# siliconsorcery/crdt

Hardware: AMD Instinct MI355X
Metric: merged records/sec (node) + % HBM roofline, 1B records x 1024 replicas (higher is better)
Workload: dtype int64

## Files before the change

crdt_amd/_capi.py:

```python
from __future__ import annotations

import ctypes
import os
import sys

_HERE = os.path.dirname(os.path.abspath(__file__))
LIB_PATH = os.environ.get("CRDT_LIB_PATH") or os.path.join(_HERE, "libcrdt_mi355x.so")

CRDT_OK = 0
CRDT_CLOCK_DRIFT = 1
CRDT_DUPLICATE_NODE = 2
CRDT_OVERFLOW = 3
CRDT_E_INVALID = -1
CRDT_E_HIP = -2
CRDT_E_NOMEM = -3
CRDT_E_KEY_RANGE = -4
CRDT_E_NO_DEVICE = -5
CRDT_E_COMM = -6

CRDT_MEM_HOST = 0
CRDT_MEM_DEVICE = 1
CRDT_NULL_VALUE = 0xFFFFFFFF


class CrdtBatch(ctypes.Structure):
    _fields_ = [("key_id", ctypes.c_void_p), ("lt", ctypes.c_void_p), ("rank", ctypes.c_void_p),
                ("val", ctypes.c_void_p), ("millis", ctypes.c_void_p), ("offsets", ctypes.c_void_p),
                ("n_changesets", ctypes.c_uint32), ("mem", ctypes.c_int32)]


class CrdtResult(ctypes.Structure):
    _fields_ = [("status", ctypes.c_int32), ("n_stored", ctypes.c_uint32),
                ("exc_changeset", ctypes.c_uint32), ("reserved", ctypes.c_uint32),
                ("exc_index", ctypes.c_uint64), ("canonical_lt", ctypes.c_int64),
                ("drift_ms", ctypes.c_int64), ("counter", ctypes.c_int64),
                ("n_present", ctypes.c_uint64), ("n_won", ctypes.c_uint64)]

    def as_dict(self) -> dict:
        return {f: getattr(self, f) for f, _ in self._fields_ if f != "reserved"}


class CrdtTiming(ctypes.Structure):
    _fields_ = [("scan_ms", ctypes.c_double), ("clock_ms", ctypes.c_double),
                ("apply_ms", ctypes.c_double), ("apply_launches", ctypes.c_uint32),
                ("apply_total", ctypes.c_uint32), ("total_ms", ctypes.c_double),
                ("route_ms", ctypes.c_double), ("part1_ms", ctypes.c_double), ("part2_ms", ctypes.c_double),
                ("resolve_ms", ctypes.c_double), ("part1_records", ctypes.c_uint64),
                ("sent_bytes", ctypes.c_uint64)]

    def as_dict(self) -> dict:
        return {f: getattr(self, f) for f, _ in self._fields_}


class CrdtExport(ctypes.Structure):
    _fields_ = [("key_id", ctypes.c_void_p), ("lt", ctypes.c_void_p), ("rank", ctypes.c_void_p),
                ("val", ctypes.c_void_p), ("mod", ctypes.c_void_p), ("n", ctypes.c_uint64),
                ("n_live", ctypes.c_uint64), ("mem", ctypes.c_int32), ("device", ctypes.c_int32)]


EXPORT_TILE = 2048
EXPORT_SCAN_STEP = 1024
EXPORT_COUNT_GRID = 2048
TABLE_TILE = 2048
TABLE_CLOCK_GRID = 2048
FANIN_MAX = 8
FANOUT_MAX = 8
SYNC_CLOCK_GRID = 2048

ALL_REDUCE_FN = ctypes.CFUNCTYPE(ctypes.c_int, ctypes.c_void_p, ctypes.c_void_p, ctypes.c_uint64, ctypes.c_int32,
                                 ctypes.c_void_p)
ALL_GATHER_FN = ctypes.CFUNCTYPE(ctypes.c_int, ctypes.c_void_p, ctypes.c_void_p, ctypes.c_void_p, ctypes.c_uint64,
                                 ctypes.c_void_p)
ALL_TO_ALL_FN = ctypes.CFUNCTYPE(ctypes.c_int, ctypes.c_void_p, ctypes.c_uint32, ctypes.POINTER(ctypes.c_void_p),
                                 ctypes.POINTER(ctypes.c_void_p), ctypes.POINTER(ctypes.c_uint32),
                                 ctypes.POINTER(ctypes.c_uint64), ctypes.POINTER(ctypes.c_uint64),
                                 ctypes.POINTER(ctypes.c_uint64), ctypes.POINTER(ctypes.c_uint64), ctypes.c_void_p)


class CrdtCommOps(ctypes.Structure):
    _fields_ = [("user", ctypes.c_void_p), ("mem", ctypes.c_int32), ("reserved", ctypes.c_int32),
                ("all_reduce_i64", ALL_REDUCE_FN), ("all_gather_i64", ALL_GATHER_FN),
                ("all_to_all_v", ALL_TO_ALL_FN)]


COMM_ID_BYTES = 128
ABI_VERSION = 5

_P = ctypes.c_void_p
_U32 = ctypes.c_uint32
_U64 = ctypes.c_uint64
_I64 = ctypes.c_int64
_I32 = ctypes.c_int32
_INT = ctypes.c_int

SIGNATURES = {
    "crdt_abi_version": (_INT, []),
    "crdt_status_string": (ctypes.c_char_p, [_INT]),
    "crdt_device_count": (_INT, [_P]),
    "crdt_create": (_INT, [_INT, _U32, _U64, _P]),
    "crdt_destroy": (None, [_P]),
    "crdt_reserve": (_INT, [_P, _U64]),
    "crdt_capacity": (_INT, [_P, _P]),
    "crdt_set_local_rank": (_INT, [_P, _U32]),
    "crdt_get_canonical": (_INT, [_P, _P]),
    "crdt_set_canonical": (_INT, [_P, _I64]),
    "crdt_put_rows": (_INT, [_P, _P, _P, _P, _P, _P, _U64, _I32]),
    "crdt_read_rows": (_INT, [_P, _P, _U64, _P, _P, _P, _P, _I32]),
    "crdt_modified_since": (_INT, [_P, _U64, _I64, _P, _P]),
    "crdt_export_since": (_INT, [_P, _U64, _I64, _P]),
    "crdt_export_read": (_INT, [_P, _U64, _U64, _P, _P, _P, _P, _P]),
    "crdt_export_release": (_INT, [_P]),
    "crdt_count_since": (_INT, [_P, _U64, _I64, _P, _P]),
    "crdt_export_flagged": (_INT, [_P, _U64, _P, _I32, ctypes.c_uint8, _P]),
    "crdt_clear_rows": (_INT, [_P, _U64, _U64]),
    "crdt_remap_ranks": (_INT, [_P, _U64, _P, _U32]),
    "crdt_put_stamped": (_INT, [_P, _P, _P, _U64, _I64, _I32, _P]),
    "crdt_refresh_canonical": (_INT, [_P, _U64, _P]),
    "crdt_merge": (_INT, [_P, _P, _I64, _P, _P]),
    "crdt_merge_table": (_INT, [_P, _P, _U64, _I64, _I64, _P, _I32, _P]),
    "crdt_sync_tables": (_INT, [_P, _P, _U64, _I64, _I64, _I64, _P, _P, _I32, _P, _P]),
    "crdt_fanin_tables": (_INT, [_P, _P, _P, _U32, _U64, _I64, _P, _I32, _P]),
    "crdt_fanout_tables": (_INT, [_P, _P, _P, _U32, _U64, _I64, _P, _I32, _P]),
    "crdt_comm_unique_id": (_INT, [_P]),
    "crdt_comm_init_rccl": (_INT, [_P, _U32, _U32, _P]),
    "crdt_comm_init_ops": (_INT, [_P, _U32, _U32, _P]),
    "crdt_comm_info": (_INT, [_P, _P, _P]),
    "crdt_comm_free": (_INT, [_P]),
    "crdt_set_presharded": (_INT, [_P, _INT]),
    "crdt_set_comm_timeout": (_INT, [_P, _U32]),
    "crdt_comm_state": (_INT, [_P, _P, _P]),
    "crdt_set_merge_path": (_INT, [_P, _INT]),
    "crdt_set_counts": (_INT, [_P, _INT]),
    "crdt_set_rank_bound": (_INT, [_P, _U32]),
    "crdt_reserve_scratch": (_INT, [_P, _U64]),
    "crdt_set_row_bytes": (_INT, [_P, _U32]),
    "crdt_last_plan": (_INT, [_P, _P]),
    "crdt_route_tune_info": (_INT, [_P, _P, _P]),
    "crdt_place_info": (_INT, [_P, _P, _P, _P, _P]),
    "crdt_last_path": (_INT, [_P, _P]),
    "crdt_set_timing": (_INT, [_P, _INT]),
    "crdt_get_timing": (_INT, [_P, _P]),
}


class NativeLibraryMissing(RuntimeError):
    pass


_lib = None


def load():
    global _lib
    if _lib is not None:
        return _lib
    if os.environ.get("CRDT_AMD_NO_TORCH") != "1" and "torch" not in sys.modules:
        try:
            import torch
        except ImportError:
            pass
    if not os.path.exists(LIB_PATH):
        raise NativeLibraryMissing(
            f"{LIB_PATH} is missing: build it with `python -c 'import __graft_entry__ as g; g.build()'`"
            " (there is no CPU fallback)")
    lib = ctypes.CDLL(LIB_PATH)
    for name, (res, args) in SIGNATURES.items():
        fn = getattr(lib, name)
        fn.restype = res
        fn.argtypes = args
    if lib.crdt_abi_version() != ABI_VERSION:
        raise NativeLibraryMissing(f"{LIB_PATH} has ABI {lib.crdt_abi_version()}, the bindings ABI {ABI_VERSION}:"
                                   " rebuild it")
    _lib = lib
    return lib


def status_string(status: int) -> str:
    return load().crdt_status_string(status).decode()


def device_count() -> int:
    n = ctypes.c_int(0)
    load().crdt_device_count(ctypes.byref(n))
    return n.value
```

crdt_amd/csrc/crdt_merge.hip:

```cpp
#include <dlfcn.h>
#include <hip/hip_runtime.h>
#include <rccl/rccl.h>

#include <stdint.h>
#include <stdio.h>
#include <stdlib.h>
#include <string.h>

#include <unistd.h>

#include <algorithm>
#include <atomic>
#include <chrono>
#include <thread>
#include <new>
#include <vector>

#include "crdt_merge.h"

namespace {

constexpr int kShift = 16;
constexpr int64_t kMaxCounter = 0xFFFF;
constexpr int64_t kMaxDrift = 60000;
// ... 27 lines not shown
}
__device__ inline uint2 load_cold(const Table& t, uint64_t k) {
    const u32x2u v = *reinterpret_cast<const u32x2u*>(row_ptr(t, k) + 16);
    return make_uint2(v.x, v.y);
}
__device__ inline void store_hc(const Table& t, uint64_t k, uint4 h, uint2 x) {
    char* p = row_ptr(t, k);
    if (t.stride == 32) {
        u32x8a a;
        a.s0 = h.x; a.s1 = h.y; a.s2 = h.z; a.s3 = h.w; a.s4 = x.x; a.s5 = x.y; a.s6 = 0u; a.s7 = 0u;
        *reinterpret_cast<u32x8a*>(p) = a;
        return;
    }
    u32x4u a;
    a.x = h.x; a.y = h.y; a.z = h.z; a.w = h.w;
    *reinterpret_cast<u32x4u*>(p) = a;
    u32x2u b;
    b.x = x.x; b.y = x.y;
    *reinterpret_cast<u32x2u*>(p + 16) = b;
}
__device__ inline int64_t row_mod(const Table& t, uint64_t k) {
    const uint4 h = load_hot(t, k);
    return (int64_t)(((uint64_t)h.w << 32) | load_cold(t, k).x);
}
__device__ inline void store_row(const Table& t, uint64_t k, int64_t lt, uint32_t rank, uint32_t val, int64_t mod) {
    store_hc(t, k, make_uint4((uint32_t)lt, (uint32_t)((uint64_t)lt >> 32), rank, (uint32_t)((uint64_t)mod >> 32)),
             make_uint2((uint32_t)mod, val));
}

struct Misc {
    uint32_t cand_count;
    uint32_t stop;
    uint32_t err;
    uint32_t vdone;
    uint32_t tiles_hot;
    crdt_result result;
    unsigned long long fr_lo, fr_hi;
    uint32_t fr_rlo, fr_rhi;
    unsigned long long key_end;
    unsigned long long route_own;
    unsigned long long shard_status;
    unsigned long long fr_cmax;
    unsigned long long hot_n;
    unsigned long long hot_spare;
    unsigned long long present[kCounterSlots];
    unsigned long long won[kCounterSlots];
};
static_assert(sizeof(Misc) % 16 == 0, "Misc is memset as whole 16-B words");

typedef unsigned int u32x4 __attribute__((ext_vector_type(4)));
typedef long long i64x2 __attribute__((ext_vector_type(2)));

__host__ __device__ inline int64_t wsub(int64_t a, int64_t b) { return (int64_t)((uint64_t)a - (uint64_t)b); }
__host__ __device__ inline int64_t imax(int64_t a, int64_t b) { return a > b ? a : b; }

struct HlcSend {
    int32_t status;
    int64_t drift_ms;
    int64_t counter;
    int64_t canonical;
    __host__ __device__ void into(crdt_result& res) const {
        res.status = status;
        res.drift_ms = drift_ms;
        res.counter = counter;
        res.canonical_lt = canonical;
    }
};
__host__ __device__ inline HlcSend hlc_send(int64_t r, int64_t wall) {
    const int64_t m = r >> kShift, mn = imax(m, wall);
    const int64_t cn = (m == mn) ? (r & kMaxCounter) + 1 : 0;
    if (wsub(mn, wall) > kMaxDrift) return {CRDT_CLOCK_DRIFT, wsub(mn, wall), 0, r};
    if (cn > kMaxCounter) return {CRDT_OVERFLOW, 0, cn, r};
    return {CRDT_OK, 0, 0, (int64_t)(((uint64_t)mn << kShift) + (uint64_t)cn)};
}

__device__ inline int64_t wave_max(int64_t v) {
#pragma unroll
    for (int off = 32; off > 0; off >>= 1) v = imax(v, __shfl_xor(v, off, 64));
    return v;
}

__device__ inline void block_raise_u64(unsigned long long v, unsigned long long* dst) {
    __shared__ unsigned long long s_v[4];
#pragma unroll
    for (int off = 32; off > 0; off >>= 1) {
        const unsigned long long o = __shfl_xor(v, off, 64);
        v = o > v ? o : v;
    }
    if ((threadIdx.x & 63) == 0) s_v[threadIdx.x >> 6] = v;
    __syncthreads();
    if (threadIdx.x == 0) {
        for (int w = 1; w < 4; ++w) v = s_v[w] > v ? s_v[w] : v;
        if (v > *(volatile unsigned long long*)dst) atomicMax(dst, v);
    }
    __syncthreads();
}

__device__ inline int64_t wave_scan_max_incl(int64_t v, int lane) {
#pragma unroll
    for (int off = 1; off < 64; off <<= 1) {
        int64_t u = __shfl_up(v, off, 64);
        if (lane >= off) v = imax(v, u);
    }
    return v;
}

__device__ inline uint32_t digit_count(uint32_t* bins, uint32_t d, bool act, int lane) {
    const unsigned long long a = __ballot(act);
    if (!a) return 0;
    const int L = __ffsll((long long)a) - 1;
    const uint32_t d0 = __shfl(d, L, 64);
    const bool same = act && d == d0;
    const unsigned long long m = __ballot(same);
    const unsigned long long below = (1ull << lane) - 1;
    uint32_t base = 0;
    if (lane == L) base = atomicAdd(&bins[d0], (uint32_t)__popcll(m));
    base = __shfl(base, L, 64);
    if (same) return base + (uint32_t)__popcll(m & below);
    return act ? atomicAdd(&bins[d], 1u) : 0u;
}

constexpr uint32_t kHotSample = 16;

__host__ __device__ inline uint64_t ord64(int64_t x) { return (uint64_t)x ^ (1ull << 63); }

constexpr uint32_t kHistSub = 7;

struct KeyMap {
    uint32_t gsh;
    uint32_t dsh;
};
__host__ __device__ inline uint32_t km_digit(KeyMap m, uint32_t k, uint32_t shift) {
    return ((((k & ((1u << m.gsh) - 1u)) << m.dsh) | ((k >> m.gsh) >> shift)) & 255u);
}

constexpr uint32_t kHotShift = 12;
constexpr uint32_t kHotProbe = 15;
constexpr uint32_t kHotMax = 256;

struct ScanHist {
    const uint32_t* key;
    const uint32_t* ptb;
    uint64_t cap;
    uint32_t shift;
    uint32_t* hist;
    KeyMap km{0u, 8u};
    uint32_t htile = kHistSub * kTile;
};
struct ScanHot {
    uint32_t hot = 0;
    uint32_t* hhist = nullptr;
};

__global__ __launch_bounds__(1024) void k_hot_count(const uint32_t* __restrict__ hhist, uint64_t tiles, uint32_t hot,
                                                    Misc* __restrict__ misc)
{
    __shared__ unsigned long long s_sum[16];
    unsigned long long n = 0;
    const uint64_t words = tiles * 256;
    for (uint64_t x = (uint64_t)blockIdx.x * 1024 + threadIdx.x; x < words; x += (uint64_t)gridDim.x * 1024)
        if ((x & 255u) < hot) n += hhist[x];
#pragma unroll
    for (int off = 32; off > 0; off >>= 1) n += __shfl_xor(n, off, 64);
    if ((threadIdx.x & 63) == 0) s_sum[threadIdx.x >> 6] = n;
    __syncthreads();
    if (threadIdx.x == 0) {
        for (int k = 1; k < 16; ++k) n += s_sum[k];
        if (n) atomicAdd(&misc->hot_n, n);
    }
}

template <bool kEager, bool kMillis, bool kFrame, bool kHist, bool kVec, bool kHot = false>
__device__ __forceinline__ void scan_body(
    const int64_t* __restrict__ lt, const uint32_t* __restrict__ rank,
    const int64_t* __restrict__ millis, const uint64_t* __restrict__ offs,
    const uint32_t* __restrict__ tstart, uint32_t jbase, int64_t c0,
    int64_t wall, uint32_t local_rank,
    int64_t* __restrict__ T, Misc* __restrict__ misc, uint32_t* __restrict__ cand_tile, ScanHist sh, bool jx,
    ScanHot ho = ScanHot{})
{
    __shared__ int64_t s_max[kScanThreads / 64];
    __shared__ int s_flag[kScanThreads / 64];
    __shared__ unsigned long long s_fr[kFrame ? 5 * (kScanThreads / 64) : 1];
    constexpr uint32_t kBins = kHot ? 512u : 256u;
    __shared__ uint32_t s_h[kHist ? 2 * kBins : 1];
    static_assert(!kHist || kScanThreads == 256, "one histogram bin per thread");
    static_assert(!kHot || kHist, "hot bins: beside the fused histogram");
    const uint32_t j = jbase + (jx ? blockIdx.x : blockIdx.y);
    const uint64_t beg = offs[j], end = offs[j + 1];
    const uint32_t t0 = tstart[j], nt = tstart[j + 1] - t0;
    const int lane = threadIdx.x & 63, w = threadIdx.x >> 6;
    constexpr uint32_t kStep = kHist ? kHistSub : 1u;
    const uint32_t ustride = jx ? gridDim.y : gridDim.x;
    for (uint32_t u = jx ? blockIdx.y : blockIdx.x; u * kStep < nt; u += ustride) {
      if (kHist) {
#pragma unroll
        for (uint32_t x = 0; x < (kHist ? 2 * kBins : 0u); x += 256) s_h[kHist ? x + threadIdx.x : 0] = 0;
        __syncthreads();
      }
      const uint32_t te = std::min<uint32_t>(u * kStep + kStep, nt);
      for (uint32_t t = u * kStep; t < te; ++t) {
        const uint64_t base = beg + (uint64_t)t * kTile;
        int64_t m = INT64_MIN;
        int f = 0;
        int64_t v[kScanItems];
        uint32_t rk[kEager ? kScanItems : 1];
        int64_t mv[kEager && kMillis ? kScanItems : 1];
        uint32_t kk[kHist ? kScanItems : 1];
        auto idx = [&](int q) -> uint64_t {
            return kVec ? base + (uint64_t)(q >> 2) * (4 * kScanThreads) + threadIdx.x * 4u + (q & 3)
                        : base + (uint64_t)q * kScanThreads + threadIdx.x;
        };
        bool vec_done[kVec ? kScanItems / 4 : 1];
#pragma unroll
        for (int g = 0; g < (kVec ? kScanItems / 4 : 0); ++g) {
            const uint64_t i0 = idx(4 * g);
            vec_done[kVec ? g : 0] = i0 + 4 <= end;
            if (i0 + 4 <= end) {
                const u32x4u a = *reinterpret_cast<const u32x4u*>(lt + i0);
                const u32x4u b = *reinterpret_cast<const u32x4u*>(lt + i0 + 2);
                v[4 * g] = (int64_t)(((uint64_t)a.y << 32) | a.x); v[4 * g + 1] = (int64_t)(((uint64_t)a.w << 32) | a.z);
                v[4 * g + 2] = (int64_t)(((uint64_t)b.y << 32) | b.x); v[4 * g + 3] = (int64_t)(((uint64_t)b.w << 32) | b.z);
                if (kHist) {
                    const u32x4u kv = *reinterpret_cast<const u32x4u*>(sh.key + i0);
                    kk[kHist ? 4 * g : 0] = kv.x; kk[kHist ? 4 * g + 1 : 0] = kv.y;
                    kk[kHist ? 4 * g + 2 : 0] = kv.z; kk[kHist ? 4 * g + 3 : 0] = kv.w;
                }
                if (kEager) {
                    const u32x4u rv = *reinterpret_cast<const u32x4u*>(rank + i0);
                    rk[kEager ? 4 * g : 0] = rv.x; rk[kEager ? 4 * g + 1 : 0] = rv.y;
                    rk[kEager ? 4 * g + 2 : 0] = rv.z; rk[kEager ? 4 * g + 3 : 0] = rv.w;
                }
            }
        }
#pragma unroll
        for (int q = 0; q < kScanItems; ++q) {
            const uint64_t i = idx(q);
            const bool vd = kVec && vec_done[kVec ? q >> 2 : 0];
            if (!vd) {
                v[q] = i < end ? lt[i] : INT64_MIN;
                if (kHist) kk[kHist ? q : 0] = i < end ? __builtin_nontemporal_load(sh.key + i) : UINT32_MAX;
            }
            if (kEager) {
                if (!vd) rk[kEager ? q : 0] = i < end ? rank[i] : 0u;
                if (kMillis) mv[kMillis ? q : 0] = (millis && i < end) ? millis[i] : 0;
            }
            m = imax(m, v[q]);
        }
        if (kHist) {
            const uint32_t tb = (t - u * kStep) * (uint32_t)kTile;
#pragma unroll
            for (int q = 0; q < kScanItems; ++q) {
                const uint32_t k = kk[kHist ? q : 0];
                const uint32_t gb = kVec ? (uint32_t)(q >> 2) * (4u * kScanThreads) : (uint32_t)q * kScanThreads;
                uint32_t dg = km_digit(sh.km, k, sh.shift);
                if (kHot) dg = (k >> kHotShift) < ho.hot ? 256u + (k >> kHotShift) : dg;
                digit_count(s_h + (tb + gb >= sh.htile ? kBins : 0u), dg, (k >> sh.km.gsh) < sh.cap, lane);
            }
        }
#pragma unroll
        for (int q = 0; q < kScanItems; ++q) {
            if (v[q] > c0) {
                const uint64_t i = idx(q);
                const int64_t ms = (kMillis && millis) ? (kEager ? mv[kEager && kMillis ? q : 0] : millis[i])
                                                       : (v[q] >> kShift);
                const uint32_t r = kEager ? rk[kEager ? q : 0] : rank[i];
                f |= (r == local_rank) | (wsub(ms, wall) > kMaxDrift);
            }
        }
        unsigned long long flo = 0, fhi = 0, frl = 0, frh = 0;
        uint32_t fcm = 0;
        if (kFrame) {
#pragma unroll
            for (int q = 0; q < kScanItems; ++q) {
                const uint64_t i = idx(q);
                if (i < end) {
                    const uint64_t o = ord64(v[q]);
                    flo = ~o > flo ? ~o : flo;
                    fhi = o > fhi ? o : fhi;
                    fcm = std::max<uint32_t>(fcm, (uint32_t)v[q] & 0xFFFFu);
                    if (kEager) {
                        const uint32_t r = rk[kEager ? q : 0];
                        frl = (uint32_t)~r > frl ? (uint32_t)~r : frl;
                        frh = r > frh ? r : frh;
                    }
                }
            }
#pragma unroll
            for (int off = 32; off > 0; off >>= 1) {
                const unsigned long long a = __shfl_xor(flo, off, 64), b = __shfl_xor(fhi, off, 64);
                const unsigned long long c = __shfl_xor(frl, off, 64), d = __shfl_xor(frh, off, 64);
                flo = a > flo ? a : flo; fhi = b > fhi ? b : fhi; frl = c > frl ? c : frl; frh = d > frh ? d : frh;
                fcm = std::max<uint32_t>(fcm, (uint32_t)__shfl_xor(fcm, off, 64));
            }
            if (lane == 0) {
                s_fr[5 * w] = flo; s_fr[5 * w + 1] = fhi; s_fr[5 * w + 2] = frl; s_fr[5 * w + 3] = frh; s_fr[5 * w + 4] = fcm;
            }
        }
        m = wave_max(m);
        const int fw = __any(f) | (m > c0 ? 2 : 0);
        if (lane == 0) { s_max[w] = m; s_flag[w] = fw; }
        __syncthreads();
        if (threadIdx.x == 0) {
            if (kFrame) {
                unsigned long long fc = fcm;
                for (int k = 1; k < kScanThreads / 64; ++k) {
                    flo = s_fr[5 * k] > flo ? s_fr[5 * k] : flo;
                    fhi = s_fr[5 * k + 1] > fhi ? s_fr[5 * k + 1] : fhi;
                    frl = s_fr[5 * k + 2] > frl ? s_fr[5 * k + 2] : frl;
                    frh = s_fr[5 * k + 3] > frh ? s_fr[5 * k + 3] : frh;
                    fc = s_fr[5 * k + 4] > fc ? s_fr[5 * k + 4] : fc;
                }
                if (fc > *(volatile unsigned long long*)&misc->fr_cmax) atomicMax(&misc->fr_cmax, fc);
                if (flo > *(volatile unsigned long long*)&misc->fr_lo) atomicMax(&misc->fr_lo, flo);
                if (fhi > *(volatile unsigned long long*)&misc->fr_hi) atomicMax(&misc->fr_hi, fhi);
                if ((uint32_t)frl > *(volatile uint32_t*)&misc->fr_rlo) atomicMax(&misc->fr_rlo, (uint32_t)frl);
                if ((uint32_t)frh > *(volatile uint32_t*)&misc->fr_rhi) atomicMax(&misc->fr_rhi, (uint32_t)frh);
            }
            int64_t tm = s_max[0];
            int tf = s_flag[0];
            for (int k = 1; k < kScanThreads / 64; ++k) { tm = imax(tm, s_max[k]); tf |= s_flag[k]; }
            T[t0 + t] = tm;
// ... 1233 lines not shown
        n = 0;
    }
};

template <typename T>
struct HBuf {
    T* p = nullptr;
    size_t n = 0;
    hipError_t ensure(size_t want) {
        if (want <= n && p) return hipSuccess;
        if (p) { hipHostFree(p); p = nullptr; n = 0; }
        size_t m = std::max<size_t>(want, 16);
        hipError_t e = hipHostMalloc(&p, m * sizeof(T), hipHostMallocDefault);
        if (e == hipSuccess) n = m;
        return e;
    }
    void release() { if (p) hipHostFree(p); p = nullptr; n = 0; }
};

constexpr uint32_t kRl1MaxPieces = 4;
struct Rl1Scratch {
    DBuf<uint32_t> hist, toff, part, choff, dstart2, tseg, ibase, ibucket, ksu32, kj2;
    DBuf<int64_t> kslt;
    DBuf<u32x4> rec2;
    DBuf<uint64_t> plan;
    HBuf<uint64_t> hplan;
    size_t pw = 0, u32w = 0;
    uint32_t nt2 = 0, nc2 = 0;
    uint32_t ngrp = 0;
    size_t nsg = 0;
    uint64_t nw = 0;
    void release() {
        hist.release(); toff.release(); part.release(); choff.release(); dstart2.release(); tseg.release();
        ibase.release(); ibucket.release(); ksu32.release(); kj2.release(); kslt.release(); rec2.release();
        plan.release(); hplan.release();
    }
};

struct Segs {
    std::vector<uint64_t> beg, end;
    std::vector<uint32_t> j;
    void from_offsets(const uint64_t* offs, uint32_t R) {
        beg.resize(R); end.resize(R); j.resize(R);
        for (uint32_t x = 0; x < R; ++x) { beg[x] = offs[x]; end[x] = offs[x + 1]; j[x] = x; }
    }
};

}

constexpr uint32_t kFormNoWholeLines = 64;
constexpr uint32_t kFormNoKey8 = 128;
constexpr uint32_t kFormNoKey16 = 256;
constexpr uint32_t kFormNoReverse = 512;
constexpr uint32_t kFormNoHistW = 1024;
constexpr uint32_t kFormNoHw = 2048;
constexpr uint32_t kFormNoVecLoads = 8192;
constexpr uint32_t kFormNoVecScan = 32768;
constexpr uint32_t kFormNoVecRoute = 131072;
constexpr uint32_t kFormBigTile2 = 65536;
constexpr uint32_t kFormNoOwnInPlace = 524288;
constexpr uint32_t kFormNoCompact = 1u << 20;
constexpr uint32_t kFormFbackXcd = 1u << 21;
constexpr uint32_t kFormFbackWide = 1u << 22;
constexpr uint32_t kFormScanJx = 1u << 24;
constexpr uint32_t kFormNoScanJx = 1u << 25;
constexpr uint32_t kFormNoPosT = 1u << 31;
constexpr uint32_t kFormNoItemLists = 1u << 28;
constexpr uint32_t kFormNoFbackPre = 1u << 27;
constexpr uint32_t kFormFbackPre512 = 1u << 29;
constexpr uint32_t kFormNoSparseK = 1u << 26;
constexpr uint32_t kScanJxMax = 8192;
constexpr uint32_t kFormOverlap = 1u << 23;
constexpr uint32_t kPartPad = 1024;
constexpr uint32_t kPutGrid = 2048;

struct crdt_ctx {
    int device = 0;
    hipStream_t stream = nullptr;
    uint32_t local_rank = 0;
    Table table{nullptr, 24};
    uint64_t cap = 0;
    int64_t canonical = 0;

    Misc* d_misc = nullptr;
    Misc* h_misc = nullptr;
    DBuf<long long> d_M;
    DBuf<long long> d_event;
    DBuf<uint64_t> d_plan;
    HBuf<uint64_t> h_plan;
    const uint64_t* d_offs = nullptr;
    const uint32_t* d_tstart = nullptr;
    DBuf<int64_t> d_T, d_Cprev, d_Rj, d_Cj, d_candP, d_candms;
    DBuf<uint32_t> d_candtile, d_candkind;
    DBuf<long long> d_candkey;
    DBuf<uint32_t> s_key, s_rank, s_val;
    hipStream_t cstream = nullptr;
    std::vector<hipEvent_t> cevents;
    const uint32_t* kv_key = nullptr;
    const uint32_t* kv_val = nullptr;
    uint64_t kv_n = 0, kv_done = 0, kv_window = 4ull << 20;
    uint32_t kv_win = 0;
    DBuf<int64_t> s_lt, s_millis, s_mod;
    DBuf<uint8_t> s_flags;
    DBuf<uint32_t> s_out;
    DBuf<uint32_t> x_key, x_rank, x_val, x_counts;
    DBuf<int64_t> x_lt, x_mod;
    DBuf<uint64_t> x_offs;
    DBuf<unsigned long long> x_words;
    bool x_valid = false;
    uint64_t x_n = 0;
    DBuf<uint32_t> t_sel;
    DBuf<unsigned long long> t_words, t_mask;
    DBuf<uint8_t> t_wflags;
    DBuf<uint8_t> t_fstep, t_fmask;
    DBuf<unsigned long long> t_fcounts;
    bool table_merge = true;
    bool last_table = false;
    bool last_sync = false;
    bool last_fanin = false;
    bool last_fanout = false;
    DBuf<long long> d_word;
    DBuf<unsigned long long> d_ibase;
    uint32_t plan_R = 0;
    uint64_t plan_tiles = 0;
    uint32_t plan_mt = 0;
    int apply_items = 0;
    bool timing = false;
    std::vector<hipEvent_t> events;
    std::vector<uint32_t> windows;
    bool sorted_phases = false;
    uint64_t p1_records = 0;
    uint32_t apply_total = 0;
    int merge_path = 0;
    uint64_t hw = 0;
    uint64_t hw_read = 0;
    uint64_t hw_next = 0;
    bool key_end_valid = false;
    DBuf<u32x4> p1_rec, p2_rec;
    DBuf<uint32_t> p1_kj, p2_kj;
    static constexpr int kPlaceMax = 4;
    DBuf<u32x4> pc_rec[kPlaceMax];
    DBuf<uint32_t> pc_kj[kPlaceMax];
    int place_k = 0;
    int place_trial = 0;
    int place_best = -1;
    int place_idle = 0;
    float place_ms[kPlaceMax] = {};
    bool place_timed = false;
    bool place_warm = false;
    hipEvent_t place_ev[2] = {};
    DBuf<uint32_t> p_hist, p_toff, p_part, p_choff, p_dstart1, p_dstart2, p_l2map;
    DBuf<uint64_t> p_plan, p_l1beg;
    DBuf<uint32_t> p_ibase, p_ksu32, p_tseg, p_ibucket;
    DBuf<uint32_t> p_ilist;
    HBuf<uint32_t> h_ilist;
    DBuf<int64_t> p_kslt;
    HBuf<uint64_t> h_pplan;
    bool last_sorted = false;
    bool counts = true;
    bool fused = false;
    bool scan_eager = false;
    bool no_fuse = false;
    bool xcd_map = true;
    bool packed_resolve = true;
    bool frame_on = false;
    uint32_t rank_bound = 0;
    uint32_t form_off = 0;
    bool env_dynamic = false;
    bool hist_fuse = true;
    uint32_t l1_tile = 0;
    uint32_t plan_l1_tile = 28672;
    bool last_hist1_fused = false;
    bool frame_lt_only = false;
    const uint32_t* d_ptb = nullptr;
    uint64_t plan_ptiles = 0;
    DBuf<uint32_t> p_hist1;
    bool hist1_fused = false;
    bool hist1_routed = false;
    const uint32_t* hist1_key = nullptr;
    uint32_t hist1_shift = 0;
    bool last_packed = false;
    bool last_wire_pk = false;
    bool last_own_in_place = false;
    bool last_key8 = false;
    bool last_key16 = false;
    bool last_compact = false;
    bool last_hw = false;
    bool flags_sorted = true;
    int fback_chk = 6;
    bool last_flagged = false;
    int combine = 1;
    bool last_combined = false;
    uint32_t sparse_t = 2048;
    uint32_t hot_buckets = 256;
    uint32_t hot_share = 5;
    uint32_t hot_probe = kHotProbe;
    uint32_t hot_skip = 0;
    uint32_t hist1_hot = 0;
    bool last_hot_direct = false;
    DBuf<uint32_t> p_hist1h, p_toffh, p_dstarth;
    DBuf<uint64_t> p_l1begh;
    int route_l1 = 1;
    bool rl1_call_head = false;
    bool rl1_call_all = false;
    bool rl1_cmp = false;
    bool last_rl1_head = false;
    uint64_t last_rl1_head_in = 0, last_rl1_head_out = 0;
    uint32_t last_rl1_head_digits = 0;
    uint64_t sent_bytes = 0;
    uint32_t rl1_pieces = 2;
    uint32_t rl1_call_pieces = 2;
    uint32_t last_rl1_pieces = 0;
    bool last_route_l1 = false;
    bool route_tune = true;
    struct RouteTune {
        uint64_t shape = 0;
        uint32_t trial = 0;
        int best = -1;
        long long us[5] = {-1, -1, -1, -1, -1};
    } rt;
    int tune_mode = -1;
    bool tune_trial = false;
    DBuf<long long> d_tune;
    HBuf<long long> h_tune;
    DBuf<uint32_t> rl_rec;
    DBuf<uint16_t> rl_k16;
    uint64_t rl_cap = 0;
    Rl1Scratch rl_os[kRl1MaxPieces + 1];
    Rl1Scratch rl_hf;
    DBuf<uint32_t> rl_hrec;
    DBuf<uint16_t> rl_hk16;
    DBuf<unsigned long long> rl_hcnt;
    HBuf<unsigned long long> h_hcnt;
    hipEvent_t rl_evh = nullptr;
    hipEvent_t ov_ev[2] = {};
    DBuf<uint32_t> e_key, e_val;
    DBuf<uint64_t> e_pk;
    DBuf<unsigned long long> e_cnt, e_cur;
    HBuf<unsigned long long> h_ebase;
    DBuf<uint32_t> e_icnt;
    DBuf<uint32_t> e_bbase;
    DBuf<uint64_t> e_off;
    DBuf<unsigned long long> e_csum;
    bool last_ordered = false;
    DBuf<uint16_t> f_pos1, f_pos2;
    DBuf<uint8_t> f_flag1, f_flag2;
    DBuf<uint32_t> f_hist2, f_toff2;
    DBuf<unsigned long long> f_cin_key;
    DBuf<uint32_t> f_cin_val;
    DBuf<uint8_t> f_cin_pres;
    bool keys_checked = false;
    bool resolved = false;
    crdt_timing last_timing{};
    Segs segs;
    uint32_t n_ranks = 1, rank = 0;
    bool has_comm = false;
    bool presharded = false;
    crdt_comm_ops ops{};
    void* rccl_comm = nullptr;
    DBuf<long long> d_gsend, d_grecv, d_pbase, d_sum;
    DBuf<unsigned long long> d_rcnt, d_rrecv;
    DBuf<unsigned long long> d_rcur;
    hipEvent_t route_ev = nullptr;
    hipStream_t sstream = nullptr;
    hipStream_t ostream = nullptr;
    hipEvent_t rl_evs[kRl1MaxPieces] = {};
    hipEvent_t rl_evx[kRl1MaxPieces] = {};
    hipEvent_t rl_evo = nullptr;
    uint64_t recv_cap = 0;
    HBuf<uint64_t> h_rcnt;
    DBuf<uint32_t> r_skey, r_srank, r_sval, r_key, r_rank, r_val;
    DBuf<int64_t> r_slt, r_lt;
    DBuf<uint64_t> r_perm;
    DBuf<uint8_t> r_flags, r_sflags;
    HBuf<uint8_t> h_stage;
    HBuf<long long> h_sum;
    DBuf<long long> d_agree;
    HBuf<long long> h_agree;
    DBuf<unsigned long long> d_rl1cnt;
    HBuf<uint64_t> h_rl1cnt;
    bool finish_posted = false;
    int fail_rank = -1, fail_at = 0;
    uint32_t comm_timeout_ms = 300000;
    int64_t comm_deadline_ns = 0;
    std::atomic<int> comm_state{0};
    std::atomic<const char*> comm_phase{"idle"};
    int stall_rank = -1, stall_at = 0, stall_ms = 0;
    bool stall_dev = false;
};

constexpr uint32_t kL1TileDefault = 28672;
inline uint32_t l1_choose(const crdt_ctx* c, uint32_t R, uint64_t n) {
    if (c->l1_tile == 14336u || c->l1_tile == 28672u) return c->l1_tile;
    return R && n / R < 4ull * kL1TileDefault ? 14336u : kL1TileDefault;
}
inline uint32_t l1_plan_tile(const crdt_ctx* c) { return c->plan_l1_tile; }


namespace {

#define HIPCHK(expr)                                   \
    do {                                               \
        hipError_t _e = (expr);                        \
        if (_e != hipSuccess) return CRDT_E_HIP;       \
    } while (0)

#define HIPALLOC(expr)                                                     \
    do {                                                                   \
        hipError_t _e = (expr);                                            \
        if (_e == hipErrorOutOfMemory) return CRDT_E_NOMEM;                \
        if (_e != hipSuccess) return CRDT_E_HIP;                           \
    } while (0)

#define HIPLST(expr)                                                       \
    do {                                                                   \
        hipError_t _e = (expr);                                            \
        if (_e != hipSuccess && !lst) lst = CRDT_E_HIP;                    \
    } while (0)

int comm_wait(crdt_ctx* c, hipStream_t s, hipEvent_t e = nullptr);
#define SYNCHK(c, s)                                                       \
    do {                                                                   \
        int _w = comm_wait((c), (s));                                      \
        if (_w) return _w;                                                 \
    } while (0)

inline unsigned grid_for(uint64_t n, unsigned per) { return (unsigned)((n + per - 1) / per); }

hipError_t ensure_events(crdt_ctx* c, size_t n) {
    while (c->events.size() < n) {
        hipEvent_t e;
        hipError_t r = hipEventCreate(&e);
        if (r != hipSuccess) return r;
        c->events.push_back(e);
    }
    return hipSuccess;
}

int overlap_fork(crdt_ctx* c) {
    if (!c->sstream) HIPCHK(hipStreamCreateWithFlags(&c->sstream, hipStreamNonBlocking));
    for (hipEvent_t& e : c->ov_ev)
        if (!e) HIPCHK(hipEventCreateWithFlags(&e, hipEventDisableTiming));
    HIPCHK(hipEventRecord(c->ov_ev[0], c->stream));
    HIPCHK(hipStreamWaitEvent(c->sstream, c->ov_ev[0], 0));
    return CRDT_OK;
}
int overlap_join(crdt_ctx* c) {
    HIPCHK(hipEventRecord(c->ov_ev[1], c->sstream));
    HIPCHK(hipStreamWaitEvent(c->stream, c->ov_ev[1], 0));
    return CRDT_OK;
}

template <typename T>
int stage(crdt_ctx* c, DBuf<T>& buf, const T* src, uint64_t n, int32_t mem, const T** out) {
    if (!src) { *out = nullptr; return CRDT_OK; }
    if (mem == CRDT_MEM_DEVICE) { *out = src; return CRDT_OK; }
    HIPALLOC(buf.ensure(n ? n : 1));
    if (n) HIPCHK(hipMemcpyAsync(buf.p, src, n * sizeof(T), hipMemcpyHostToDevice, c->stream));
    *out = buf.p;
    return CRDT_OK;
}

struct Cols {
    const uint32_t* key = nullptr;
    const int64_t* lt = nullptr;
    const uint32_t* rank = nullptr;
    const uint32_t* val = nullptr;
    const int64_t* millis = nullptr;
    bool packed_in = false;
};

int validate_batch(const crdt_batch* b) {
    if (!b || !b->offsets) return CRDT_E_INVALID;
    if (b->mem != CRDT_MEM_HOST && b->mem != CRDT_MEM_DEVICE) return CRDT_E_INVALID;
    if (b->offsets[0] != 0) return CRDT_E_INVALID;
    for (uint32_t j = 0; j < b->n_changesets; ++j)
        if (b->offsets[j + 1] < b->offsets[j]) return CRDT_E_INVALID;
    const uint64_t n = b->offsets[b->n_changesets];
    if (n > 0 && (!b->lt || !b->rank)) return CRDT_E_INVALID;
    if ((uint64_t)b->n_changesets >= (1ull << 24)) return CRDT_E_INVALID;
    for (uint32_t j = 0; j < b->n_changesets; ++j)
        if (b->offsets[j + 1] - b->offsets[j] >= kLowMask) return CRDT_E_INVALID;
    return CRDT_OK;
}

int stage_check_cols(crdt_ctx* c, const crdt_batch* b, Cols* cols) {
    const uint64_t n = b->offsets[b->n_changesets];
    int st;
    if ((st = stage(c, c->s_lt, b->lt, n, b->mem, &cols->lt))) return st;
    if ((st = stage(c, c->s_rank, b->rank, n, b->mem, &cols->rank))) return st;
    if ((st = stage(c, c->s_millis, b->millis, n, b->mem, &cols->millis))) return st;
    return CRDT_OK;
}

int stage_apply_cols(crdt_ctx* c, const crdt_batch* b, Cols* cols) {
    const uint64_t n = b->offsets[b->n_changesets];
    if (n > 0 && (!b->key_id || !b->val)) return CRDT_E_INVALID;
    int st;
    if ((st = stage(c, c->s_key, b->key_id, n, b->mem, &cols->key))) return st;
    if ((st = stage(c, c->s_lt, b->lt, n, b->mem, &cols->lt))) return st;
    if ((st = stage(c, c->s_rank, b->rank, n, b->mem, &cols->rank))) return st;
    if ((st = stage(c, c->s_val, b->val, n, b->mem, &cols->val))) return st;
    return CRDT_OK;
}

int upload_plan(crdt_ctx* c, const crdt_batch* b, uint64_t* tiles_out, uint32_t* max_tiles) {
    const uint32_t R = b->n_changesets;
    const size_t half = (R + 2) / 2;
    const size_t words = (R + 1) + 2 * half;
    HIPALLOC(c->h_plan.ensure(words));
    HIPALLOC(c->d_plan.ensure(words));
    uint64_t* h_offs = c->h_plan.p;
    uint32_t* h_tstart = reinterpret_cast<uint32_t*>(c->h_plan.p + (R + 1));
    uint32_t* h_ptb = reinterpret_cast<uint32_t*>(c->h_plan.p + (R + 1) + half);
    uint64_t tiles = 0, ptiles = 0;
    uint32_t mt = 0;
    c->plan_l1_tile = l1_choose(c, R, b->offsets[R] - b->offsets[0]);
    for (uint32_t j = 0; j <= R; ++j) {
        h_offs[j] = b->offsets[j];
        h_tstart[j] = (uint32_t)tiles;
        h_ptb[j] = (uint32_t)ptiles;
        if (j < R) {
            const uint64_t nj = b->offsets[j + 1] - b->offsets[j];
            const uint64_t tj = (nj + kTile - 1) / kTile;
            tiles += tj;
            ptiles += (nj + l1_plan_tile(c) - 1) / l1_plan_tile(c);
            mt = std::max<uint32_t>(mt, (uint32_t)tj);
        }
    }
    if (tiles >= (1ull << 32)) return CRDT_E_INVALID;
    HIPCHK(hipMemcpyAsync(c->d_plan.p, c->h_plan.p, words * sizeof(uint64_t), hipMemcpyHostToDevice, c->stream));
    c->d_offs = c->d_plan.p;
    c->d_tstart = reinterpret_cast<const uint32_t*>(c->d_plan.p + (R + 1));
    c->d_ptb = reinterpret_cast<const uint32_t*>(c->d_plan.p + (R + 1) + half);
    c->plan_ptiles = ptiles;
    *tiles_out = tiles;
    *max_tiles = mt;
    return CRDT_OK;
}

int reset_misc(crdt_ctx* c) {
    HIPCHK(hipMemsetAsync(c->d_misc, 0, sizeof(Misc), c->stream));
    return CRDT_OK;
}

crdt_result cleared_result(int64_t canonical) {
    crdt_result res;
    memset(&res, 0, sizeof(res));
    res.exc_index = UINT64_MAX;
    res.canonical_lt = canonical;
    return res;
}

constexpr size_t kEvStart = 0, kEvScan = 1, kEvClock = 2, kEvApply = 3, kEvEnd = 4;
inline size_t ev_window(size_t k, bool end) { return 5 + 2 * k + (end ? 1 : 0); }
inline size_t events_for(size_t nsegs) {
    return std::max(ev_window(nsegs / kTimingStride + 2, true), ev_window(3, true)) + 1;
}

inline void raise_hw(crdt_ctx* c, uint64_t key_end) {
    c->hw = std::max<uint64_t>(c->hw, std::min<uint64_t>(key_end, c->cap));
}

inline void ev_record(crdt_ctx* c, size_t idx) {
    if (c->timing && idx < c->events.size()) hipEventRecord(c->events[idx], c->stream);
}

int phase_scan(crdt_ctx* c, const crdt_batch* home, int64_t wall, long long* d_maxima, bool allow_fuse = false,
               bool frame = false, bool bound_ok = true, bool keys_ready = false, const KeyMap* route_km = nullptr) {
    c->fused = false;
    c->resolved = false;
    c->hist1_fused = false;
    c->hist1_hot = 0;
    int st = validate_batch(home);
    if (st) return st;
    const uint32_t R = home->n_changesets;
    Cols cols;
    if ((st = stage_check_cols(c, home, &cols))) return st;
    uint64_t tiles = 0;
    uint32_t mt = 0;
    if ((st = upload_plan(c, home, &tiles, &mt))) return st;
    HIPALLOC(c->d_T.ensure(tiles + 1));
    HIPALLOC(c->d_candtile.ensure(tiles + 1));
    HIPALLOC(c->d_candkey.ensure(tiles + 1));
    HIPALLOC(c->d_candP.ensure(tiles + 1));
    HIPALLOC(c->d_candkind.ensure(tiles + 1));
    HIPALLOC(c->d_candms.ensure(tiles + 1));
    if ((st = reset_misc(c))) return st;
    if (!tiles)
        k_fill_i64<<<grid_for(std::max<uint32_t>(R, 1), 256), 256, 0, c->stream>>>(d_maxima, std::max<uint32_t>(R, 1),
                                                                                     INT64_MIN);
    c->plan_R = R;
    c->plan_tiles = tiles;
    c->plan_mt = mt;
    c->frame_on = frame;
    c->frame_lt_only = frame && bound_ok && c->rank_bound && !c->scan_eager;
    c->fused = allow_fuse && !c->no_fuse && tiles > 0 && tiles <= kClockTilesMax && R <= kClockRMax;
    const bool hist = c->frame_lt_only && c->hist_fuse && keys_ready && home->mem == CRDT_MEM_DEVICE &&
                      R <= kWindow && tiles > 0 && home->key_id;
    const bool rhist = !hist && route_km && frame && c->hist_fuse && R <= kWindow && tiles > 0 && home->key_id &&
                       !home->millis;
    if (hist || rhist) {
        HIPALLOC(c->p_hist1.ensure(c->plan_ptiles * kDigits));
        c->hist1_fused = true;
        c->hist1_routed = rhist;
        c->hist1_key = home->key_id;
        c->hist1_shift = rhist || c->cap > (1ull << 20) ? 20u : (uint32_t)kSBits;
    }
    uint32_t hot = hist && c->cap > (1ull << 20) ? std::min<uint32_t>(c->hot_buckets, kHotMax) : 0u;
    if (hot && c->hot_skip) {
        --c->hot_skip;
        hot = 0;
    }
    if (hot) {
        HIPALLOC(c->p_hist1h.ensure(c->plan_ptiles * kDigits));
        c->hist1_hot = hot;
    }
    const ScanHot shot{hot, c->p_hist1h.p};
    ScanHist shr{home->key_id, c->d_ptb, c->cap, 20u, c->p_hist1.p};
    shr.htile = l1_plan_tile(c);
    ScanHist shist{home->key_id, c->d_ptb, c->cap, c->hist1_shift, c->p_hist1.p};
    shist.htile = l1_plan_tile(c);
    if (rhist) shr.km = *route_km;
    if (tiles) {
        const uint32_t cap_x = std::max<uint32_t>(1, 65536u / std::max<uint32_t>(R, 1));
        const uint32_t gx = std::max<uint32_t>(1, std::min<uint32_t>(mt, cap_x));
        const uint32_t gxh = std::max<uint32_t>(1, std::min<uint32_t>((mt + kHistSub - 1) / kHistSub, cap_x));
        const bool hgrid = hist || rhist;
        const uint64_t nwg = (uint64_t)(hgrid ? gxh : gx) * R;
        const bool jx = !(c->form_off & kFormNoScanJx) && ((c->form_off & kFormScanJx) || nwg <= kScanJxMax);
        for (uint32_t jb = 0; jb < R; jb += 65535) {
            const uint32_t gy = std::min<uint32_t>(65535, R - jb);
            const dim3 gdh = jx ? dim3(gy, std::min<uint32_t>(gxh, 65535)) : dim3(gxh, gy);
            const dim3 gd = jx ? dim3(gy, std::min<uint32_t>(gx, 65535)) : dim3(gx, gy);
            if (rhist)
                k_scan<true, false, true, true, true><<<gdh, kScanThreads, 0, c->stream>>>(
                    cols.lt, cols.rank, nullptr, c->d_offs, c->d_tstart, jb, c->canonical, wall,
                    c->local_rank, c->d_T.p, c->d_misc, c->d_candtile.p, shr, jx);
            else if (hist && hot && !(c->form_off & kFormNoVecScan))
                k_scan<true><<<gdh, kScanThreads, 0, c->stream>>>(
                    cols.lt, cols.rank, cols.millis, c->d_offs, c->d_tstart, jb, c->canonical, wall,
                    c->local_rank, c->d_T.p, c->d_misc, c->d_candtile.p, shist, jx, shot);
            else if (hist && hot)
                k_scan<false><<<gdh, kScanThreads, 0, c->stream>>>(
                    cols.lt, cols.rank, cols.millis, c->d_offs, c->d_tstart, jb, c->canonical, wall,
                    c->local_rank, c->d_T.p, c->d_misc, c->d_candtile.p, shist, jx, shot);
            else if (hist && !(c->form_off & kFormNoVecScan))
                k_scan<false, true, true, true, true><<<gdh, kScanThreads, 0, c->stream>>>(
                    cols.lt, cols.rank, cols.millis, c->d_offs, c->d_tstart, jb, c->canonical, wall,
                    c->local_rank, c->d_T.p, c->d_misc, c->d_candtile.p,
                    shist, jx);
            else if (hist)
                k_scan<false, true, true, true><<<gdh, kScanThreads, 0, c->stream>>>(
                    cols.lt, cols.rank, cols.millis, c->d_offs, c->d_tstart, jb, c->canonical, wall,
                    c->local_rank, c->d_T.p, c->d_misc, c->d_candtile.p, shist, jx);
            else if (c->frame_lt_only)
                k_scan<false, true, true><<<gd, kScanThreads, 0, c->stream>>>(
                    cols.lt, cols.rank, cols.millis, c->d_offs, c->d_tstart, jb, c->canonical, wall,
                    c->local_rank, c->d_T.p, c->d_misc, c->d_candtile.p, ScanHist{}, jx);
            else if (frame && !cols.millis)
                k_scan<true, false, true><<<gd, kScanThreads, 0, c->stream>>>(
                    cols.lt, cols.rank, nullptr, c->d_offs, c->d_tstart, jb, c->canonical, wall,
                    c->local_rank, c->d_T.p, c->d_misc, c->d_candtile.p, ScanHist{}, jx);
            else if (frame)
                k_scan<true, true, true><<<gd, kScanThreads, 0, c->stream>>>(
                    cols.lt, cols.rank, cols.millis, c->d_offs, c->d_tstart, jb, c->canonical, wall,
                    c->local_rank, c->d_T.p, c->d_misc, c->d_candtile.p, ScanHist{}, jx);
            else if (c->scan_eager && !cols.millis)
                k_scan<true, false><<<gd, kScanThreads, 0, c->stream>>>(
                    cols.lt, cols.rank, nullptr, c->d_offs, c->d_tstart, jb, c->canonical, wall,
                    c->local_rank, c->d_T.p, c->d_misc, c->d_candtile.p, ScanHist{}, jx);
            else if (c->scan_eager)
                k_scan<true><<<gd, kScanThreads, 0, c->stream>>>(
                    cols.lt, cols.rank, cols.millis, c->d_offs, c->d_tstart, jb, c->canonical, wall,
                    c->local_rank, c->d_T.p, c->d_misc, c->d_candtile.p, ScanHist{}, jx);
            else
                k_scan<false><<<gd, kScanThreads, 0, c->stream>>>(
                    cols.lt, cols.rank, cols.millis, c->d_offs, c->d_tstart, jb, c->canonical, wall,
                    c->local_rank, c->d_T.p, c->d_misc, c->d_candtile.p, ScanHist{}, jx);
        }
        if (hot)
            k_hot_count<<<64, 1024, 0, c->stream>>>(c->p_hist1h.p, c->plan_ptiles, hot, c->d_misc);
        if (!c->fused)
            k_tmax<<<std::min<uint32_t>(R, 4096), 256, 0, c->stream>>>(c->d_T.p, c->d_tstart, R, d_maxima);
        HIPCHK(hipGetLastError());
    }
    return CRDT_OK;
}

int phase_clock(crdt_ctx* c, const crdt_batch* home, int64_t wall, const long long* d_maxima,
                long long* d_event, const long long* d_pbase = nullptr,
                const unsigned long long* d_ibase_in = nullptr) {
    const uint32_t R = c->plan_R;
    if (!home || home->n_changesets != R) return CRDT_E_INVALID;
    int st;
    Cols cols;
    if ((st = stage_check_cols(c, home, &cols))) return st;
    HIPALLOC(c->d_Cprev.ensure(R + 1));
    HIPALLOC(c->d_Rj.ensure(R + 1));
    HIPALLOC(c->d_Cj.ensure(R + 1));
    const unsigned long long* d_ibase = d_ibase_in;
    if (!R) k_event_init<<<1, 64, 0, c->stream>>>(d_event);
    if (c->fused) {
        k_clock<true><<<1, 1024, 0, c->stream>>>(nullptr, c->d_T.p, c->d_tstart, R, wall, c->canonical,
                                                 c->d_Cprev.p, c->d_Rj.p, c->d_Cj.p, d_event);
        k_verify<true><<<kVerifyBlocks, 64, 0, c->stream>>>(
            cols.lt, cols.rank, cols.millis, c->d_offs, c->d_tstart, R, c->d_T.p, c->d_Cprev.p, wall,
            c->local_rank, c->d_misc, c->d_candtile.p, c->d_candkey.p, c->d_candP.p, c->d_candkind.p,
            c->d_candms.p, d_pbase, d_ibase, d_event, c->canonical, c->d_Rj.p, c->d_Cj.p, (uint32_t)kTile);
        c->resolved = true;
        HIPCHK(hipGetLastError());
        return CRDT_OK;
    }
    if (R) k_clock<false><<<1, 1024, 0, c->stream>>>(d_maxima, nullptr, nullptr, R, wall, c->canonical,
                                                     c->d_Cprev.p, c->d_Rj.p, c->d_Cj.p, d_event);
    if (c->plan_tiles)
        k_verify<false><<<kVerifyBlocks, 64, 0, c->stream>>>(
            cols.lt, cols.rank, cols.millis, c->d_offs, c->d_tstart, R, c->d_T.p, c->d_Cprev.p, wall,
            c->local_rank, c->d_misc, c->d_candtile.p, c->d_candkey.p, c->d_candP.p, c->d_candkind.p,
            c->d_candms.p, d_pbase, d_ibase, d_event, 0, nullptr, nullptr, (uint32_t)kTile);
    HIPCHK(hipGetLastError());
    return CRDT_OK;
}

int phase_resolve(crdt_ctx* c, long long* d_event) {
    k_resolve_local<<<1, 256, 0, c->stream>>>(c->d_misc, c->d_candkey.p, c->d_candP.p, c->d_candkind.p,
                                              c->d_candms.p, d_event);
    HIPCHK(hipGetLastError());
    return CRDT_OK;
}


int kv_copy_next(crdt_ctx* c) {
    const uint64_t b = c->kv_done, e = std::min<uint64_t>(c->kv_n, b + c->kv_window);
    if (c->kv_win >= c->cevents.size()) {
        hipEvent_t ev;
        HIPCHK(hipEventCreateWithFlags(&ev, hipEventDisableTiming));
        c->cevents.push_back(ev);
    }
    HIPCHK(hipMemcpyAsync(c->s_key.p + b, c->kv_key + b, (e - b) * sizeof(uint32_t), hipMemcpyHostToDevice,
                          c->cstream));
    HIPCHK(hipMemcpyAsync(c->s_val.p + b, c->kv_val + b, (e - b) * sizeof(uint32_t), hipMemcpyHostToDevice,
                          c->cstream));
    HIPCHK(hipEventRecord(c->cevents[c->kv_win], c->cstream));
    HIPCHK(hipStreamWaitEvent(c->stream, c->cevents[c->kv_win], 0));
    c->kv_win++;
    c->kv_done = e;
    return CRDT_OK;
}

int kv_copy_all(crdt_ctx* c) {
    while (c->kv_key && c->kv_done < c->kv_n) {
        int st = kv_copy_next(c);
        if (st) return st;
    }
    return CRDT_OK;
}

int comm_all_reduce(crdt_ctx* c, long long* d, uint64_t n, int32_t op);
void test_stall(crdt_ctx* c, int point);

PackFrame frame_of(const crdt_ctx* c) {
    const Misc* m = c->h_misc;
    const bool any = m->fr_lo != 0 || m->fr_hi != 0;
    const bool bound = c->frame_lt_only;
    const uint32_t rlo = bound ? (any ? ~0u : 0u) : m->fr_rlo;
    const uint32_t rhi = bound ? (any ? c->rank_bound - 1 : 0u) : m->fr_rhi;
    PackFrame f = make_frame(m->fr_lo, m->fr_hi, rlo, rhi, c->plan_R);
    f.rk_limit = bound ? c->rank_bound : UINT32_MAX;
    return f;
}

int finish_apply(crdt_ctx* c, uint8_t* host_flags, const uint8_t* dflags, uint64_t n, bool sorted,
                 crdt_result* out, int local_st = 0) {
    const bool counted = !sorted || c->counts || c->last_flagged;
    if (c->has_comm) {
        c->finish_posted = true;
        k_sum_counts<<<1, 64, 0, c->stream>>>(c->d_misc, counted, c->d_sum.p, local_st);
        int st = comm_all_reduce(c, c->d_sum.p, kSumWords + kSumCodes, CRDT_REDUCE_SUM);
        if (st) return st;
        test_stall(c, 5);
        HIPCHK(hipMemcpyAsync(c->h_sum.p, c->d_sum.p, (kSumWords + kSumCodes) * sizeof(long long),
                              hipMemcpyDeviceToHost, c->stream));
    } else if (local_st) {
        return local_st;
    }
    HIPCHK(hipMemcpyAsync(c->h_misc, c->d_misc, sizeof(Misc), hipMemcpyDeviceToHost, c->stream));
    if (host_flags && n && !local_st) HIPCHK(hipMemcpyAsync(host_flags, dflags, n, hipMemcpyDeviceToHost, c->stream));
    SYNCHK(c, c->stream);
    if (c->has_comm)
        for (int k = kSumCodes - 1; k > 0; --k)
            if (c->h_sum.p[kSumWords + k]) return -k;
    crdt_result res = c->h_misc->result;
    c->scan_eager = 2ull * kHotSample * c->h_misc->tiles_hot > c->plan_tiles;
    if (c->key_end_valid && !c->has_comm)
        c->hw_next = std::max<uint64_t>(c->hw, std::min<uint64_t>(c->h_misc->key_end, c->cap));
    uint64_t np = 0, nw = 0;
    for (int s = 0; s < kCounterSlots; ++s) { np += c->h_misc->present[s]; nw += c->h_misc->won[s]; }
    bool all_counted = counted, err = c->h_misc->err != 0;
    if (c->has_comm) {
        np = (uint64_t)c->h_sum.p[0];
        nw = (uint64_t)c->h_sum.p[1];
        err = c->h_sum.p[2] != 0;
        all_counted = c->h_sum.p[3] == 0;
    }
    res.n_present = all_counted ? np : UINT64_MAX;
    res.n_won = all_counted ? nw : UINT64_MAX;
    if (c->h_misc->err & 2u) {
        res.status = CRDT_E_INVALID;
        res.canonical_lt = c->canonical;
        if (out) *out = res;
        return res.status;
    }
    if (err) {
        res.status = CRDT_E_KEY_RANGE;
        if ((sorted || c->keys_checked) && (c->h_misc->err & 1u)) {
            res.canonical_lt = c->canonical;
            if (out) *out = res;
            return res.status;
        }
    }
    c->canonical = res.canonical_lt;
    if (out) *out = res;
    return res.status;
}

int apply_ranges(crdt_ctx* c, const Cols& cols, const Segs& sg, uint64_t n, int32_t mem,
                 int64_t wall, const long long* d_event, uint8_t* win_flags, crdt_result* out) {
    const uint32_t R = c->plan_R;
    uint8_t* dflags = nullptr;
    if (win_flags) {
        if (mem == CRDT_MEM_DEVICE) {
            dflags = win_flags;
        } else {
            HIPALLOC(c->s_flags.ensure(n ? n : 1));
// ... 7 lines not shown
    c->keys_checked = !c->kv_key;
    if (c->keys_checked && n)
        k_key_check<<<std::min<uint32_t>(grid_for(n, 256 * 16), 8192), 256, 0, c->stream>>>(cols.key, n, c->cap,
                                                                                           c->d_misc);
    ev_record(c, kEvApply);
    c->windows.clear();
    uint32_t nl = 0;
    c->apply_total = 0;
    bool win_open = false;
    uint32_t win_n = 0;
    for (size_t s = 0; s < sg.j.size(); ++s) {
      const uint32_t j = sg.j[s];
      for (uint64_t pb = sg.beg[s], pe; pb < sg.end[s]; pb = pe) {
        pe = sg.end[s];
        if (c->kv_key) {
            while (c->kv_done <= pb) {
                int st = kv_copy_next(c);
                if (st) return st;
            }
            pe = std::min<uint64_t>(pe, c->kv_done);
        }
        const uint64_t b = pb, e = pe;
        if (c->timing && b == sg.beg[s] && (nl++ % kTimingStride) == 0 && !win_open) {
            win_open = true;
            win_n = 0;
            ev_record(c, ev_window(c->windows.size(), false));
        }
        c->apply_total++;
        const int items = c->apply_items ? c->apply_items : ((e - b) >= (512ull << 10) ? 4 : 2);
        const unsigned grid = grid_for(e - b, (uint64_t)kApplyThreads * items);
        if (items == 8)
            k_apply<8><<<grid, kApplyThreads, 0, c->stream>>>(cols.key, cols.lt, cols.rank, cols.val, b, e, j,
                                                              c->table, c->cap, c->d_Rj.p, c->d_misc, dflags);
        else if (items == 4)
            k_apply<4><<<grid, kApplyThreads, 0, c->stream>>>(cols.key, cols.lt, cols.rank, cols.val, b, e, j,
                                                              c->table, c->cap, c->d_Rj.p, c->d_misc, dflags);
        else if (items == 2)
            k_apply<2><<<grid, kApplyThreads, 0, c->stream>>>(cols.key, cols.lt, cols.rank, cols.val, b, e, j,
                                                              c->table, c->cap, c->d_Rj.p, c->d_misc, dflags);
        else
            k_apply<1><<<grid, kApplyThreads, 0, c->stream>>>(cols.key, cols.lt, cols.rank, cols.val, b, e, j,
                                                              c->table, c->cap, c->d_Rj.p, c->d_misc, dflags);
        if (win_open && ++win_n == kTimingWindow) {
            ev_record(c, ev_window(c->windows.size(), true));
            c->windows.push_back(win_n);
            win_open = false;
        }
      }
    }
    if (win_open) {
        ev_record(c, ev_window(c->windows.size(), true));
        c->windows.push_back(win_n);
    }
    HIPCHK(hipGetLastError());
    return finish_apply(c, win_flags && mem == CRDT_MEM_HOST ? win_flags : nullptr, dflags, n, false, out);
}

#ifdef CRDT_PROF_RESOLVE
void prof_resolve_report() {
        unsigned long long pr[8];
        hipMemcpyFromSymbol(pr, HIP_SYMBOL(g_rprof), sizeof(pr));
        fprintf(stderr, "[rprof] items %llu chunks %llu | per item: init %.2f us final %.2f us | per chunk: "
                "A %.2f us B %.2f us | max chunk B %.2f us, max item %.2f us\n", pr[4], pr[5],
                pr[0] / 100.0 / (pr[4] ? pr[4] : 1), pr[3] / 100.0 / (pr[4] ? pr[4] : 1),
                pr[1] / 100.0 / (pr[5] ? pr[5] : 1), pr[2] / 100.0 / (pr[5] ? pr[5] : 1), pr[6] / 100.0,
                pr[7] / 100.0);
        memset(pr, 0, sizeof(pr));
        hipMemcpyToSymbol(HIP_SYMBOL(g_rprof), pr, sizeof(pr));
        static std::vector<unsigned long long> it(1 << 18);
        hipMemcpyFromSymbol(it.data(), HIP_SYMBOL(g_item_dur), it.size() * 8);
        uint64_t hist[8] = {0}, hsum[8] = {0};
        unsigned long long top = 0;
        size_t top_i = 0;
        for (size_t i = 0; i < it.size(); ++i) {
            const double us = (it[i] >> 24) / 100.0;
            if (!it[i]) continue;
            int b = us < 25 ? 0 : us < 50 ? 1 : us < 100 ? 2 : us < 200 ? 3 : us < 400 ? 4 : us < 800 ? 5 : us < 1600 ? 6 : 7;
            hist[b]++;
            hsum[b] += (it[i] >> 8) & 0xFFFF;
            if (it[i] > top) { top = it[i]; top_i = i; }
        }
        fprintf(stderr, "[rprof] items by duration <25/50/100/200/400/800/1600/more us: ");
        for (int b = 0; b < 8; ++b) fprintf(stderr, "%llu(%.1f ch) ", (unsigned long long)hist[b], hist[b] ? (double)hsum[b] / hist[b] : 0.0);
        fprintf(stderr, "| slowest item %zu: %.1f us, %llu chunks, flags %llu\n", top_i, (top >> 24) / 100.0,
                (top >> 8) & 0xFFFF, top & 3);
        std::fill(it.begin(), it.end(), 0ull);
        hipMemcpyToSymbol(HIP_SYMBOL(g_item_dur), it.data(), it.size() * 8);
}
#endif

void place_take(crdt_ctx* c, size_t rec_units, size_t kj_units) {
    size_t free_b = 0, total_b = 0;
    if (hipMemGetInfo(&free_b, &total_b) != hipSuccess) free_b = total_b = 0;
    const size_t cb = rec_units * sizeof(u32x4) + kj_units * sizeof(uint32_t);
    size_t used = 0;
    int k = 1;
    for (; k < c->place_k; ++k) {
        if (used + cb > total_b / 8 || free_b < used + cb + total_b / 4) break;
        if (c->pc_rec[k].ensure(rec_units) != hipSuccess || c->pc_kj[k].ensure(kj_units) != hipSuccess) {
            c->pc_rec[k].release();
            c->pc_kj[k].release();
            break;
        }
        used += cb;
    }
    c->place_k = k;
    if (k == 1) {
        c->place_trial = 0;
        c->place_best = 0;
    }
}

void place_drop(crdt_ctx* c) {
    for (int i = 1; i < crdt_ctx::kPlaceMax; ++i) { c->pc_rec[i].release(); c->pc_kj[i].release(); }
    c->place_k = 1;
    c->place_trial = 0;
    c->place_best = 0;
}

int apply_sorted(crdt_ctx* c, const Cols& cols, const Segs& sg, int64_t wall, const long long* d_event,
                 crdt_result* out, uint8_t* dflags = nullptr,
                 EmitOut* emit = nullptr) {
    const uint32_t R = c->plan_R;
    const bool fl = dflags != nullptr;
    const bool em = emit != nullptr;
    if (!em) {
        if (!c->resolved)
            k_resolve<<<1, 64, 0, c->stream>>>(d_event, R, wall, c->canonical, c->d_Rj.p, c->d_Cj.p, c->d_misc);
        c->resolved = false;
        ev_record(c, kEvApply);
        c->windows.clear();
        c->apply_total = 1;
        if (c->timing) ev_record(c, ev_window(0, false));
    }
    const bool two = c->cap > (1ull << 20);
    const uint32_t shift1 = two ? 20u : (uint32_t)kSBits;
    const size_t ns_all = sg.j.size();
    PackFrame pf{};
    bool pk = false;
    if (cols.packed_in || (c->packed_resolve && c->frame_on)) {
        HIPCHK(hipMemcpyAsync(c->h_misc, c->d_misc, sizeof(Misc), hipMemcpyDeviceToHost, c->stream));
        SYNCHK(c, c->stream);
        pf = frame_of(c);
        pk = pf.ok;
        if (cols.packed_in && !pk) return CRDT_E_INVALID;
    }
    if ((fl || em) && (!pk || cols.packed_in)) return CRDT_E_INVALID;
    const bool ord = !em && (fl || (c->counts && pk && !cols.packed_in));
    c->last_ordered = ord;
    c->last_packed = pk;
    c->key_end_valid = true;
    c->last_hist1_fused = false;
    c->last_hot_direct = false;
    c->sorted_phases = false;
    const bool k8 = pk && two && pf.key4 && !(c->form_off & kFormNoKey8);
    const bool k16 = k8 && !(c->form_off & kFormNoKey16);
    bool cmp = false;
    if (k16 && (ord || !c->counts) && !em && !c->has_comm && !cols.packed_in && c->frame_on &&
        !(c->form_off & (kFormNoCompact | kFormNoHistW | kFormBigTile2 | kFormNoWholeLines | kFormNoVecLoads))) {
        const PackFrame cf = compact_frame(pf, (uint32_t)std::min<unsigned long long>(c->h_misc->fr_cmax, 0xFFFFull),
                                           c->plan_R);
        if (cf.cb) {
            pf = cf;
            cmp = true;
        }
    }
    c->last_compact = cmp;
    c->last_key8 = k8;
    c->last_key16 = k16;
    c->last_hw = pk && (!c->counts || ord) && c->hw_read < c->cap;
    const uint32_t win0 = pk ? pf.jwin : kWindow;
    const bool pt1 = fl && cmp && ns_all && sg.j[0] / win0 == sg.j[ns_all - 1] / win0 &&
                     !(c->form_off & (kFormNoPosT | kFormNoFbackPre | kFormFbackWide)) &&
                     !(c->xcd_map && (c->form_off & kFormFbackXcd));
    if (fl && !pt1) {
        uint64_t ncol = 0;
        for (size_t s = 0; s < ns_all; ++s) ncol = std::max<uint64_t>(ncol, sg.end[s]);
        HIPALLOC(c->f_pos1.ensure((ncol ? ncol : 1) + 8));
    }
    for (size_t sb = 0; sb < ns_all;) {
        const uint32_t win = pk ? pf.jwin : kWindow;
        const uint32_t jb = sg.j[sb] - sg.j[sb] % win;
        size_t se = sb;
        uint64_t nw = 0;
        while (se < ns_all && sg.j[se] < jb + win) { nw += sg.end[se] - sg.beg[se]; ++se; }
        const uint32_t nseg = (uint32_t)(se - sb);
        const size_t s0 = sb;
        sb = se;
        if (nw == 0) continue;
        if (s0 > 0) SYNCHK(c, c->stream);
        const size_t u32_words = (2 * (size_t)nseg + 2) / 2;
        const size_t words = 2 * (size_t)nseg + u32_words + 3;
        HIPALLOC(c->h_pplan.ensure(words));
        HIPALLOC(c->p_plan.ensure(words));
        uint64_t* h_beg = c->h_pplan.p;
        uint64_t* h_end = c->h_pplan.p + nseg;
        uint32_t* h_sj = reinterpret_cast<uint32_t*>(c->h_pplan.p + 2 * (size_t)nseg);
        uint32_t* tb = h_sj + nseg;
        uint32_t nt1 = 0;
        const uint32_t l1t = !c->l1_tile ? l1_plan_tile(c) : c->l1_tile;
        for (uint32_t s = 0; s <= nseg; ++s) {
            tb[s] = nt1;
            if (s < nseg) {
                h_beg[s] = sg.beg[s0 + s];
                h_end[s] = sg.end[s0 + s];
                h_sj[s] = sg.j[s0 + s];
                nt1 += (uint32_t)((h_end[s] - h_beg[s] + l1t - 1) / l1t);
            }
        }
        const uint32_t nc1 = (nt1 + kChunkTiles - 1) / kChunkTiles;
        const size_t tail = 2 * (size_t)nseg + u32_words;
        uint32_t* sm_t = reinterpret_cast<uint32_t*>(c->h_pplan.p + tail);
        sm_t[0] = 0; sm_t[1] = nt1;
        uint32_t* sm_c = reinterpret_cast<uint32_t*>(c->h_pplan.p + tail + 1);
        sm_c[0] = 0; sm_c[1] = nc1;
        c->h_pplan.p[tail + 2] = 0;
        HIPCHK(hipMemcpyAsync(c->p_plan.p, c->h_pplan.p, words * sizeof(uint64_t), hipMemcpyHostToDevice,
                              c->stream));
        const uint32_t nt2 = two ? (uint32_t)((nw + kPTile2 - 1) / kPTile2) + kDigits : 0;
        const uint32_t nc2 = two ? (nt2 + kChunkTiles - 1) / kChunkTiles + kDigits : 0;
        const uint32_t ntm = std::max(nt1, nt2), ncm = std::max(nc1, nc2);
        HIPALLOC(c->p_hist.ensure((size_t)ntm * kDigits));
        HIPALLOC(c->p_toff.ensure((size_t)ntm * kDigits));
        HIPALLOC(c->p_part.ensure((size_t)ncm * kDigits));
        HIPALLOC(c->p_choff.ensure((size_t)ncm * kDigits));
        HIPALLOC(c->p_dstart1.ensure(kDigits + 1));
        const size_t rec_units = (pk ? (3 * (size_t)nw + 3) / 4 : (size_t)nw) + kPartPad;
        const size_t kj1_units = (k16 ? ((size_t)nw + 1) / 2 : (size_t)nw) + kPartPad;
        const size_t kj2_units = (k8 ? ((size_t)nw + 3) / 4 : (size_t)nw) + kPartPad;
        if (c->place_k > 1 && c->place_trial < 0 && !c->has_comm && s0 == 0 && !c->place_warm) {
            c->place_warm = true;
            place_take(c, rec_units, kj1_units);
        }
        if (c->place_k > 1 && c->place_trial >= 0 && c->place_trial < 2 * c->place_k && !c->has_comm && s0 == 0 &&
            !c->place_timed) {
            const int k = c->place_trial % c->place_k;
            if (k) {
                HIPALLOC(c->pc_rec[k].ensure(rec_units));
                HIPALLOC(c->pc_kj[k].ensure(kj1_units));
                std::swap(c->p1_rec, c->pc_rec[k]);
                std::swap(c->p1_kj, c->pc_kj[k]);
            }
            for (hipEvent_t& e : c->place_ev)
                if (!e) HIPCHK(hipEventCreate(&e));
            c->place_timed = true;
        }
        HIPALLOC(c->p1_rec.ensure(rec_units)); HIPALLOC(c->p1_kj.ensure(kj1_units));
        u32x4* p1r = c->p1_rec.p;
        uint32_t* p1k = c->p1_kj.p;
        u32x4* p2r = nullptr;
        uint32_t* p2k = nullptr;
        const uint64_t* d_beg = c->p_plan.p;
        const uint64_t* d_end = c->p_plan.p + nseg;
        const uint32_t* d_sj = reinterpret_cast<const uint32_t*>(c->p_plan.p + 2 * (size_t)nseg);
        const uint32_t* d_tb1 = d_sj + nseg;
        HIPALLOC(c->p_tseg.ensure(ntm));
        k_seg_index<<<std::min<uint32_t>(grid_for(nt1, 256), 4096), 256, 0, c->stream>>>(d_tb1, nseg, nt1, c->p_tseg.p);
        const TileMap tm1{d_beg, d_end, d_tb1, c->p_tseg.p, d_sj, nseg, l1t};
        const ScanMap sm1z{reinterpret_cast<const uint32_t*>(c->p_plan.p + tail),
                          reinterpret_cast<const uint32_t*>(c->p_plan.p + tail + 1), c->p_plan.p + tail + 2, 1};
        if (two) HIPALLOC(c->p_l1beg.ensure(kDigits + 1));
        const bool h1 = c->hist1_fused && !c->hist1_routed && s0 == 0 && se == ns_all && !cols.packed_in &&
                        cols.key == c->hist1_key && c->hist1_shift == shift1 && nt1 == c->plan_ptiles &&
                        l1t == l1_plan_tile(c);
        const uint32_t* hist1 = h1 ? c->p_hist1.p : c->p_hist.p;
        const uint32_t hb = h1 ? c->hist1_hot : 0u;
        const uint64_t hot_n = hb && pk ? std::min<uint64_t>(c->h_misc->hot_n, nw) : 0;
        const bool hotp = hb && cmp && !ord && !em && two && !c->has_comm && hot_n * 100 >= (uint64_t)c->hot_share * nw;
        if (hb && !hotp) {
            k_hot_fold<<<std::min<uint32_t>(nt1, 1024u), 64, 0, c->stream>>>(c->p_hist1.p, c->p_hist1h.p, nt1);
            c->hist1_hot = 0;
            c->hot_skip = c->hot_probe;
        }
        c->last_hot_direct = hotp;
        if (hotp) {
            HIPALLOC(c->p_toffh.ensure((size_t)nt1 * kDigits));
            HIPALLOC(c->p_dstarth.ensure(kDigits + 1));
            HIPALLOC(c->p_l1begh.ensure(kDigits + 1));
            HIPALLOC(c->p2_rec.ensure(rec_units));
            k_hist_trim<<<256, 256, 0, c->stream>>>(c->p_hist1h.p, c->d_ptb, R, c->d_misc);
            k_scan_part<<<nc1, 256, 0, c->stream>>>(c->p_hist1h.p, sm1z, c->p_part.p);
            k_scan_seg<<<1, 256, 0, c->stream>>>(c->p_part.p, sm1z, c->p_choff.p, c->p_dstarth.p, c->p_l1begh.p);
            k_scan_tiles<<<nc1, 256, 0, c->stream>>>(c->p_hist1h.p, c->p_choff.p, sm1z, c->p_dstarth.p, c->p_toffh.p);
        }
        const ScanMap sm1 = hotp ? ScanMap{sm1z.tbase, sm1z.cbase, c->p_l1begh.p + kDigits, 1} : sm1z;
        if (h1)
            k_hist_trim<<<256, 256, 0, c->stream>>>(c->p_hist1.p, c->d_ptb, R, c->d_misc);
        else
            k_part_hist<true><<<nt1, kHThreads, 0, c->stream>>>(cols.key, tm1, jb, c->d_misc,
                                                                 c->cap, shift1, c->p_hist.p);
        c->last_hist1_fused = h1;
        k_scan_part<<<nc1, 256, 0, c->stream>>>(hist1, sm1, c->p_part.p);
        k_scan_seg<<<1, 256, 0, c->stream>>>(c->p_part.p, sm1, c->p_choff.p, c->p_dstart1.p,
                                             two ? c->p_l1beg.p : nullptr);
        k_scan_tiles<<<nc1, 256, 0, c->stream>>>(hist1, c->p_choff.p, sm1, c->p_dstart1.p, c->p_toff.p);
        const bool ph = c->timing && s0 == 0 && !em;
        if (ph) ev_record(c, ev_window(1, false));
        if (c->place_timed && s0 == 0) HIPCHK(hipEventRecord(c->place_ev[0], c->stream));
        const uint32_t xper1 = c->xcd_map ? (nt1 + kXcds - 1) / kXcds : 0;
        const bool rev1 = c->xcd_map && !(c->form_off & kFormNoReverse);
        if (pt1) HIPALLOC(c->f_pos1.ensure((size_t)nt1 * kPTile + 16));
        if (pt1)
            k_part_scatter1<true, false, true, kL1Items, true, true, true, true, true>
                <<<xcd_grid(nt1, c->xcd_map), kPThreads, 0, c->stream>>>(
                cols.key, cols.lt, cols.rank, cols.val, tm1, jb, c->d_misc, c->cap, shift1, c->p_toff.p, p1r,
                p1k, xper1, pf, rev1 ? hist1 : nullptr, c->f_pos1.p, hist1);
        else if (cmp && fl)
            k_part_scatter1<true, false, true, kL1Items, true, true, true, true>
                <<<xcd_grid(nt1, c->xcd_map), kPThreads, 0, c->stream>>>(
                cols.key, cols.lt, cols.rank, cols.val, tm1, jb, c->d_misc, c->cap, shift1, c->p_toff.p, p1r,
                p1k, xper1, pf, rev1 ? hist1 : nullptr, c->f_pos1.p, hist1);
        else if (hotp)
            k_part_scatter1<kL1Items><<<xcd_grid(nt1, c->xcd_map), kPThreads, 0, c->stream>>>(
                cols.key, cols.lt, cols.rank, cols.val, tm1, jb, c->d_misc, c->cap, shift1, c->p_toff.p, p1r,
                p1k, xper1, pf, rev1 ? hist1 : nullptr,
                HotL1{hb, c->p_toffh.p, rev1 ? c->p_hist1h.p : nullptr, c->p2_rec.p});
        else if (cmp)
            k_part_scatter1<true, false, true, kL1Items, true, true, false, true>
                <<<xcd_grid(nt1, c->xcd_map), kPThreads, 0, c->stream>>>(
                cols.key, cols.lt, cols.rank, cols.val, tm1, jb, c->d_misc, c->cap, shift1, c->p_toff.p, p1r,
                p1k, xper1, pf, rev1 ? hist1 : nullptr);
        else if (fl && k16)
            k_part_scatter1<true, false, true, kL1Items, true, true, true>
                <<<xcd_grid(nt1, c->xcd_map), kPThreads, 0, c->stream>>>(
                cols.key, cols.lt, cols.rank, cols.val, tm1, jb, c->d_misc, c->cap, shift1, c->p_toff.p, p1r,
                p1k, xper1, pf, rev1 ? hist1 : nullptr, c->f_pos1.p, hist1);
        else if (fl)
            k_part_scatter1<true, false, false, kL1Items, true, false, true>
                <<<xcd_grid(nt1, c->xcd_map), kPThreads, 0, c->stream>>>(
                cols.key, cols.lt, cols.rank, cols.val, tm1, jb, c->d_misc, c->cap, shift1, c->p_toff.p, p1r,
                p1k, xper1, pf, rev1 ? hist1 : nullptr, c->f_pos1.p, hist1);
        else if (cols.packed_in && k16)
            k_part_scatter1<true, true, true, kL1Items, true><<<xcd_grid(nt1, c->xcd_map), kPThreads, 0, c->stream>>>(
                cols.key, cols.lt, cols.rank, cols.val, tm1, jb, c->d_misc, c->cap, shift1, c->p_toff.p, p1r,
                p1k, xper1, pf, rev1 ? hist1 : nullptr);
        else if (cols.packed_in)
            k_part_scatter1<true, true, false, kL1Items, true><<<xcd_grid(nt1, c->xcd_map), kPThreads, 0, c->stream>>>(
                cols.key, cols.lt, cols.rank, cols.val, tm1, jb, c->d_misc, c->cap, shift1, c->p_toff.p, p1r,
                p1k, xper1, pf, rev1 ? hist1 : nullptr);
        else if (k16 && !(c->form_off & kFormNoVecLoads))
            k_part_scatter1<true, false, true, kL1Items, true><<<xcd_grid(nt1, c->xcd_map), kPThreads, 0, c->stream>>>(
                cols.key, cols.lt, cols.rank, cols.val, tm1, jb, c->d_misc, c->cap, shift1, c->p_toff.p, p1r,
                p1k, xper1, pf, rev1 ? hist1 : nullptr);
        else if (k16)
            k_part_scatter1<true, false, true><<<xcd_grid(nt1, c->xcd_map), kPThreads, 0, c->stream>>>(
                cols.key, cols.lt, cols.rank, cols.val, tm1, jb, c->d_misc, c->cap, shift1, c->p_toff.p, p1r,
                p1k, xper1, pf, rev1 ? hist1 : nullptr);
        else if (pk)
            k_part_scatter1<true, false, false, kL1Items, true><<<xcd_grid(nt1, c->xcd_map), kPThreads, 0, c->stream>>>(
                cols.key, cols.lt, cols.rank, cols.val, tm1, jb, c->d_misc, c->cap, shift1, c->p_toff.p, p1r,
                p1k, xper1, pf, rev1 ? hist1 : nullptr);
        else
            k_part_scatter1<false, false, false, kL1Items, true><<<xcd_grid(nt1, c->xcd_map), kPThreads, 0, c->stream>>>(
                cols.key, cols.lt, cols.rank, cols.val, tm1, jb, c->d_misc, c->cap, shift1, c->p_toff.p, p1r,
                p1k, xper1, pf, rev1 ? hist1 : nullptr);
        if (ph) ev_record(c, ev_window(1, true));
        if (c->place_timed && s0 == 0) HIPCHK(hipEventRecord(c->place_ev[1], c->stream));
        if (ph) ev_record(c, ev_window(2, false));
        TileMap tm2f{};
        uint32_t nt2f = 0;
        const uint32_t* h2f = nullptr;
        const uint32_t* t2f = nullptr;
        if (two) {
            HIPALLOC(c->p_l2map.ensure(2 * (kDigits + 1)));
            HIPALLOC(c->p_dstart2.ensure(kDigits * kDigits + 1));
            HIPALLOC(c->p2_rec.ensure(rec_units)); HIPALLOC(c->p2_kj.ensure(kj2_units));
            p2r = c->p2_rec.p;
            p2k = c->p2_kj.p;
            uint32_t* tb2 = c->p_l2map.p;
            uint32_t* cb2 = c->p_l2map.p + kDigits + 1;
            const uint32_t ts2 = k16 && !(c->form_off & kFormNoHistW) && !(c->form_off & kFormBigTile2)
                                 ? (uint32_t)kPTile2 : (uint32_t)kPTile;
            if (fl) {
                HIPALLOC(c->f_hist2.ensure((size_t)nt2 * kDigits));
                HIPALLOC(c->f_toff2.ensure((size_t)nt2 * kDigits));
            }
            uint32_t* h2p = fl ? c->f_hist2.p : c->p_hist.p;
            uint32_t* t2p = fl ? c->f_toff2.p : c->p_toff.p;
            h2f = h2p;
            t2f = t2p;
            k_l2_plan<<<1, 256, 0, c->stream>>>(c->p_l1beg.p, tb2, cb2, ts2);
            k_seg_index<<<std::min<uint32_t>(grid_for(nt2, 256), 4096), 256, 0, c->stream>>>(tb2, kDigits, nt2,
                                                                                            c->p_tseg.p);
            const TileMap tm2{c->p_l1beg.p, c->p_l1beg.p + 1, tb2, c->p_tseg.p, nullptr, kDigits, ts2};
            tm2f = tm2;
            nt2f = (uint32_t)((nw + ts2 - 1) / ts2) + kDigits;
            const ScanMap sm2{tb2, cb2, c->p_l1beg.p, kDigits};
            if (cmp)
                k_part_hist16w<256, kPTile2, true><<<nt2, 256, 0, c->stream>>>(
                    reinterpret_cast<const uint16_t*>(p1k), tm2, 0, h2p);
            else if (k16 && !(c->form_off & kFormNoHistW) && ts2 == (uint32_t)kPTile2)
                k_part_hist16w<256, kPTile2><<<nt2, 256, 0, c->stream>>>(
                    reinterpret_cast<const uint16_t*>(p1k), tm2, kSBits - 4, h2p);
            else if (k16 && !(c->form_off & kFormNoHistW))
                k_part_hist16w<<<nt2, kHThreads, 0, c->stream>>>(
                    reinterpret_cast<const uint16_t*>(p1k), tm2, kSBits - 4, h2p);
            else if (k16)
                k_part_hist<false, true><<<nt2, kHThreads, 0, c->stream>>>(p1k, tm2, 0, c->d_misc, c->cap,
                                                                          kSBits - 4, h2p);
            else
                k_part_hist<false><<<nt2, kHThreads, 0, c->stream>>>(p1k, tm2, 0, c->d_misc, c->cap, kSBits,
                                                                      h2p);
            k_scan_part<<<nc2, 256, 0, c->stream>>>(h2p, sm2, c->p_part.p);
            k_scan_seg<<<kDigits, 256, 0, c->stream>>>(c->p_part.p, sm2, c->p_choff.p, c->p_dstart2.p, nullptr);
            k_scan_tiles<<<nc2, 256, 0, c->stream>>>(h2p, c->p_choff.p, sm2, c->p_dstart2.p, t2p);
            if (hotp) k_hot_starts<<<1, 256, 0, c->stream>>>(c->p_dstart2.p, c->p_dstarth.p, hb);
            const uint64_t nw2 = hotp ? nw - hot_n : nw;
            const uint32_t nt2s = (uint32_t)((nw2 + ts2 - 1) / ts2) + kDigits;
            const uint32_t xper2 = c->xcd_map ? (nt2s + kXcds - 1) / kXcds : 0;
            if (ord) {
                if (fl) HIPALLOC(c->f_pos2.ensure(nw + 8));
                uint16_t* pos2 = fl ? c->f_pos2.p : nullptr;
                const Rec12* i12 = reinterpret_cast<const Rec12*>(p1r);
                Rec12* o12 = reinterpret_cast<Rec12*>(p2r);
                const uint32_t jm = (uint32_t)pack_jmask(pf);
                if (cmp)
                    k_part_scatter2_seg<true, true, true><<<xcd_grid(nt2s, c->xcd_map), kPThreads, 0, c->stream>>>(
                        i12, nullptr, tm2, 24, t2p, o12, nullptr, xper2, jm, pos2, h2p);
                else if (k16)
                    k_part_scatter2_seg<true, true><<<xcd_grid(nt2s, c->xcd_map), kPThreads, 0, c->stream>>>(
                        i12, p1k, tm2, kSBits - 4, t2p, o12, p2k, xper2, jm, pos2, h2p);
                else if (k8)
                    k_part_scatter2_seg<true, false><<<xcd_grid(nt2s, c->xcd_map), kPThreads, 0, c->stream>>>(
                        i12, p1k, tm2, kSBits, t2p, o12, p2k, xper2, jm, pos2, h2p);
                else
                    k_part_scatter2_seg<false, false><<<xcd_grid(nt2s, c->xcd_map), kPThreads, 0, c->stream>>>(
                        i12, p1k, tm2, kSBits, t2p, o12, p2k, xper2, jm, pos2, h2p);
            } else if (c->counts)
                k_part_scatter2<true, false><<<xcd_grid(nt2s, c->xcd_map), kPThreads, 0, c->stream>>>(
                    p1r, p1k, tm2, kSBits, t2p, p2r, p2k, xper2, rev1 ? h2p : nullptr);
            else if (pk)
                if (cmp)
                    k_part_scatter2<false, true, true, true, true, true>
                        <<<xcd_grid(nt2s, c->xcd_map), kPThreads, 0, c->stream>>>(
                        p1r, nullptr, tm2, 24, t2p, p2r, nullptr, xper2, rev1 ? h2p : nullptr);
                else if (k16)
                    k_part_scatter2<false, true, true, true><<<xcd_grid(nt2s, c->xcd_map), kPThreads, 0, c->stream>>>(
                        p1r, p1k, tm2, kSBits - 4, t2p, p2r, p2k, xper2, rev1 ? h2p : nullptr);
                else if (k8)
                    k_part_scatter2<false, true, true><<<xcd_grid(nt2s, c->xcd_map), kPThreads, 0, c->stream>>>(
                        p1r, p1k, tm2, kSBits, t2p, p2r, p2k, xper2, rev1 ? h2p : nullptr);
                else
                    k_part_scatter2<false, true><<<xcd_grid(nt2s, c->xcd_map), kPThreads, 0, c->stream>>>(
                        p1r, p1k, tm2, kSBits, t2p, p2r, p2k, xper2, rev1 ? h2p : nullptr);
            else
                k_part_scatter2<false, false><<<xcd_grid(nt2s, c->xcd_map), kPThreads, 0, c->stream>>>(
                    p1r, p1k, tm2, kSBits, t2p, p2r, p2k, xper2, rev1 ? h2p : nullptr);
        }
        if (ph) ev_record(c, ev_window(2, true));
        const uint32_t nb = two ? kDigits * kDigits : kDigits;
        const uint32_t* bst = two ? c->p_dstart2.p : c->p_dstart1.p;
        const u32x4* rec = two ? p2r : p1r;
        const uint32_t* rv = two ? p2k : p1k;
        const uint32_t max_items = nb + (uint32_t)(nw / kRPart) + 1;
        const size_t ksn = (size_t)(2 * (nw / kRPart) + 2) * kSKeys;
        const uint32_t max_hot = std::min<uint32_t>(nb, (uint32_t)(nw / kRPart) + 1);
        HIPALLOC(c->p_ibase.ensure(2 * (nb + 1) + 1 + max_hot));
        HIPALLOC(c->p_kslt.ensure(2 * ksn));
        HIPALLOC(c->p_ksu32.ensure(6 * ksn));
        uint32_t* d_ib = c->p_ibase.p;
        uint32_t* d_hb = c->p_ibase.p + nb + 1;
        uint32_t* d_hot = c->p_ibase.p + 2 * (nb + 1);
        KeyState ps{c->p_kslt.p, c->p_ksu32.p, c->p_ksu32.p + ksn, c->p_ksu32.p + 2 * ksn};
        KeyState cy{c->p_kslt.p + ksn, c->p_ksu32.p + 3 * ksn, c->p_ksu32.p + 4 * ksn, c->p_ksu32.p + 5 * ksn};
        HIPALLOC(c->p_ibucket.ensure(max_items));
        const bool ov = !em && pk && (ord || !c->counts) && two && (c->form_off & kFormOverlap);
        if (ph) ev_record(c, ev_window(3, false));
        if (em) HIPALLOC(c->e_bbase.ensure(nb));
        k_bucket_items<<<(nb + 1023) / 1024, 1024, 0, c->stream>>>(bst, nb, d_ib, d_hb, d_hot, c->d_misc,
                                                                    em ? c->e_bbase.p : nullptr);
        k_seg_index<<<std::min<uint32_t>(grid_for(max_items, 256), 4096), 256, 0, c->stream>>>(d_ib, nb, max_items,
                                                                                               c->p_ibucket.p);
        auto item_lists = [&](uint64_t hw_s, uint32_t sparse_s, uint32_t* n_fold, uint32_t* n_dense, uint32_t* n_sparse,
                              uint32_t* n_hot, uint32_t* n_items) -> int {
            HIPALLOC(c->p_ilist.ensure(kListHead + 3 * (size_t)max_items));
            HIPALLOC(c->h_ilist.ensure(kListHead));
            k_item_lists<<<(nb + 1023) / 1024, 1024, 0, c->stream>>>(bst, nb, d_ib, d_hb, d_hot, hw_s, sparse_s,
                                                                    c->p_ilist.p, max_items);
            HIPCHK(hipMemcpyAsync(c->h_ilist.p, c->p_ilist.p, kListHead * sizeof(uint32_t), hipMemcpyDeviceToHost,
                                  c->stream));
            HIPCHK(hipStreamSynchronize(c->stream));
            const uint32_t* h = c->h_ilist.p;
            if (h[0] > max_items || h[1] > max_items || h[2] > max_items || h[3] > max_hot || h[4] > max_items)
                return CRDT_E_HIP;
            *n_fold = h[0]; *n_dense = h[1]; *n_sparse = h[2]; *n_hot = h[3]; *n_items = h[4];
            return CRDT_OK;
        };
        if (em) {
            const uint32_t n_items = max_items + max_hot * (kSKeys / 256);
            const size_t slots = (size_t)std::min<uint64_t>(nw, (uint64_t)nb * kSKeys) + 1;
            HIPALLOC(c->e_key.ensure(slots));
            HIPALLOC(c->e_pk.ensure(slots));
            HIPALLOC(c->e_val.ensure(slots));
            HIPALLOC(c->e_icnt.ensure((size_t)n_items * (2 + emit->G)));
            HIPCHK(hipMemsetAsync(c->e_icnt.p, 0, (size_t)n_items * (2 + emit->G) * sizeof(uint32_t), c->stream));
            emit->key = c->e_key.p;
            emit->pk = c->e_pk.p;
            emit->val = c->e_val.p;
            emit->bbase = c->e_bbase.p;
            emit->icount = c->e_icnt.p;
            emit->ibase = c->e_icnt.p + n_items;
            emit->ocount = c->e_icnt.p + 2 * (size_t)n_items;
            emit->item0 = max_items;
            emit->n_items = n_items;
            uint64_t* ps_key = reinterpret_cast<uint64_t*>(c->p_kslt.p);
            uint32_t* ps_val = c->p_ksu32.p;
            const Rec12* rec12 = reinterpret_cast<const Rec12*>(rec);
            if (k8) {
                k_resolve_packed<true, true, true><<<max_items, kQThreads, 0, c->stream>>>(
                    bst, d_ib, d_hb, c->p_ibucket.p, nb, rec12, rv, c->table, c->cap, 0, c->d_Rj.p, jb, ps_key, ps_val,
                    pf, c->d_misc);
                k_resolve_packed<false, false, true, true><<<max_items, kQThreads, 0, c->stream>>>(
                    bst, d_ib, d_hb, c->p_ibucket.p, nb, rec12, rv, c->table, c->cap, 0, c->d_Rj.p, jb, ps_key, ps_val,
                    pf, c->d_misc, *emit);
            } else {
                k_resolve_packed<true><<<max_items, kQThreads, 0, c->stream>>>(
                    bst, d_ib, d_hb, c->p_ibucket.p, nb, rec12, rv, c->table, c->cap, 0, c->d_Rj.p, jb, ps_key, ps_val,
                    pf, c->d_misc);
                k_resolve_packed<false, false, false, true><<<max_items, kQThreads, 0, c->stream>>>(
                    bst, d_ib, d_hb, c->p_ibucket.p, nb, rec12, rv, c->table, c->cap, 0, c->d_Rj.p, jb, ps_key, ps_val,
                    pf, c->d_misc, *emit);
            }
            k_part_carry_packed<true><<<dim3(kSKeys / 256, max_hot), 256, 0, c->stream>>>(
                d_hot, d_ib, d_hb, c->table, c->cap, 0, ps_key, ps_val, c->d_Rj.p, jb, pf, c->d_misc, *emit);
        } else if (ord) {
            uint64_t* ps_key = reinterpret_cast<uint64_t*>(c->p_kslt.p);
            uint32_t* ps_val = c->p_ksu32.p;
            const Rec12* rec12 = reinterpret_cast<const Rec12*>(rec);
            HIPALLOC(c->f_cin_key.ensure(ksn));
            HIPALLOC(c->f_cin_val.ensure(ksn));
            HIPALLOC(c->f_cin_pres.ensure(ksn));
            if (fl) HIPALLOC(c->f_flag2.ensure(nw + 8));
            uint8_t* fl2 = fl ? c->f_flag2.p : nullptr;
            int st = CRDT_OK;
            uint32_t g_fold = max_items, g_hot = max_hot, g_items = max_items, g_d, g_s;
            const uint32_t* l_fold = nullptr;
            if (!c->has_comm && !(c->form_off & kFormNoItemLists)) {
                if ((st = item_lists(0, 0, &g_fold, &g_d, &g_s, &g_hot, &g_items))) return st;
                l_fold = c->p_ilist.p + kListHead;
            }
            if ((st = ov ? overlap_fork(c) : CRDT_OK)) return st;
            const hipStream_t fs = ov ? c->sstream : c->stream;
            if (!g_fold) {
            } else if (cmp)
                k_resolve_packed<true, true, false, false, true><<<g_fold, kQThreads, 0, fs>>>(
                    bst, d_ib, d_hb, c->p_ibucket.p, nb, rec12, nullptr, c->table, c->cap, c->hw_read, c->d_Rj.p, jb,
                    ps_key, ps_val, pf, c->d_misc, EmitOut{}, 0, false, l_fold);
            else if (k8)
                k_resolve_packed<true, true, true><<<g_fold, kQThreads, 0, fs>>>(
                    bst, d_ib, d_hb, c->p_ibucket.p, nb, rec12, rv, c->table, c->cap, c->hw_read, c->d_Rj.p, jb, ps_key,
                    ps_val, pf, c->d_misc, EmitOut{}, 0, false, l_fold);
            else
                k_resolve_packed<true><<<g_fold, kQThreads, 0, fs>>>(
                    bst, d_ib, d_hb, c->p_ibucket.p, nb, rec12, rv, c->table, c->cap, c->hw_read, c->d_Rj.p, jb, ps_key,
                    ps_val, pf, c->d_misc, EmitOut{}, 0, false, l_fold);
            if (g_hot)
                k_part_cin_packed<<<dim3(kSKeys / 256, g_hot), 256, 0, fs>>>(
                    d_hot, d_ib, d_hb, c->table, c->cap, c->hw_read, ps_key, ps_val, pf, c->d_misc,
                    reinterpret_cast<uint64_t*>(c->f_cin_key.p), c->f_cin_val.p, c->f_cin_pres.p);
            const uint64_t* cink = reinterpret_cast<const uint64_t*>(c->f_cin_key.p);
            for (uint32_t which = ov ? 1u : 0u; which <= (ov ? 2u : 0u); ++which) {
                if (which == 2 && (st = overlap_join(c))) return st;
                if (!g_items) {
                } else if (cmp)
                    k_resolve_pflags<false, true><<<g_items, kRThreads, 0, c->stream>>>(
                        bst, d_ib, d_hb, c->p_ibucket.p, nb, rec12, nullptr, c->table, c->cap, c->hw_read, c->d_Rj.p,
                        jb, cink, c->f_cin_val.p, c->f_cin_pres.p, pf, c->d_misc, fl2, which);
                else if (k8)
                    k_resolve_pflags<true><<<g_items, kRThreads, 0, c->stream>>>(
                        bst, d_ib, d_hb, c->p_ibucket.p, nb, rec12, rv, c->table, c->cap, c->hw_read, c->d_Rj.p, jb,
                        cink, c->f_cin_val.p, c->f_cin_pres.p, pf, c->d_misc, fl2, which);
                else
                    k_resolve_pflags<false><<<g_items, kRThreads, 0, c->stream>>>(
                        bst, d_ib, d_hb, c->p_ibucket.p, nb, rec12, rv, c->table, c->cap, c->hw_read, c->d_Rj.p, jb,
                        cink, c->f_cin_val.p, c->f_cin_pres.p, pf, c->d_misc, fl2, which);
            }
            const uint8_t* f1 = c->f_flag2.p;
            if (fl && two) {
                HIPALLOC(c->f_flag1.ensure(nw + 8));
                const bool fx = c->xcd_map && (c->form_off & kFormFbackXcd);
                const uint32_t xf2 = fx ? (nt2f + kXcds - 1) / kXcds : 0;
#define CRDT_FBACK2(CHK, W)                                                                               \
    if (tm2f.tsize == (uint32_t)kPTile2)                                                                  \
        k_flags_back<false, CHK, kPTile2, W><<<xcd_grid(nt2f, fx), 512, 0, c->stream>>>(                  \
            tm2f, h2f, t2f, c->f_pos2.p, c->f_flag2.p, c->f_flag1.p, c->d_misc, xf2);                     \
    else                                                                                                  \
        k_flags_back<false, CHK, kPTile, W><<<xcd_grid(nt2f, fx), 512, 0, c->stream>>>(                   \
            tm2f, h2f, t2f, c->f_pos2.p, c->f_flag2.p, c->f_flag1.p, c->d_misc, xf2)
                const bool pre2 = !(c->form_off & (kFormNoFbackPre | kFormFbackWide)) && !fx &&
                                  tm2f.tsize == (uint32_t)kPTile2;
                if (pre2 && (c->form_off & kFormFbackPre512))
                    k_flags_back_pre<false, 6, kPTile2, 16><<<nt2f, 512, 0, c->stream>>>(
                        tm2f, h2f, t2f, c->f_pos2.p, c->f_flag2.p, c->f_flag1.p, c->d_misc);
                else if (pre2)
                    k_flags_back_pre<false, 6, kPTile2, 32, 256><<<nt2f, 256, 0, c->stream>>>(
                        tm2f, h2f, t2f, c->f_pos2.p, c->f_flag2.p, c->f_flag1.p, c->d_misc);
                else if (c->form_off & kFormFbackWide) { CRDT_FBACK2(6, true); }
                else if (c->fback_chk == 4) { CRDT_FBACK2(4, false); }
                else if (c->fback_chk == 6) { CRDT_FBACK2(6, false); }
                else { CRDT_FBACK2(0, false); }
#undef CRDT_FBACK2
                f1 = c->f_flag1.p;
                k_seg_index<<<std::min<uint32_t>(grid_for(nt1, 256), 4096), 256, 0, c->stream>>>(d_tb1, nseg, nt1,
                                                                                                 c->p_tseg.p);
            }
            const bool fx1 = c->xcd_map && (c->form_off & kFormFbackXcd);
            const uint32_t xf1 = fx1 ? (nt1 + kXcds - 1) / kXcds : 0;
#define CRDT_FBACK1(CHK, W)                                                                               \
    k_flags_back<true, CHK, kPTile, W><<<xcd_grid(nt1, fx1), 512, 0, c->stream>>>(                        \
        tm1, hist1, c->p_toff.p, c->f_pos1.p, f1, dflags, c->d_misc, xf1)
            if (fl) {
                if (pt1)
                    k_flags_back_pre<true, 6, kPTile, 14, 512, true><<<nt1, 512, 0, c->stream>>>(
                        tm1, hist1, c->p_toff.p, c->f_pos1.p, f1, dflags, c->d_misc);
                else if (!(c->form_off & (kFormNoFbackPre | kFormFbackWide)) && !fx1)
                    k_flags_back_pre<true, 6, kPTile, 14><<<nt1, 512, 0, c->stream>>>(
                        tm1, hist1, c->p_toff.p, c->f_pos1.p, f1, dflags, c->d_misc);
                else if (c->form_off & kFormFbackWide) { CRDT_FBACK1(6, true); }
                else if (c->fback_chk == 4) { CRDT_FBACK1(4, false); }
                else if (c->fback_chk == 6) { CRDT_FBACK1(6, false); }
                else { CRDT_FBACK1(0, false); }
            }
#undef CRDT_FBACK1
        } else if (c->counts) {
            k_resolve<true><<<max_items, kRThreads, 0, c->stream>>>(bst, d_ib, d_hb, c->p_ibucket.p, nb, rec, rv,
                                                                    c->table, c->cap, c->d_Rj.p, jb, ps, cy, c->d_misc);
            k_part_carry<false><<<dim3(kSKeys / 256, max_hot), 256, 0, c->stream>>>(d_hot, d_ib, d_hb, c->table,
                                                                                    c->cap, ps, cy, c->d_Rj.p, jb, c->d_misc);
            k_resolve<false><<<max_items, kRThreads, 0, c->stream>>>(bst, d_ib, d_hb, c->p_ibucket.p, nb, rec, rv,
                                                                     c->table, c->cap, c->d_Rj.p, jb, ps, cy, c->d_misc);
        } else if (pk) {
            uint64_t* ps_key = reinterpret_cast<uint64_t*>(c->p_kslt.p);
            uint32_t* ps_val = c->p_ksu32.p;
            const Rec12* rec12 = reinterpret_cast<const Rec12*>(rec);
            const bool spk = c->sparse_t > 0 && !(c->form_off & (kFormNoSparseK | kFormNoWholeLines));
            int st = CRDT_OK;
            const bool lists = !c->has_comm && !(c->form_off & (kFormNoItemLists | kFormNoWholeLines));
            uint32_t g_fold = max_items, g_dense = max_items, g_sparse = max_items, g_hot = max_hot;
            const uint32_t *l_fold = nullptr, *l_dense = nullptr, *l_sparse = nullptr;
            if (lists) {
                uint32_t g_items;
                if ((st = item_lists(spk ? c->hw_read : 0, spk ? c->sparse_t : 0, &g_fold, &g_dense, &g_sparse, &g_hot,
                                     &g_items)))
                    return st;
                l_fold = c->p_ilist.p + kListHead;
                l_dense = l_fold + max_items;
                l_sparse = l_dense + max_items;
            }
            if ((st = ov ? overlap_fork(c) : CRDT_OK)) return st;
            const hipStream_t fs = ov ? c->sstream : c->stream;
            if (g_fold) {
                if (cmp)
                    k_resolve_packed<true, true, false, false, true><<<g_fold, kQThreads, 0, fs>>>(
                        bst, d_ib, d_hb, c->p_ibucket.p, nb, rec12, nullptr, c->table, c->cap, c->hw_read, c->d_Rj.p, jb,
                        ps_key, ps_val, pf, c->d_misc, EmitOut{}, 0, false, l_fold);
                else if (k8)
                    k_resolve_packed<true, true, true><<<g_fold, kQThreads, 0, fs>>>(
                        bst, d_ib, d_hb, c->p_ibucket.p, nb, rec12, rv, c->table, c->cap, c->hw_read, c->d_Rj.p, jb, ps_key,
                        ps_val, pf, c->d_misc, EmitOut{}, 0, false, l_fold);
                else
                    k_resolve_packed<true><<<g_fold, kQThreads, 0, fs>>>(
                        bst, d_ib, d_hb, c->p_ibucket.p, nb, rec12, rv, c->table, c->cap, c->hw_read, c->d_Rj.p, jb, ps_key,
                        ps_val, pf, c->d_misc, EmitOut{}, 0, false, l_fold);
            }
            if (g_hot)
                k_part_carry_packed<false><<<dim3(kSKeys / 256, g_hot), 256, 0, fs>>>(
                    d_hot, d_ib, d_hb, c->table, c->cap, c->hw_read, ps_key, ps_val, c->d_Rj.p, jb, pf, c->d_misc);
            if (!g_dense) {
            } else if (cmp)
                k_resolve_packed<false, true, false, false, true><<<g_dense, kQThreads, 0, c->stream>>>(
                    bst, d_ib, d_hb, c->p_ibucket.p, nb, rec12, nullptr, c->table, c->cap, c->hw_read, c->d_Rj.p, jb,
                    ps_key, ps_val, pf, c->d_misc, EmitOut{}, c->sparse_t, spk, l_dense);
            else if ((c->form_off & kFormNoWholeLines) && k8)
                k_resolve_packed<false, false, true><<<max_items, kQThreads, 0, c->stream>>>(
                    bst, d_ib, d_hb, c->p_ibucket.p, nb, rec12, rv, c->table, c->cap, c->hw_read, c->d_Rj.p, jb, ps_key, ps_val,
                    pf, c->d_misc);
            else if (c->form_off & kFormNoWholeLines)
                k_resolve_packed<false, false><<<max_items, kQThreads, 0, c->stream>>>(
                    bst, d_ib, d_hb, c->p_ibucket.p, nb, rec12, rv, c->table, c->cap, c->hw_read, c->d_Rj.p, jb, ps_key, ps_val,
                    pf, c->d_misc);
            else if (k8)
                k_resolve_packed<false, true, true><<<g_dense, kQThreads, 0, c->stream>>>(
                    bst, d_ib, d_hb, c->p_ibucket.p, nb, rec12, rv, c->table, c->cap, c->hw_read, c->d_Rj.p, jb, ps_key, ps_val,
                    pf, c->d_misc, EmitOut{}, c->sparse_t, spk, l_dense);
            else
                k_resolve_packed<false><<<g_dense, kQThreads, 0, c->stream>>>(
                    bst, d_ib, d_hb, c->p_ibucket.p, nb, rec12, rv, c->table, c->cap, c->hw_read, c->d_Rj.p, jb, ps_key, ps_val,
                    pf, c->d_misc, EmitOut{}, c->sparse_t, spk, l_dense);
            if (!spk || !g_sparse) {
            } else if (cmp)
                k_resolve_sparse<false, true><<<g_sparse, kSpThreads, 0, c->stream>>>(
                    bst, d_ib, c->p_ibucket.p, nb, rec12, nullptr, c->table, c->hw_read, c->d_Rj.p, jb, pf, c->d_misc,
                    c->sparse_t, l_sparse);
            else if (k8)
                k_resolve_sparse<true, false><<<g_sparse, kSpThreads, 0, c->stream>>>(
                    bst, d_ib, c->p_ibucket.p, nb, rec12, rv, c->table, c->hw_read, c->d_Rj.p, jb, pf, c->d_misc,
                    c->sparse_t, l_sparse);
            else
                k_resolve_sparse<false, false><<<g_sparse, kSpThreads, 0, c->stream>>>(
                    bst, d_ib, c->p_ibucket.p, nb, rec12, rv, c->table, c->hw_read, c->d_Rj.p, jb, pf, c->d_misc,
                    c->sparse_t, l_sparse);
            if (ov && (st = overlap_join(c))) return st;
        } else {
            k_resolve<true, true><<<max_items, kRThreads, 0, c->stream>>>(bst, d_ib, d_hb, c->p_ibucket.p, nb, rec,
                                                                          rv, c->table, c->cap, c->d_Rj.p, jb, ps, cy,
                                                                          c->d_misc);
            k_part_carry<true><<<dim3(kSKeys / 256, max_hot), 256, 0, c->stream>>>(d_hot, d_ib, d_hb, c->table,
                                                                                   c->cap, ps, cy, c->d_Rj.p, jb, c->d_misc);
            k_resolve<false, true><<<max_items, kRThreads, 0, c->stream>>>(bst, d_ib, d_hb, c->p_ibucket.p, nb, rec,
                                                                           rv, c->table, c->cap, c->d_Rj.p, jb, ps, cy,
                                                                           c->d_misc);
        }
        if (ph) {
            ev_record(c, ev_window(3, true));
            c->sorted_phases = true;
            c->p1_records = nw;
        }
        HIPCHK(hipGetLastError());
        c->hw_read = c->cap;
    }
    if (em) return CRDT_OK;
    if (c->timing) {
        ev_record(c, ev_window(0, true));
        c->windows.push_back(1u);
    }
    HIPCHK(hipGetLastError());
#ifdef CRDT_PROF_RESOLVE
    HIPCHK(hipStreamSynchronize(c->stream));
    prof_resolve_report();
#endif
    return finish_apply(c, nullptr, nullptr, 0, true, out);
}

bool use_sorted(const crdt_ctx* c, const Segs& sg, uint32_t R, const uint8_t* win_flags) {
    if (c->merge_path == 1 || c->canonical < 0 || c->cap > kSortedMaxCap) return false;
    if (win_flags && (!c->flags_sorted || !c->packed_resolve)) return false;
    uint64_t n = 0, nw = 0;
    uint32_t jb = 0;
    for (size_t s = 0; s < sg.j.size(); ++s) {
        if (sg.j[s] >= jb + kWindow) { jb = sg.j[s] - sg.j[s] % kWindow; nw = 0; }
        nw += sg.end[s] - sg.beg[s];
        n += sg.end[s] - sg.beg[s];
        if (nw >= (1ull << 31)) return false;
    }
    if (c->merge_path == 2) return true;
    return R >= 64 && n >= (8ull << 20) &&
           (win_flags || !c->counts || c->packed_resolve || n / R <= (256ull << 10));
}

int apply_segs(crdt_ctx* c, const Cols& cols, uint64_t n, int32_t mem, int64_t wall, const long long* d_event,
               uint8_t* win_flags, crdt_result* out, bool allow_sorted) {
    if (c->timing) HIPCHK(ensure_events(c, events_for(c->segs.j.size())));
    c->last_sorted = allow_sorted && use_sorted(c, c->segs, c->plan_R, win_flags);
    c->last_flagged = false;
    const uint64_t nrec = c->segs.j.empty() ? 0 : n;
    const bool big_cs = c->counts && c->merge_path != 2 && c->plan_R && nrec / c->plan_R > (256ull << 10);
    if (c->last_sorted && (win_flags || big_cs)) {
        bool ok = mem == CRDT_MEM_DEVICE && c->frame_on && !cols.packed_in;
        if (ok) {
            HIPCHK(hipMemcpyAsync(c->h_misc, c->d_misc, sizeof(Misc), hipMemcpyDeviceToHost, c->stream));
            SYNCHK(c, c->stream);
            ok = frame_of(c).ok;
        }
        c->last_sorted = ok;
    }
    if (c->last_sorted) {
        int st = kv_copy_all(c);
        if (st) return st;
        if (win_flags) {
            if (n) HIPCHK(hipMemsetAsync(win_flags, 0, n, c->stream));
            c->last_flagged = true;
        }
        return apply_sorted(c, cols, c->segs, wall, d_event, out, win_flags);
    }
    return apply_ranges(c, cols, c->segs, n, mem, wall, d_event, win_flags, out);
}

int phase_apply(crdt_ctx* c, const crdt_batch* owned, int64_t wall, const long long* d_event,
                uint8_t* win_flags, crdt_result* out, bool allow_sorted = false) {
    int st = validate_batch(owned);
    if (st) return st;
    const uint32_t R = c->plan_R;
    if (owned->n_changesets != R) return CRDT_E_INVALID;
    Cols cols;
    if ((st = stage_apply_cols(c, owned, &cols))) return st;
    c->segs.from_offsets(owned->offsets, R);
    return apply_segs(c, cols, owned->offsets[R], owned->mem, wall, d_event, win_flags, out, allow_sorted);
}

void place_finish(crdt_ctx* c, bool ok) {
    if (c->place_warm) {
        c->place_warm = false;
        if (ok) c->place_trial = 0;
        return;
    }
    if (!c->place_timed) return;
    c->place_timed = false;
// ... 17 lines not shown
    if (c->timing) {
        float ms = 0;
        auto el = [&](size_t a, size_t b) {
            return hipEventElapsedTime(&ms, c->events[a], c->events[b]) == hipSuccess ? (double)ms : 0.0;
        };
        t.scan_ms = el(kEvStart, kEvScan);
        t.clock_ms = el(kEvScan, kEvClock);
        t.route_ms = el(kEvClock, kEvApply);
        for (size_t k = 0; k < c->windows.size(); ++k) {
            t.apply_ms += el(ev_window(k, false), ev_window(k, true));
            t.apply_launches += c->windows[k];
        }
        t.apply_total = c->apply_total;
        t.total_ms = el(kEvStart, kEvEnd);
        if (c->last_sorted && c->sorted_phases) {
            t.part1_ms = el(ev_window(1, false), ev_window(1, true));
            t.part2_ms = el(ev_window(2, false), ev_window(2, true));
            t.resolve_ms = el(ev_window(3, false), ev_window(3, true));
            t.part1_records = c->p1_records;
        }
    }
    t.sent_bytes = c->sent_bytes;
    c->last_timing = t;
}

#include "comm_path.inc"

}

extern "C" {

int crdt_abi_version(void) { return CRDT_ABI_VERSION; }

const char* crdt_status_string(int s) {
    switch (s) {
        case CRDT_OK: return "ok";
        case CRDT_CLOCK_DRIFT: return "clock drift";
        case CRDT_DUPLICATE_NODE: return "duplicate node";
        case CRDT_OVERFLOW: return "counter overflow";
        case CRDT_E_INVALID: return "invalid argument";
        case CRDT_E_HIP: return "HIP runtime error";
        case CRDT_E_NOMEM: return "device out of memory";
        case CRDT_E_KEY_RANGE: return "key id out of range";
        case CRDT_E_NO_DEVICE: return "no gfx950 device";
        case CRDT_E_COMM: return "communicator error";
        default: return "unknown status";
    }
}

int crdt_device_count(int* out) {
    if (!out) return CRDT_E_INVALID;
    int n = 0;
    if (hipGetDeviceCount(&n) != hipSuccess) n = 0;
    *out = n;
    return CRDT_OK;
}

static void read_env_knobs(crdt_ctx* c) {
    if (const char* e = getenv("CRDT_NO_FUSE")) c->no_fuse = atoi(e) != 0;
    if (const char* e = getenv("CRDT_XCD_MAP")) c->xcd_map = atoi(e) != 0;
    if (const char* e = getenv("CRDT_PACKED")) c->packed_resolve = atoi(e) != 0;
    if (const char* e = getenv("CRDT_FLAGS_SORTED")) c->flags_sorted = atoi(e) != 0;
    if (const char* e = getenv("CRDT_TABLE_MERGE")) c->table_merge = atoi(e) != 0;
    if (const char* e = getenv("CRDT_COMBINE")) c->combine = std::min(std::max(atoi(e), 0), 2);
    if (const char* e = getenv("CRDT_ROUTE_L1")) c->route_l1 = std::min(std::max(atoi(e), 0), 3);
    if (const char* e = getenv("CRDT_RL1_SPLIT")) {
        const int v = atoi(e);
        c->rl1_pieces = std::min<uint32_t>(v <= 0 ? 1u : v == 1 ? 2u : (uint32_t)v, kRl1MaxPieces);
    }
    if (const char* e = getenv("CRDT_ROUTE_TUNE")) c->route_tune = atoi(e) != 0;
    if (const char* e = getenv("CRDT_SPARSE_T")) c->sparse_t = (uint32_t)std::max(atoi(e), 0);
    if (const char* e = getenv("CRDT_HOT_BUCKETS")) c->hot_buckets = (uint32_t)std::min(std::max(atoi(e), 0), (int)kHotMax);
    if (const char* e = getenv("CRDT_HOT_PROBE")) c->hot_probe = (uint32_t)std::min(std::max(atoi(e), 0), 1 << 20);
    if (const char* e = getenv("CRDT_HOT_SHARE")) c->hot_share = (uint32_t)std::min(std::max(atoi(e), 0), 100);
    if (const char* e = getenv("CRDT_FBACK_CHK")) c->fback_chk = atoi(e) == 4 ? 4 : atoi(e) == 0 ? 0 : 6;
    if (const char* e = getenv("CRDT_HIST_FUSE")) c->hist_fuse = atoi(e) != 0;
    if (const char* e = getenv("CRDT_L1_TILE"))
        c->l1_tile = std::min<uint32_t>((uint32_t)std::max(atoi(e), 0) / 1024u * 1024u, (uint32_t)kPTile);
    if (const char* e = getenv("CRDT_SORTED_FORM")) c->form_off = (uint32_t)strtoul(e, nullptr, 10);
    if (const char* e = getenv("CRDT_APPLY_ITEMS")) {
        const int v = atoi(e);
        c->apply_items = (v == 1 || v == 2 || v == 4 || v == 8) ? v : 0;
    }
    c->fail_rank = -1;
    c->fail_at = 0;
    if (const char* e = getenv("CRDT_TEST_FAIL")) {
        int r = -1, at = 0;
        if (sscanf(e, "%d:%d", &r, &at) == 2) { c->fail_rank = r; c->fail_at = at; }
    }
    c->stall_rank = -1;
    c->stall_at = c->stall_ms = 0;
    c->stall_dev = false;
    if (const char* e = getenv("CRDT_TEST_STALL")) {
        int r = -1, at = 0, ms = 0;
        char d = 0;
        const int k = sscanf(e, "%d:%d:%d:%c", &r, &at, &ms, &d);
        if (k >= 3) { c->stall_rank = r; c->stall_at = at; c->stall_ms = ms; c->stall_dev = k == 4 && d == 'd'; }
    }
}

int crdt_create(int device, uint32_t local_rank, uint64_t capacity, crdt_ctx** out) {
    if (!out) return CRDT_E_INVALID;
    *out = nullptr;
    int n = 0;
    if (hipGetDeviceCount(&n) != hipSuccess || device < 0 || device >= n) return CRDT_E_NO_DEVICE;
    hipDeviceProp_t prop;
    if (hipGetDeviceProperties(&prop, device) != hipSuccess) return CRDT_E_NO_DEVICE;
    if (strncmp(prop.gcnArchName, "gfx950", 6) != 0) return CRDT_E_NO_DEVICE;
    HIPCHK(hipSetDevice(device));
    crdt_ctx* c = new (std::nothrow) crdt_ctx();
    if (!c) return CRDT_E_NOMEM;
    c->device = device;
    c->local_rank = local_rank;
    if (const char* e = getenv("CRDT_MERGE_PATH")) {
        c->merge_path = strcmp(e, "gather") == 0 ? 1 : strcmp(e, "sorted") == 0 ? 2 : 0;
    }
    read_env_knobs(c);
    if (const char* e = getenv("CRDT_ENV_DYNAMIC")) c->env_dynamic = atoi(e) != 0;
    if (const char* e = getenv("CRDT_COMM_TIMEOUT_MS")) c->comm_timeout_ms = (uint32_t)std::max(atoll(e), 0ll);
    if (const char* e = getenv("CRDT_KV_WINDOW")) {
        const long long v = atoll(e);
        if (v > 0) c->kv_window = (uint64_t)v;
    }
    if (hipStreamCreateWithFlags(&c->stream, hipStreamNonBlocking) != hipSuccess ||
        hipMalloc(&c->d_misc, sizeof(Misc)) != hipSuccess ||
        hipHostMalloc(&c->h_misc, sizeof(Misc), hipHostMallocDefault) != hipSuccess ||
        c->d_M.ensure(1024) != hipSuccess || c->d_event.ensure(8) != hipSuccess ||
        c->d_word.ensure(4) != hipSuccess) {
        crdt_destroy(c);
        return CRDT_E_HIP;
    }
    int st = crdt_reserve(c, capacity);
    if (st) { crdt_destroy(c); return st; }
    *out = c;
    return CRDT_OK;
}

void crdt_destroy(crdt_ctx* c) {
    if (!c) return;
    hipSetDevice(c->device);
    if (c->stream) hipStreamSynchronize(c->stream);
    comm_release(c);
    for (auto* b : {&c->r_skey, &c->r_srank, &c->r_sval, &c->r_key, &c->r_rank, &c->r_val}) b->release();
    c->r_slt.release(); c->r_lt.release(); c->r_perm.release(); c->r_flags.release(); c->r_sflags.release();
    c->d_gsend.release(); c->d_grecv.release(); c->d_pbase.release(); c->d_sum.release(); c->d_tune.release(); c->h_tune.release();
    c->d_rcnt.release(); c->d_rrecv.release(); c->h_rcnt.release(); c->h_stage.release(); c->h_sum.release();
    c->d_rcur.release(); c->d_agree.release(); c->h_agree.release(); c->d_rl1cnt.release(); c->h_rl1cnt.release();
    if (c->route_ev) hipEventDestroy(c->route_ev);
    for (hipEvent_t e : c->rl_evs) if (e) hipEventDestroy(e);
    for (hipEvent_t e : c->rl_evx) if (e) hipEventDestroy(e);
    if (c->rl_evo) hipEventDestroy(c->rl_evo);
    if (c->rl_evh) hipEventDestroy(c->rl_evh);
    for (hipEvent_t e : c->ov_ev) if (e) hipEventDestroy(e);
    if (c->sstream) hipStreamDestroy(c->sstream);
    if (c->ostream) hipStreamDestroy(c->ostream);
    if (c->table.base) hipFree(c->table.base);
    if (c->d_misc) hipFree(c->d_misc);
    if (c->h_misc) hipHostFree(c->h_misc);
    c->d_M.release(); c->d_event.release(); c->d_plan.release();
    c->h_plan.release();
    c->d_T.release(); c->d_Cprev.release(); c->d_Rj.release(); c->d_Cj.release();
    c->d_candP.release(); c->d_candms.release(); c->d_candtile.release(); c->d_candkind.release();
    c->d_candkey.release();
    c->s_key.release(); c->s_rank.release(); c->s_val.release(); c->s_lt.release();
    c->s_millis.release(); c->s_mod.release(); c->s_flags.release(); c->s_out.release();
    c->x_key.release(); c->x_rank.release(); c->x_val.release(); c->x_lt.release(); c->x_mod.release();
    c->x_counts.release(); c->x_offs.release(); c->x_words.release();
    c->t_sel.release(); c->t_words.release(); c->t_mask.release(); c->t_wflags.release();
    c->t_fstep.release(); c->t_fmask.release(); c->t_fcounts.release();
    c->d_word.release();
    c->d_ibase.release();
    c->p1_rec.release(); c->p1_kj.release(); c->p2_rec.release(); c->p2_kj.release();
    for (int i = 0; i < crdt_ctx::kPlaceMax; ++i) { c->pc_rec[i].release(); c->pc_kj[i].release(); }
    for (hipEvent_t e : c->place_ev) if (e) hipEventDestroy(e);
    c->p_hist1h.release(); c->p_toffh.release(); c->p_dstarth.release(); c->p_l1begh.release();
    c->p_hist.release(); c->p_hist1.release(); c->p_toff.release(); c->p_part.release(); c->p_choff.release();
    c->p_dstart1.release(); c->p_dstart2.release(); c->p_l2map.release();
    c->p_plan.release(); c->p_l1beg.release(); c->h_pplan.release();
    c->p_ibase.release(); c->p_ksu32.release(); c->p_kslt.release(); c->p_tseg.release();
    c->p_ibucket.release(); c->p_ilist.release(); c->h_ilist.release();
    c->f_pos1.release(); c->f_pos2.release(); c->f_flag1.release(); c->f_flag2.release();
    c->f_cin_key.release(); c->f_cin_val.release(); c->f_cin_pres.release();
    c->f_hist2.release(); c->f_toff2.release();
    c->e_key.release(); c->e_val.release(); c->e_pk.release(); c->e_cnt.release(); c->e_cur.release();
    c->e_icnt.release(); c->e_off.release(); c->e_csum.release(); c->e_bbase.release();
    c->h_ebase.release();
    c->rl_rec.release(); c->rl_k16.release(); for (Rl1Scratch& os : c->rl_os) os.release();
    c->rl_hf.release(); c->rl_hrec.release(); c->rl_hk16.release(); c->rl_hcnt.release(); c->h_hcnt.release();
    for (hipEvent_t e : c->events) hipEventDestroy(e);
    for (hipEvent_t e : c->cevents) hipEventDestroy(e);
    if (c->cstream) hipStreamDestroy(c->cstream);
    if (c->stream) hipStreamDestroy(c->stream);
    delete c;
}

int crdt_reserve(crdt_ctx* c, uint64_t capacity) {
    if (!c) return CRDT_E_INVALID;
    if (capacity <= c->cap && c->table.base) return CRDT_OK;
    if (capacity > (1ull << 32)) return CRDT_E_INVALID;
    HIPCHK(hipSetDevice(c->device));
    const uint64_t newcap = std::max<uint64_t>(capacity, 16);
    const uint64_t rb = c->table.stride;
    Table t{nullptr, c->table.stride};
    HIPALLOC(hipMalloc(&t.base, newcap * rb));
    if (c->table.base && c->cap)
        HIPCHK(hipMemcpyAsync(t.base, c->table.base, c->cap * rb, hipMemcpyDeviceToDevice, c->stream));
    HIPCHK(hipMemsetAsync(t.base + c->cap * rb, 0x80, (newcap - c->cap) * rb, c->stream));
    HIPCHK(hipStreamSynchronize(c->stream));
    if (c->table.base) hipFree(c->table.base);
    c->table = t;
    c->cap = newcap;
    return CRDT_OK;
}

int crdt_set_row_bytes(crdt_ctx* c, uint32_t row_bytes) {
    if (!c || (row_bytes != 24 && row_bytes != 32)) return CRDT_E_INVALID;
    if (row_bytes == c->table.stride) return CRDT_OK;
    HIPCHK(hipSetDevice(c->device));
    Table t{nullptr, row_bytes};
    HIPALLOC(hipMalloc(&t.base, c->cap * (uint64_t)row_bytes));
    if (c->cap) {
        k_relayout<<<std::min<uint32_t>(grid_for(c->cap, 256), 65536), 256, 0, c->stream>>>(c->table, t, c->cap);
        HIPCHK(hipGetLastError());
    }
    HIPCHK(hipStreamSynchronize(c->stream));
    hipFree(c->table.base);
    c->table = t;
    return CRDT_OK;
}

int crdt_reserve_scratch(crdt_ctx* c, uint64_t n_records) {
    if (!c) return CRDT_E_INVALID;
    if (n_records == 0) return CRDT_OK;
    HIPCHK(hipSetDevice(c->device));
    HIPALLOC(c->p1_rec.ensure((3 * n_records + 3) / 4 + kPartPad));
    HIPALLOC(c->p1_kj.ensure((n_records + 1) / 2 + kPartPad));
    HIPALLOC(c->p2_rec.ensure((3 * n_records + 3) / 4 + kPartPad));
    HIPALLOC(c->p2_kj.ensure((n_records + 3) / 4 + kPartPad));
    int tries = 3;
    if (const char* e = getenv("CRDT_PLACE_TRIES")) tries = std::min(std::max(atoi(e), 1), crdt_ctx::kPlaceMax);
    if (c->has_comm) tries = 1;
    c->place_k = tries;
    c->place_idle = 0;
    c->place_trial = tries > 1 ? -1 : 0;
    c->place_best = tries > 1 ? -1 : 0;
    return CRDT_OK;
}



int crdt_capacity(const crdt_ctx* c, uint64_t* out) {
    if (!c || !out) return CRDT_E_INVALID;
    *out = c->cap;
    return CRDT_OK;
}

int crdt_set_local_rank(crdt_ctx* c, uint32_t rank) {
    if (!c) return CRDT_E_INVALID;
    c->local_rank = rank;
    return CRDT_OK;
}

int crdt_get_canonical(const crdt_ctx* c, int64_t* lt) {
    if (!c || !lt) return CRDT_E_INVALID;
    *lt = c->canonical;
    return CRDT_OK;
}

int crdt_set_canonical(crdt_ctx* c, int64_t lt) {
    if (!c) return CRDT_E_INVALID;
    c->canonical = lt;
    return CRDT_OK;
}

int crdt_put_rows(crdt_ctx* c, const uint32_t* key_id, const int64_t* lt, const uint32_t* rank,
                  const uint32_t* val, const int64_t* mod, uint64_t n, int32_t mem) {
    if (!c) return CRDT_E_INVALID;
    if (n == 0) return CRDT_OK;
    if (!key_id || !lt || !rank || !val || !mod) return CRDT_E_INVALID;
    HIPCHK(hipSetDevice(c->device));
    const uint32_t *dk, *dr, *dv;
    const int64_t *dl, *dm;
    int st;
    if ((st = stage(c, c->s_key, key_id, n, mem, &dk))) return st;
    if ((st = stage(c, c->s_lt, lt, n, mem, &dl))) return st;
    if ((st = stage(c, c->s_rank, rank, n, mem, &dr))) return st;
    if ((st = stage(c, c->s_val, val, n, mem, &dv))) return st;
    if ((st = stage(c, c->s_mod, mod, n, mem, &dm))) return st;
    if ((st = reset_misc(c))) return st;
    k_put_rows<<<std::min<uint32_t>(grid_for(n, 256), kPutGrid), 256, 0, c->stream>>>(dk, dl, dr, dv, dm, n,
                                                                                     c->table, c->cap, c->d_misc);
    HIPCHK(hipGetLastError());
    HIPCHK(hipMemcpyAsync(c->h_misc, c->d_misc, sizeof(Misc), hipMemcpyDeviceToHost, c->stream));
    HIPCHK(hipStreamSynchronize(c->stream));
    raise_hw(c, c->h_misc->key_end);
    return c->h_misc->err ? CRDT_E_KEY_RANGE : CRDT_OK;
}

int crdt_put_stamped(crdt_ctx* c, const uint32_t* key_id, const uint32_t* val, uint64_t n, int64_t wall,
                     int32_t mem, crdt_result* out) {
    if (!c) return CRDT_E_INVALID;
    crdt_result res = cleared_result(c->canonical);
    if (n == 0) { if (out) *out = res; return CRDT_OK; }
    if (!key_id || !val) return CRDT_E_INVALID;
    const HlcSend send = hlc_send(c->canonical, wall);
    if (send.status != CRDT_OK) {
        send.into(res);
        if (out) *out = res;
        return res.status;
    }
    const int64_t stamp = send.canonical;
    HIPCHK(hipSetDevice(c->device));
    const uint32_t *dk, *dv;
    int st;
    if ((st = stage(c, c->s_key, key_id, n, mem, &dk))) return st;
    if ((st = stage(c, c->s_val, val, n, mem, &dv))) return st;
    if ((st = reset_misc(c))) return st;
    k_key_check<<<std::min<uint32_t>(grid_for(n, 256 * 16), 8192), 256, 0, c->stream>>>(dk, n, c->cap, c->d_misc);
    k_put_stamped<<<std::min<uint32_t>(grid_for(n, 256), kPutGrid), 256, 0, c->stream>>>(
        dk, dv, n, stamp, c->local_rank, c->table, c->cap, c->d_misc);
    HIPCHK(hipGetLastError());
    HIPCHK(hipMemcpyAsync(c->h_misc, c->d_misc, sizeof(Misc), hipMemcpyDeviceToHost, c->stream));
    HIPCHK(hipStreamSynchronize(c->stream));
    raise_hw(c, c->h_misc->key_end);
    if (c->h_misc->err) return CRDT_E_KEY_RANGE;
    c->canonical = stamp;
    res.canonical_lt = stamp;
    res.n_won = n;
    if (out) *out = res;
    return CRDT_OK;
}

// ... 722 lines not shown
    for (uint32_t j = 0; j < n_dst; ++j) {
        st = crdt_merge_table(dsts[j], src, n_rows, since[j], wall, step, CRDT_MEM_DEVICE, &out[j]);
        if (st >= 0 && win_mask && n_rows) {
            k_fan_or_flags<<<std::min<uint32_t>(grid_for(n_rows, 256), 8192), 256, 0, d0->stream>>>(step, n_rows, j, wm);
            HIPCHK(hipGetLastError());
            HIPCHK(hipStreamSynchronize(d0->stream));
        }
        if (st != 0) {
            for (uint32_t k = j + 1; k < n_dst; ++k) out[k] = cleared_result(dsts[k]->canonical);
            break;
        }
    }
    if (win_mask && n_rows) {
        if (mask_mem == CRDT_MEM_HOST)
            HIPCHK(hipMemcpyAsync(win_mask, wm, n_rows, hipMemcpyDeviceToHost, d0->stream));
        HIPCHK(hipStreamSynchronize(d0->stream));
    }
    return st;
}

int crdt_fanout_tables(crdt_ctx* src, crdt_ctx* const* dsts, const int64_t* since_lt, uint32_t n_dst,
                       uint64_t n_rows, int64_t wall, uint8_t* win_mask, int32_t mask_mem, crdt_result* out) {
    if (!src || !dsts || !since_lt || !out || n_dst == 0 || n_dst > CRDT_FANOUT_MAX) return CRDT_E_INVALID;
    for (uint32_t j = 0; j < n_dst; ++j)
        if (!dsts[j]) return CRDT_E_INVALID;
    for (uint32_t j = 0; j < n_dst; ++j)
        if (!tm_args_ok(dsts[j], src, win_mask != nullptr, mask_mem)) return CRDT_E_INVALID;
    if (n_rows > src->cap) return CRDT_E_INVALID;
    if (n_dst == 1) return crdt_merge_table(dsts[0], src, n_rows, since_lt[0], wall, win_mask, mask_mem, out);
    crdt_ctx* d0 = dsts[0];
    HIPCHK(hipSetDevice(d0->device));
    bool composed = false;
    for (uint32_t j = 0; j < n_dst; ++j) {
        crdt_ctx* d = dsts[j];
        if (d->env_dynamic) read_env_knobs(d);
        composed |= !d->table_merge || d == src || d->merge_path == CRDT_PATH_SORTED;
        for (uint32_t k = 0; k < j; ++k) composed |= dsts[k] == d;
    }
    if (composed) return fanout_tables_composed(src, dsts, since_lt, n_dst, n_rows, wall, win_mask, mask_mem, out);
    HIPCHK(hipStreamSynchronize(src->stream));
    for (uint32_t j = 1; j < n_dst; ++j) HIPCHK(hipStreamSynchronize(dsts[j]->stream));
    FoArgs fa{};
    uint64_t covered = 0;
    for (uint32_t j = 0; j < n_dst; ++j) {
        fa.dst[j] = dsts[j]->table;
        fa.rows[j] = ex_rows(src, n_rows, since_lt[j]);
        fa.cap[j] = dsts[j]->cap;
        fa.since[j] = since_lt[j];
        fa.canonical[j] = dsts[j]->canonical;
        fa.rank[j] = dsts[j]->local_rank;
        covered = std::max(covered, fa.rows[j]);
    }
    const unsigned nb = grid_for(covered, kTmTile);
    uint8_t* rf;
    int st;
    if ((st = tm_stage_flags(d0, win_mask, mask_mem, n_rows, &rf))) return st;
    if ((st = tm_begin(d0, nb, (int)n_dst))) return st;
    if (covered) {
        k_fo_clock<<<std::min(nb, kFoClockGrid), kTmThreads, 0, d0->stream>>>(
            fa, n_dst, src->table, covered, nb, wall, d0->t_sel.p, d0->t_mask.p, d0->t_words.p);
        HIPCHK(hipGetLastError());
    }
    unsigned long long w[kFoMax * kTmWords] = {};
    if ((st = tm_read_words(d0, w, (int)n_dst))) return st;
    crdt_result res[kFoMax];
    bool has = false;
    for (uint32_t j = 0; j < n_dst; ++j) {
        const unsigned long long* wj = w + j * kTmWords;
        composed |= wj[2] || (wj[3] && wj[1] > dsts[j]->cap);
        has |= wj[3] != 0;
        fa.stamp[j] = tm_recv_canonical(fa.canonical[j], wj);
        res[j] = cleared_result(fa.canonical[j]);
        res[j].n_stored = 1;
        hlc_send(fa.stamp[j], wall).into(res[j]);
        composed |= res[j].status != CRDT_OK;
    }
    if (composed) return fanout_tables_composed(src, dsts, since_lt, n_dst, n_rows, wall, win_mask, mask_mem, out);
    ev_record(d0, kEvClock);
    HIPALLOC(d0->t_fcounts.ensure(kFanCounts));
    HIPCHK(hipMemsetAsync(d0->t_fcounts.p, 0, kFanCounts * sizeof(unsigned long long), d0->stream));
    if ((st = tm_zero_uncovered(d0, rf, has ? covered : 0, n_rows))) return st;
    tm_apply_begin(d0, has);
    if (has) {
        k_fo_apply<<<nb, kTmThreads, 0, d0->stream>>>(fa, n_dst, src->table, covered, nb, d0->t_sel.p, d0->t_mask.p,
                                                      d0->t_fcounts.p, rf);
        HIPCHK(hipGetLastError());
    }
    tm_apply_end(d0, has);
    if ((st = tm_flags_to_host(d0, win_mask, rf, mask_mem, n_rows))) return st;
    std::vector<unsigned long long> counts(kFanCounts);
    HIPCHK(hipMemcpyAsync(counts.data(), d0->t_fcounts.p, kFanCounts * sizeof(unsigned long long),
                          hipMemcpyDeviceToHost, d0->stream));
    HIPCHK(hipStreamSynchronize(d0->stream));
    for (uint32_t j = 0; j < n_dst; ++j) {
        const unsigned long long* cj = counts.data() + 2 * j * kCounterSlots;
        for (int s = 0; s < kCounterSlots; ++s) {
            res[j].n_present += cj[s];
            res[j].n_won += cj[kCounterSlots + s];
        }
        tm_finish(dsts[j], &res[j], d0->h_misc, 0, 0, w + j * kTmWords, false);
        dsts[j]->last_fanout = true;
        out[j] = res[j];
    }
    collect_timing(d0);
    return CRDT_OK;
}

int crdt_set_rank_bound(crdt_ctx* c, uint32_t bound) {
    if (!c) return CRDT_E_INVALID;
    c->rank_bound = bound;
    return CRDT_OK;
}

int crdt_set_counts(crdt_ctx* c, int exact) {
    if (!c || (exact != 0 && exact != 1)) return CRDT_E_INVALID;
    c->counts = exact != 0;
    return CRDT_OK;
}

int crdt_set_merge_path(crdt_ctx* c, int path) {
    if (!c || path < CRDT_PATH_AUTO || path > CRDT_PATH_SORTED) return CRDT_E_INVALID;
    c->merge_path = path;
    return CRDT_OK;
}

int crdt_last_path(const crdt_ctx* c, int* path) {
    if (!c || !path) return CRDT_E_INVALID;
    *path = c->last_sorted ? CRDT_PATH_SORTED : CRDT_PATH_GATHER;
    return CRDT_OK;
}

int crdt_last_plan(const crdt_ctx* c, uint32_t* flags) {
    if (!c || !flags) return CRDT_E_INVALID;
    uint32_t f = 0;
    if (c->last_table) {
        *flags = CRDT_PLAN_TABLE | (c->last_sync ? CRDT_PLAN_SYNC : 0u) | (c->last_fanin ? CRDT_PLAN_FANIN : 0u) |
                 (c->last_fanout ? CRDT_PLAN_FANOUT : 0u);
        return CRDT_OK;
    }
    if (c->last_sorted) {
        f |= CRDT_PLAN_SORTED;
        if (c->last_packed) f |= CRDT_PLAN_PACKED;
        if (c->cap > (1ull << 20)) f |= CRDT_PLAN_TWO_LEVEL;
        if (c->last_hist1_fused) f |= CRDT_PLAN_HIST_IN_SCAN;
        if (c->last_key8) f |= CRDT_PLAN_KEY8;
        if (c->last_key16) f |= CRDT_PLAN_KEY16;
        if (c->last_hw) f |= CRDT_PLAN_HIGH_WATER;
        if (c->last_flagged) f |= CRDT_PLAN_FLAGGED;
        if (c->last_ordered) f |= CRDT_PLAN_ORDERED;
        if (c->last_combined) f |= CRDT_PLAN_COMBINED;
        if (c->last_route_l1) f |= CRDT_PLAN_ROUTE_L1;
        if (c->last_compact) f |= CRDT_PLAN_COMPACT;
        if (c->last_hot_direct) f |= CRDT_PLAN_HOT_DIRECT;
    }
    if (c->last_wire_pk) f |= CRDT_PLAN_WIRE_PACKED;
    if (c->last_own_in_place) f |= CRDT_PLAN_OWN_IN_PLACE;
    if (c->tune_trial) f |= CRDT_PLAN_ROUTE_TUNED;
    if (c->last_route_l1) f |= (c->last_rl1_pieces & 7u) << CRDT_PLAN_RL1_PIECES_SHIFT;
    if (c->last_route_l1 && c->last_rl1_head) f |= CRDT_PLAN_RL1_HEAD;
    *flags = f;
    return CRDT_OK;
}

int crdt_place_info(const crdt_ctx* c, int32_t* n, int32_t* kept, int32_t* done, float* ms) {
    if (!c || !n || !kept || !done || !ms) return CRDT_E_INVALID;
    *n = c->place_k;
    *kept = c->place_best;
    *done = c->place_k > 1 ? c->place_trial + 1 : 0;
    for (int i = 0; i < crdt_ctx::kPlaceMax; ++i) ms[i] = i < c->place_k ? c->place_ms[i] : 0.f;
    return CRDT_OK;
}

int crdt_route_tune_info(const crdt_ctx* c, int32_t* best, int64_t* us) {
    if (!c || !best || !us) return CRDT_E_INVALID;
    *best = c->rt.best;
    for (int w = 0; w < 5; ++w) us[w] = c->rt.us[w];
    return CRDT_OK;
}

int crdt_set_timing(crdt_ctx* c, int enable) {
    if (!c) return CRDT_E_INVALID;
    c->timing = enable != 0;
    return CRDT_OK;
}

int crdt_get_timing(const crdt_ctx* c, crdt_timing* out) {
    if (!c || !out) return CRDT_E_INVALID;
    *out = c->last_timing;
    return CRDT_OK;
}

}
```

crdt_amd/csrc/sorted_path.inc:

```

constexpr int kSBits = 12;
constexpr uint32_t kSKeys = 1u << kSBits;
constexpr uint32_t kDigits = 256;
constexpr int kJShift = 20;
constexpr uint32_t kKeyLoMask = (1u << kJShift) - 1;
constexpr uint32_t kWindow = 1u << (32 - kJShift);
constexpr int kHThreads = 1024;
constexpr int kPThreads = 1024;
constexpr int kPWaves = kPThreads / 64;
constexpr int kPItems = 4;
constexpr int kPSub = kPThreads * kPItems;
constexpr int kPTile = 28672;
constexpr int kPTile2 = 8192;
constexpr int kPGroups = kPItems * kPWaves;
#ifndef CRDT_FREE_ITEMS
#define CRDT_FREE_ITEMS 7
#endif
#ifndef CRDT_L1_ITEMS
#define CRDT_L1_ITEMS 7
#endif
constexpr int kFreeItems = CRDT_FREE_ITEMS;
constexpr int kL1Items = CRDT_L1_ITEMS;
constexpr int kPLanes = kPThreads / 256;
static_assert(kPGroups / kPLanes == 16, "group scan: 16 groups per lane");
// ... 15 lines not shown
    uint32_t tsize;
    uint32_t tile0 = 0;
};

struct ScanMap {
    const uint32_t* tbase;
    const uint32_t* cbase;
    const uint64_t* seg_pos;
    uint32_t nseg;
};

__device__ inline uint32_t seg_of(const uint32_t* base, uint32_t n, uint32_t x) {
    uint32_t lo = 0, hi = n;
    while (hi - lo > 1) {
        const uint32_t mid = (lo + hi) >> 1;
        if (base[mid] <= x) lo = mid; else hi = mid;
    }
    return lo;
}

__global__ __launch_bounds__(256) void k_seg_index(const uint32_t* __restrict__ base, uint32_t n, uint32_t max_x,
                                                   uint32_t* __restrict__ idx)
{
    const uint32_t total = std::min<uint32_t>(base[n], max_x);
    for (uint32_t x = blockIdx.x * 256 + threadIdx.x; x < total; x += gridDim.x * 256) idx[x] = seg_of(base, n, x);
}

__device__ inline void tile_info(const TileMap& m, uint32_t t, uint32_t* seg, uint64_t* beg, uint32_t* len) {
    const uint32_t s = m.tile_seg[t];
    const uint64_t b = m.seg_beg[s] + (uint64_t)(t - m.tbase[s]) * m.tsize;
    const uint64_t e = m.seg_end[s];
    *seg = s;
    *beg = b;
    *len = (uint32_t)(e > b ? std::min<uint64_t>(m.tsize, e - b) : 0);
}

constexpr uint32_t kXcds = 8;
__device__ inline uint32_t xcd_tile(uint32_t i, uint32_t per, bool on) {
    return on ? (i % kXcds) * per + i / kXcds : i;
}
inline uint32_t xcd_grid(uint32_t n, bool on) { return on ? ((n + kXcds - 1) / kXcds) * kXcds : n; }

__device__ inline unsigned long long match_digit(uint32_t d, bool active) {
    unsigned long long m = __ballot(active);
#pragma unroll
    for (int b = 0; b < 8; ++b) {
        const bool bit = (d >> b) & 1u;
        const unsigned long long bb = __ballot(active && bit);
        m &= bit ? bb : ~bb;
    }
    return m;
}

__device__ inline uint32_t scan256_excl(uint32_t v, uint32_t* s_w , uint32_t* total) {
    const int tid = threadIdx.x, lane = tid & 63, w = tid >> 6;
    uint32_t inc = v;
#pragma unroll
    for (int off = 1; off < 64; off <<= 1) {
        const uint32_t u = __shfl_up(inc, off, 64);
        if (lane >= off) inc += u;
    }
    if (tid < 256 && lane == 63) s_w[w] = inc;
    __syncthreads();
    uint32_t wp = 0;
    for (int k = 0; k < w && k < 4; ++k) wp += s_w[k];
    *total = s_w[0] + s_w[1] + s_w[2] + s_w[3];
    return wp + inc - v;
}


template <bool kLevel1, bool k16 = false>
__global__ __launch_bounds__(kHThreads) void k_part_hist(
    const void* __restrict__ keyw, TileMap tm, uint32_t jbase, const Misc* __restrict__ misc,
    uint64_t cap, uint32_t shift, uint32_t* __restrict__ hist, KeyMap km = KeyMap{0u, 8u})
{
    constexpr int kQ = kPTile / kHThreads;
    __shared__ uint32_t h[kDigits];
    const uint32_t t = blockIdx.x;
    if (t >= tm.tbase[tm.nseg]) return;
    uint32_t seg, len;
    uint64_t beg;
    tile_info(tm, t, &seg, &beg, &len);
    if (kLevel1 && misc && tm.seg_j[seg] >= misc->stop) len = 0;
    const int tid = threadIdx.x, lane = tid & 63;
    if (tid < (int)kDigits) h[tid] = 0;
    uint32_t k[kQ];
#pragma unroll
    for (int q = 0; q < kQ; ++q) {
        const uint32_t i = q * kHThreads + tid;
        k[q] = i >= len ? 0u
             : k16 ? (uint32_t)__builtin_nontemporal_load(static_cast<const uint16_t*>(keyw) + beg + i)
                   : __builtin_nontemporal_load(static_cast<const uint32_t*>(keyw) + beg + i);
    }
    __syncthreads();
#pragma unroll
    for (int q = 0; q < kQ; ++q) {
        const uint32_t i = q * kHThreads + tid;
        const bool act = i < len && (!kLevel1 || (k[q] >> km.gsh) < cap);
        const uint32_t d = kLevel1 ? km_digit(km, k[q], shift) : (k[q] >> shift) & (kDigits - 1);
        digit_count(h, d, act, lane);
    }
    __syncthreads();
    if (tid < (int)kDigits) hist[(uint64_t)t * kDigits + tid] = h[tid];
}

template <int kT = kHThreads, int kTile = kPTile, bool kD8 = false>
__global__ __launch_bounds__(kT) void k_part_hist16w(
    const uint16_t* __restrict__ key16, TileMap tm, uint32_t shift, uint32_t* __restrict__ hist)
{
    constexpr uint32_t kE = kD8 ? 16u : 8u, kEsh = kD8 ? 4u : 3u;
    constexpr int kWv = kT / 64;
    __shared__ uint32_t hw[kWv][kDigits];
    const uint32_t t = blockIdx.x;
    if (t >= tm.tbase[tm.nseg]) return;
    uint32_t seg, len;
    uint64_t beg;
    tile_info(tm, t, &seg, &beg, &len);
    const int tid = threadIdx.x, w = tid >> 6;
    for (int i = tid; i < kWv * (int)kDigits; i += kT) (&hw[0][0])[i] = 0;
    const uint64_t end = beg + len;
    const uint64_t b0 = beg >> kEsh, nblk = len ? ((end + kE - 1) >> kEsh) - b0 : 0;
    constexpr int kB = ((int)(kTile / kE) + 1 + kT - 1) / kT;
    u32x4 v[kB];
#pragma unroll
    for (int q = 0; q < kB; ++q) {
        const uint64_t b = (uint64_t)q * kT + tid;
        v[q] = b < nblk ? __builtin_nontemporal_load(reinterpret_cast<const u32x4*>(key16) + b0 + b)
                        : u32x4{0u, 0u, 0u, 0u};
    }
    __syncthreads();
#pragma unroll
    for (int q = 0; q < kB; ++q) {
        const uint64_t b = (uint64_t)q * kT + tid;
        if (b >= nblk) continue;
        const uint64_t e0 = (b0 + b) << kEsh;
        const uint32_t wd[4] = {v[q].x, v[q].y, v[q].z, v[q].w};
#pragma unroll
        for (int x = 0; x < (int)kE; ++x) {
            const uint64_t e = e0 + x;
            const uint32_t k = kD8 ? (wd[x >> 2] >> ((x & 3) * 8)) & 0xFFu : (wd[x >> 1] >> ((x & 1) * 16)) & 0xFFFFu;
            if (e >= beg && e < end) atomicAdd(&hw[w][kD8 ? k : (k >> shift) & (kDigits - 1)], 1u);
        }
    }
    __syncthreads();
    for (int d = tid; d < (int)kDigits; d += kT) {
        uint32_t s = 0;
#pragma unroll
        for (int x = 0; x < kWv; ++x) s += hw[x][d];
        hist[(uint64_t)t * kDigits + d] = s;
    }
}

__global__ __launch_bounds__(256) void k_hist_trim(uint32_t* __restrict__ hist, const uint32_t* __restrict__ ptb,
                                                   uint32_t R, const Misc* __restrict__ misc)
{
    const uint32_t stop = misc->stop;
    if (stop >= R) return;
    const uint64_t a = (uint64_t)ptb[stop] * kDigits, b = (uint64_t)ptb[R] * kDigits;
    for (uint64_t x = a + (uint64_t)blockIdx.x * 256 + threadIdx.x; x < b; x += (uint64_t)gridDim.x * 256)
        hist[x] = 0;
}
__global__ __launch_bounds__(64) void k_hot_fold(uint32_t* __restrict__ hist, const uint32_t* __restrict__ hhist,
                                                 uint32_t tiles)
{
    for (uint32_t t = blockIdx.x; t < tiles; t += gridDim.x) {
        const uint32_t* h = hhist + (uint64_t)t * kDigits;
        uint32_t s = h[threadIdx.x] + h[64 + threadIdx.x] + h[128 + threadIdx.x] + h[192 + threadIdx.x];
#pragma unroll
        for (int off = 32; off > 0; off >>= 1) s += __shfl_xor(s, off, 64);
        if (threadIdx.x == 0) hist[(uint64_t)t * kDigits] += s;
    }
}

__global__ __launch_bounds__(256) void k_hot_starts(uint32_t* __restrict__ bstart, const uint32_t* __restrict__ hstart,
                                                    uint32_t hot)
{
    if (threadIdx.x < hot) bstart[threadIdx.x] = hstart[threadIdx.x];
}
static_assert(kHotShift == (uint32_t)kSBits && kHotMax == kDigits, "a hot bin is a final bucket of level-1 digit 0");
static_assert(kPTile == (int)kHistSub * kTile && (kPTile / 2) % 1024 == 0,
              "the largest level-1 tile is kHistSub scan tiles; half of it splits on the scan's 1024-record groups");
static_assert(kDigits == 256, "k_scan<.., kHist> counts 256 digits");

__global__ __launch_bounds__(256) void k_scan_part(const uint32_t* __restrict__ hist, ScanMap sm,
                                                   uint32_t* __restrict__ part)
{
    const uint32_t c = blockIdx.x;
    if (c >= sm.cbase[sm.nseg]) return;
    const uint32_t s = seg_of(sm.cbase, sm.nseg, c);
    const uint32_t t0 = sm.tbase[s] + (c - sm.cbase[s]) * kChunkTiles;
    const uint32_t t1 = std::min<uint32_t>(t0 + kChunkTiles, sm.tbase[s + 1]);
    const uint32_t d = threadIdx.x;
    uint32_t sum = 0;
#pragma unroll 8
    for (uint32_t t = t0; t < t1; ++t) sum += hist[(uint64_t)t * kDigits + d];
    part[(uint64_t)c * kDigits + d] = sum;
}

__global__ __launch_bounds__(256) void k_scan_seg(const uint32_t* __restrict__ part, ScanMap sm,
                                                  uint32_t* __restrict__ choff, uint32_t* __restrict__ dstart,
                                                  uint64_t* __restrict__ dstart64)
{
    __shared__ uint32_t s_w[4];
    const uint32_t s = blockIdx.x, d = threadIdx.x;
    const uint32_t c0 = sm.cbase[s], c1 = sm.cbase[s + 1];
    uint32_t run = 0;
#pragma unroll 8
    for (uint32_t c = c0; c < c1; ++c) {
        const uint32_t v = part[(uint64_t)c * kDigits + d];
        choff[(uint64_t)c * kDigits + d] = run;
        run += v;
    }
    uint32_t total;
    const uint32_t ex = scan256_excl(run, s_w, &total);
    const uint64_t pos = sm.seg_pos[s] + ex;
    dstart[(uint64_t)s * kDigits + d] = (uint32_t)pos;
    if (dstart64) {
        dstart64[(uint64_t)s * kDigits + d] = pos;
        if (s + 1 == sm.nseg && d == kDigits - 1) dstart64[(uint64_t)sm.nseg * kDigits] = sm.seg_pos[s] + total;
    }
    if (s + 1 == sm.nseg && d == kDigits - 1) dstart[(uint64_t)sm.nseg * kDigits] = (uint32_t)(sm.seg_pos[s] + total);
}

__global__ __launch_bounds__(256) void k_scan_tiles(const uint32_t* __restrict__ hist,
                                                    const uint32_t* __restrict__ choff, ScanMap sm,
                                                    const uint32_t* __restrict__ dstart,
                                                    uint32_t* __restrict__ toff)
{
    const uint32_t c = blockIdx.x;
    if (c >= sm.cbase[sm.nseg]) return;
    const uint32_t s = seg_of(sm.cbase, sm.nseg, c);
    const uint32_t t0 = sm.tbase[s] + (c - sm.cbase[s]) * kChunkTiles;
    const uint32_t t1 = std::min<uint32_t>(t0 + kChunkTiles, sm.tbase[s + 1]);
    const uint32_t d = threadIdx.x;
    uint32_t run = dstart[(uint64_t)s * kDigits + d] + choff[(uint64_t)c * kDigits + d];
    for (uint32_t t = t0; t < t1; t += 8) {
        uint32_t h[8];
#pragma unroll
        for (uint32_t u = 0; u < 8; ++u) h[u] = t + u < t1 ? hist[(uint64_t)(t + u) * kDigits + d] : 0u;
#pragma unroll
        for (uint32_t u = 0; u < 8; ++u) {
            if (t + u < t1) toff[(uint64_t)(t + u) * kDigits + d] = run;
            run += h[u];
        }
    }
}

__global__ __launch_bounds__(256) void k_l2_plan(const uint64_t* __restrict__ l1_beg, uint32_t* __restrict__ tbase,
                                                 uint32_t* __restrict__ cbase, uint32_t tsize)
{
    __shared__ uint32_t s_w[4];
    const uint32_t s = threadIdx.x;
    const uint64_t n = l1_beg[s + 1] - l1_beg[s];
    const uint32_t nt = (uint32_t)((n + tsize - 1) / tsize);
    const uint32_t nc = (nt + kChunkTiles - 1) / kChunkTiles;
    uint32_t tt, tc;
    const uint32_t et = scan256_excl(nt, s_w, &tt);
    __syncthreads();
    const uint32_t ec = scan256_excl(nc, s_w, &tc);
    tbase[s] = et;
    cbase[s] = ec;
    if (s == 255) { tbase[256] = tt; cbase[256] = tc; }
}

struct PackFrame {
    int64_t lt0;
    uint64_t lt_span;
    uint32_t rk0, rk_span;
    uint32_t jb;
    uint32_t jwin;
    uint32_t sh;
    uint64_t rk_mask;
    uint32_t rk_limit;
    bool ok;
    bool key4;
    uint32_t cb;
    int64_t m0;
};

constexpr uint32_t kCKeyShift = 44;
constexpr uint64_t kCPkMask = (1ull << kCKeyShift) - 1;

__host__ __device__ inline uint64_t pack_ltf(const PackFrame& f, int64_t lt) {
    if (!f.cb) return (uint64_t)lt - (uint64_t)f.lt0;
    return ((uint64_t)((lt >> 16) - f.m0) << f.cb) | ((uint64_t)lt & 0xFFFFull);
}
__host__ __device__ inline int64_t pack_lt(const PackFrame& f, uint64_t x) {
    const uint64_t lf = x >> f.sh;
    if (!f.cb) return (int64_t)((uint64_t)f.lt0 + lf);
    return (int64_t)(((uint64_t)((int64_t)(lf >> f.cb) + f.m0) << 16) | (lf & ((1ull << f.cb) - 1)));
}

__host__ __device__ inline int bitlen64(uint64_t x) {
    int b = 0;
    while (b < 64 && (x >> b) != 0) ++b;
    return b;
}

__host__ __device__ inline bool frame_window(int L, int K, uint32_t R, uint32_t* jb, uint32_t* jwin) {
    const uint32_t want = R < 1u ? 1u : (R > kWindow ? kWindow : R);
    int J = bitlen64((uint64_t)want + 1);
    if (L + K + J > 64) {
        J = 64 - L - K;
        if (J < 10) return false;
    }
    *jb = (uint32_t)J;
    *jwin = std::min<uint32_t>(want, (1u << J) - 2);
    return true;
}

__host__ __device__ inline PackFrame make_frame(unsigned long long acc_lo, unsigned long long acc_hi,
                                                uint32_t acc_rlo, uint32_t acc_rhi, uint32_t R) {
    PackFrame f;
    f.rk_limit = UINT32_MAX;
    f.cb = 0;
    f.m0 = 0;
    f.jb = 13;
    f.jwin = kWindow;
    if (acc_lo == 0 && acc_hi == 0) {
        f.lt0 = 0; f.lt_span = 0; f.rk0 = 0; f.rk_span = 0; f.rk_mask = 1; f.key4 = true;
        f.ok = frame_window(0, 1, R, &f.jb, &f.jwin);
        f.sh = 1 + f.jb;
        return f;
    }
    f.lt0 = (int64_t)(~acc_lo ^ (1ull << 63));
    const uint64_t lt_max = acc_hi ^ (1ull << 63);
    f.lt_span = lt_max - (uint64_t)f.lt0;
    f.rk0 = ~acc_rlo;
    f.rk_span = acc_rhi - f.rk0;
    const int K = bitlen64((uint64_t)f.rk_span + 1), L = bitlen64(f.lt_span);
    f.rk_mask = K >= 64 ? ~0ull : (1ull << K) - 1;
    f.ok = L + K <= 54 && frame_window(L, K, R, &f.jb, &f.jwin);
    f.sh = (uint32_t)K + f.jb;
    f.key4 = f.ok && L + K + (int)f.jb <= 60;
    return f;
}

template <bool kCmp = false>
__host__ __device__ inline uint64_t pack_record(const PackFrame& f, int64_t lt, uint32_t rank, uint32_t jw) {
    const uint64_t lf = kCmp ? ((uint64_t)((lt >> 16) - f.m0) << f.cb) | ((uint64_t)lt & 0xFFFFull)
                             : (uint64_t)lt - (uint64_t)f.lt0;
    return (lf << f.sh) | ((uint64_t)(rank - f.rk0) << f.jb) | (uint64_t)(f.jwin - jw);
}

__host__ __device__ inline PackFrame compact_frame(PackFrame f, uint32_t cmax, uint32_t R) {
    if (!f.ok || cmax > 0xFFFDu) return f;
    const int64_t m0 = f.lt0 >> 16, m1 = (int64_t)((uint64_t)f.lt0 + f.lt_span) >> 16;
    const int cb = bitlen64((uint64_t)cmax + 1);
    const int L = bitlen64((uint64_t)(m1 - m0)) + cb, K = bitlen64((uint64_t)f.rk_span + 1);
    uint32_t jb, jwin;
    if (L + K > 54 || !frame_window(L, K, R, &jb, &jwin) || L + K + (int)jb > (int)kCKeyShift) return f;
    PackFrame c = f;
    c.cb = (uint32_t)cb;
    c.m0 = m0;
    c.jb = jb;
    c.jwin = jwin;
    c.sh = (uint32_t)K + jb;
    c.key4 = true;
    return c;
}
__host__ __device__ inline uint64_t pack_jmask(const PackFrame& f) { return (1ull << f.jb) - 1; }
__host__ __device__ inline uint32_t pack_jw(const PackFrame& f, uint64_t x) {
    return f.jwin - (uint32_t)(x & pack_jmask(f));
}
__host__ __device__ inline uint32_t pack_rank(const PackFrame& f, uint64_t x) {
    return f.rk0 + (uint32_t)((x >> f.jb) & f.rk_mask);
}

__device__ inline uint64_t pack_local(const PackFrame& f, bool present, int64_t lt, uint32_t rank) {
    if (!present || lt < f.lt0) return 0;
    if ((uint64_t)lt - (uint64_t)f.lt0 > f.lt_span) return UINT64_MAX;
    const uint64_t lo = (uint64_t)lt & 0xFFFFull, top = (1ull << f.cb) - 1;
    const uint64_t hi = (f.cb && lo > top ? pack_ltf(f, (int64_t)(((uint64_t)lt & ~0xFFFFull) | top))
                                          : pack_ltf(f, lt)) << f.sh;
    if (rank < f.rk0) return hi;
    if (rank - f.rk0 > f.rk_span) return hi | ((uint64_t)(f.rk_span + 1) << f.jb);
    return hi | ((uint64_t)(rank - f.rk0) << f.jb) | (uint64_t)(f.jwin + 1);
}

__device__ inline bool pack_is_record(const PackFrame& f, uint64_t st) {
    const uint32_t jf = (uint32_t)(st & pack_jmask(f));
    return st != UINT64_MAX && jf >= 1u && jf <= f.jwin;
}
// ... 2009 lines not shown
```

crdt_amd/device.py:

```python
from __future__ import annotations

import ctypes

import numpy as np

from . import _capi
from ._capi import CrdtBatch, CrdtResult, CrdtTiming


class CrdtNativeError(RuntimeError):
    def __init__(self, status: int, what: str = ""):
        self.status = status
        msg = _capi.status_string(status) if status else "ok"
        super().__init__(f"{what}: {msg} ({status})" if what else f"{msg} ({status})")


def _is_torch(a) -> bool:
    return type(a).__module__.startswith("torch")


_NP_TYPES = {"u4": np.uint32, "i8": np.int64, "u1": np.uint8}
_TORCH_KINDS = {"u4": ("int32", "uint32"), "i8": ("int64",), "u1": ("uint8", "bool")}


# ... 282 lines not shown
        if win_mask is True:
            mask_arr = mask_arr[:n_rows]
        return [res[j].as_dict() for j in range(n_src)], mask_arr

    def fanout_tables(self, dsts, n_rows: int, sinces, wall: int, win_mask=False):
        dsts, sinces = list(dsts), [int(s) for s in sinces]
        if len(sinces) != len(dsts):
            raise ValueError(f"fanout_tables: {len(dsts)} destinations but {len(sinces)} sinces")
        for d in dsts:
            if d.device != self.device:
                raise ValueError(f"fanout_tables: a destination table is on device {d.device}, this one on {self.device}")
        n_rows, n_dst = int(n_rows), len(dsts)
        mask_arr, mptr, mem = self._row_flags_arg(win_mask, n_rows)
        ctxs = (ctypes.c_void_p * max(n_dst, 1))(*(d._ctx.value for d in dsts))
        since_arr = (ctypes.c_int64 * max(n_dst, 1))(*sinces)
        res = (CrdtResult * max(n_dst, 1))()
        st = self._lib.crdt_fanout_tables(self._ctx, ctxs, since_arr, n_dst, n_rows, int(wall), mptr, mem, res)
        self._check(st, "crdt_fanout_tables")
        if win_mask is True:
            mask_arr = mask_arr[:n_rows]
        return [res[j].as_dict() for j in range(n_dst)], mask_arr

    def clear_rows(self, first: int, count: int):
        self._check(self._lib.crdt_clear_rows(self._ctx, first, count), "crdt_clear_rows")

    def remap_ranks(self, n_rows: int, old_to_new):
        lut = np.ascontiguousarray(old_to_new, dtype=np.uint32)
        self._check(self._lib.crdt_remap_ranks(self._ctx, n_rows, lut.ctypes.data_as(ctypes.c_void_p),
                                               len(lut)), "crdt_remap_ranks")

    def refresh_canonical(self, n_rows: int) -> int:
        v = ctypes.c_int64()
        self._check(self._lib.crdt_refresh_canonical(self._ctx, n_rows, ctypes.byref(v)),
                    "crdt_refresh_canonical")
        return v.value

    def put_stamped(self, key, val, wall: int) -> dict:
        c = _Cols(self.device, key=(key, "u4"), val=(val, "u4"))
        res = CrdtResult()
        self._check(self._lib.crdt_put_stamped(self._ctx, c.ptrs["key"], c.ptrs["val"], len(key), int(wall),
                                               c.mem, ctypes.byref(res)), "crdt_put_stamped")
        return res.as_dict()

    def _batch(self, key, lt, rank, val, offsets, millis):
        c = _Cols(self.device, key=(key, "u4"), lt=(lt, "i8"), rank=(rank, "u4"), val=(val, "u4"), millis=(millis, "i8"))
        offs = np.ascontiguousarray(offsets, dtype=np.uint64)
        c.keep.append(offs)
        b = CrdtBatch(c.ptrs["key"], c.ptrs["lt"], c.ptrs["rank"], c.ptrs["val"], c.ptrs["millis"],
                      offs.ctypes.data_as(ctypes.c_void_p), len(offs) - 1, c.mem)
        return b, c, offs

    def merge(self, key, lt, rank, val, offsets, wall: int, millis=None, win_flags=True):
        b, c, offs = self._batch(key, lt, rank, val, offsets, millis)
        dev = c.keep[0].device if c.mem == _capi.CRDT_MEM_DEVICE else None
        return self._merge_batch(b, int(offs[-1]), dev, wall, win_flags)

    def _merge_batch(self, b, n: int, torch_device, wall: int, win_flags):
        flags_arr = None
        fptr = None
        if win_flags is True:
            if torch_device is not None:
                import torch
                flags_arr = torch.zeros(max(n, 1), dtype=torch.uint8, device=torch_device)
                torch_ready(flags_arr)
                fptr = ctypes.c_void_p(flags_arr.data_ptr())
            else:
                flags_arr = np.zeros(max(n, 1), np.uint8)
                fptr = flags_arr.ctypes.data_as(ctypes.c_void_p)
        elif win_flags is not None and win_flags is not False:
            flags_arr = win_flags
            if _is_torch(win_flags):
                fptr = self._dptr(win_flags, "u1", "win_flags")
            else:
                if win_flags.dtype != np.uint8 or not win_flags.flags.c_contiguous or len(win_flags) < n:
                    raise ValueError("win_flags must be a contiguous uint8 array of one entry per record")
                fptr = win_flags.ctypes.data_as(ctypes.c_void_p)
        res = CrdtResult()
        st = self._lib.crdt_merge(self._ctx, ctypes.byref(b), int(wall), fptr, ctypes.byref(res))
        if st == _capi.CRDT_E_COMM and getattr(self, "_comm", None) is not None and self._comm.error is not None:
            raise CrdtNativeError(st, f"crdt_merge (communicator: {self._comm.error!r})")
        self._check(st, "crdt_merge")
        if flags_arr is not None and win_flags is True:
            flags_arr = flags_arr[:n]
        return res.as_dict(), flags_arr

    def comm_unique_id(self) -> bytes:
        buf = (ctypes.c_uint8 * _capi.COMM_ID_BYTES)()
        self._check(self._lib.crdt_comm_unique_id(buf), "crdt_comm_unique_id")
        return bytes(buf)

    def comm_init_rccl(self, n_ranks: int, rank: int, uid: bytes):
        buf = (ctypes.c_uint8 * _capi.COMM_ID_BYTES).from_buffer_copy(uid)
        self._check(self._lib.crdt_comm_init_rccl(self._ctx, n_ranks, rank, buf), "crdt_comm_init_rccl")

    def comm_init_ops(self, n_ranks: int, rank: int, comm):
        self._comm = comm
        ops = comm.ops()
        st = self._lib.crdt_comm_init_ops(self._ctx, n_ranks, rank, ctypes.byref(ops))
        self._check(st, "crdt_comm_init_ops")
        ms = getattr(self, "_comm_timeout_ms", None)
        if ms is not None and hasattr(comm, "timeout") and comm.timeout is None:
            comm.timeout = ms / 1e3 if ms else None

    def set_comm_timeout(self, ms: int):
        self._check(self._lib.crdt_set_comm_timeout(self._ctx, int(ms)), "crdt_set_comm_timeout")
        self._comm_timeout_ms = int(ms)
        comm = getattr(self, "_comm", None)
        if comm is not None and hasattr(comm, "timeout"):
            comm.timeout = ms / 1e3 if ms else None

    def comm_state(self) -> tuple[int, str]:
        st, ph = ctypes.c_int32(), ctypes.c_char_p()
        self._check(self._lib.crdt_comm_state(self._ctx, ctypes.byref(st), ctypes.byref(ph)), "crdt_comm_state")
        return st.value, (ph.value or b"").decode()

    def comm_info(self) -> tuple[int, int]:
        n, r = ctypes.c_uint32(), ctypes.c_uint32()
        self._check(self._lib.crdt_comm_info(self._ctx, ctypes.byref(n), ctypes.byref(r)), "crdt_comm_info")
        return n.value, r.value

    def comm_free(self):
        self._check(self._lib.crdt_comm_free(self._ctx), "crdt_comm_free")

    def set_presharded(self, on: bool):
        self._check(self._lib.crdt_set_presharded(self._ctx, 1 if on else 0), "crdt_set_presharded")

    PATHS = {"auto": 0, "gather": 1, "sorted": 2}

    def set_counts(self, exact: bool):
        self._check(self._lib.crdt_set_counts(self._ctx, 1 if exact else 0), "crdt_set_counts")

    def set_row_bytes(self, row_bytes: int):
        self._check(self._lib.crdt_set_row_bytes(self._ctx, int(row_bytes)), "crdt_set_row_bytes")

    def reserve_scratch(self, n_records: int):
        self._check(self._lib.crdt_reserve_scratch(self._ctx, int(n_records)), "crdt_reserve_scratch")

    def set_rank_bound(self, bound: int):
        self._check(self._lib.crdt_set_rank_bound(self._ctx, int(bound)), "crdt_set_rank_bound")

    def set_merge_path(self, path: str):
        self._check(self._lib.crdt_set_merge_path(self._ctx, self.PATHS[path]), "crdt_set_merge_path")

    def last_path(self) -> str:
        v = ctypes.c_int(0)
        self._check(self._lib.crdt_last_path(self._ctx, ctypes.byref(v)), "crdt_last_path")
        return {1: "gather", 2: "sorted"}[v.value]

    PLAN_FLAGS = {"sorted": 1, "packed": 2, "two_level": 4, "hist_in_scan": 8, "key8": 16, "key16": 32,
                  "high_water": 64, "anchored": 128, "wire_packed": 256, "own_in_place": 512,
                  "flagged": 1024, "ordered": 2048,
                  "combined": 4096, "route_l1": 8192, "route_tuned": 16384, "rl1_head": 262144,
                  "compact": 524288, "hot_direct": 1048576, "table": 2097152,
                  "sync": 4194304, "fanin": 8388608, "fanout": 16777216}

    def last_plan(self) -> dict:
        v = ctypes.c_uint32(0)
        self._check(self._lib.crdt_last_plan(self._ctx, ctypes.byref(v)), "crdt_last_plan")
        plan = {k: bool(v.value & b) for k, b in self.PLAN_FLAGS.items()}
        plan["rl1_pieces"] = (v.value >> 15) & 7
        return plan

    def place_info(self) -> dict:
        n, kept, done = ctypes.c_int32(0), ctypes.c_int32(0), ctypes.c_int32(0)
        ms = (ctypes.c_float * 4)()
        self._check(self._lib.crdt_place_info(self._ctx, ctypes.byref(n), ctypes.byref(kept), ctypes.byref(done), ms),
                    "crdt_place_info")
        return {"candidates": n.value, "kept": kept.value if kept.value >= 0 else None, "merges_used": done.value,
                "level1_ms": [round(float(m), 3) for m in ms[:max(n.value, 0)]]}

    TUNE_WAYS = ("route_l1", "combine", "route_l1_4", "route_l1_1", "route_l1_head")

    def route_tune(self) -> dict:
        best = ctypes.c_int32(0)
        us = (ctypes.c_int64 * 5)()
        self._check(self._lib.crdt_route_tune_info(self._ctx, ctypes.byref(best), us), "crdt_route_tune_info")
        out = {"best": self.TUNE_WAYS[best.value] if 0 <= best.value < len(self.TUNE_WAYS) else None}
        for w, u in zip(self.TUNE_WAYS, us):
            out[f"{w}_ms"] = u / 1e3 if u >= 0 else None
        return out

    def set_timing(self, enable: bool):
        self._check(self._lib.crdt_set_timing(self._ctx, int(bool(enable))), "crdt_set_timing")

    def timing(self) -> dict:
        t = CrdtTiming()
        self._check(self._lib.crdt_get_timing(self._ctx, ctypes.byref(t)), "crdt_get_timing")
        return t.as_dict()
```

include/crdt_merge.h:

```cpp
#ifndef CRDT_MERGE_H
#define CRDT_MERGE_H

#include <stdint.h>

#ifdef __cplusplus
extern "C" {
#endif

#define CRDT_ABI_VERSION 5
#define CRDT_NULL_VALUE 0xFFFFFFFFu

enum crdt_status {
    CRDT_OK = 0,
    CRDT_CLOCK_DRIFT = 1,
    CRDT_DUPLICATE_NODE = 2,
    CRDT_OVERFLOW = 3,
    CRDT_E_INVALID = -1,
    CRDT_E_HIP = -2,
    CRDT_E_NOMEM = -3,
    CRDT_E_KEY_RANGE = -4,
    CRDT_E_NO_DEVICE = -5,
    CRDT_E_COMM = -6
};

// ... 9 lines not shown
    const int64_t* millis;
    const uint64_t* offsets;
    uint32_t n_changesets;
    int32_t mem;
} crdt_batch;

typedef struct crdt_result {
    int32_t status;
    uint32_t n_stored;
    uint32_t exc_changeset;
    uint32_t reserved;
    uint64_t exc_index;
    int64_t canonical_lt;
    int64_t drift_ms;
    int64_t counter;
    uint64_t n_present;
    uint64_t n_won;
} crdt_result;

typedef struct crdt_timing {
    double scan_ms;
    double clock_ms;
    double apply_ms;
    uint32_t apply_launches;
    uint32_t apply_total;
    double total_ms;
    double route_ms;
    double part1_ms;
    double part2_ms;
    double resolve_ms;
    uint64_t part1_records;
    uint64_t sent_bytes;
} crdt_timing;

int crdt_abi_version(void);
const char* crdt_status_string(int status);
int crdt_device_count(int* out);

int crdt_create(int device, uint32_t local_rank, uint64_t capacity, crdt_ctx** out);
void crdt_destroy(crdt_ctx* ctx);
int crdt_reserve(crdt_ctx* ctx, uint64_t capacity);
int crdt_reserve_scratch(crdt_ctx* ctx, uint64_t n_records);
int crdt_set_row_bytes(crdt_ctx* ctx, uint32_t row_bytes);
int crdt_capacity(const crdt_ctx* ctx, uint64_t* out);
int crdt_set_local_rank(crdt_ctx* ctx, uint32_t rank);

int crdt_get_canonical(const crdt_ctx* ctx, int64_t* lt);
int crdt_set_canonical(crdt_ctx* ctx, int64_t lt);

int crdt_put_rows(crdt_ctx* ctx, const uint32_t* key_id, const int64_t* lt, const uint32_t* rank,
                  const uint32_t* val, const int64_t* mod, uint64_t n, int32_t mem);
int crdt_read_rows(crdt_ctx* ctx, const uint32_t* key_id, uint64_t n, int64_t* lt, uint32_t* rank,
                   uint32_t* val, int64_t* mod, int32_t mem);
int crdt_modified_since(crdt_ctx* ctx, uint64_t n_rows, int64_t since_lt, uint32_t* out_ids,
                        uint64_t* n_out);
typedef struct crdt_export {
    const uint32_t* key_id;
    const int64_t* lt;
    const uint32_t* rank;
    const uint32_t* val;
    const int64_t* mod;
    uint64_t n;
    uint64_t n_live;
    int32_t mem;
    int32_t device;
} crdt_export;
int crdt_export_since(crdt_ctx* ctx, uint64_t n_rows, int64_t since_lt, crdt_export* out);
int crdt_export_read(crdt_ctx* ctx, uint64_t first, uint64_t count, uint32_t* key_id, int64_t* lt,
                     uint32_t* rank, uint32_t* val, int64_t* mod);
int crdt_export_release(crdt_ctx* ctx);
int crdt_count_since(crdt_ctx* ctx, uint64_t n_rows, int64_t since_lt, uint64_t* n, uint64_t* n_live);
int crdt_export_flagged(crdt_ctx* ctx, uint64_t n_rows, const uint8_t* flags, int32_t flags_mem,
                        uint8_t bits, crdt_export* out);
int crdt_clear_rows(crdt_ctx* ctx, uint64_t first, uint64_t count);
int crdt_remap_ranks(crdt_ctx* ctx, uint64_t n_rows, const uint32_t* old_to_new, uint32_t n_ranks);

int crdt_put_stamped(crdt_ctx* ctx, const uint32_t* key_id, const uint32_t* val, uint64_t n,
                     int64_t wall_millis, int32_t mem, crdt_result* out);

int crdt_refresh_canonical(crdt_ctx* ctx, uint64_t n_rows, int64_t* out_lt);

int crdt_merge(crdt_ctx* ctx, const crdt_batch* batch, int64_t wall_millis, uint8_t* win_flags,
               crdt_result* out);

int crdt_merge_table(crdt_ctx* dst, crdt_ctx* src, uint64_t n_rows, int64_t since_lt, int64_t wall_millis,
                     uint8_t* row_flags, int32_t flags_mem, crdt_result* out);

int crdt_sync_tables(crdt_ctx* a, crdt_ctx* b, uint64_t n_rows, int64_t since_a, int64_t since_b,
                     int64_t wall_millis, uint8_t* flags_a, uint8_t* flags_b, int32_t flags_mem,
                     crdt_result* out_a, crdt_result* out_b);

#define CRDT_FANIN_MAX 8
int crdt_fanin_tables(crdt_ctx* dst, crdt_ctx* const* srcs, const int64_t* since_lt, uint32_t n_src,
                      uint64_t n_rows, int64_t wall_millis, uint8_t* win_mask, int32_t mask_mem,
                      crdt_result* out );

#define CRDT_FANOUT_MAX 8
int crdt_fanout_tables(crdt_ctx* src, crdt_ctx* const* dsts, const int64_t* since_lt, uint32_t n_dst,
                       uint64_t n_rows, int64_t wall_millis, uint8_t* win_mask, int32_t mask_mem,
                       crdt_result* out );

enum crdt_reduce_op { CRDT_REDUCE_SUM = 0, CRDT_REDUCE_MAX = 1, CRDT_REDUCE_MIN = 2 };

typedef struct crdt_comm_ops {
    void* user;
    int32_t mem;
    int32_t reserved;
    int (*all_reduce_i64)(void* user, int64_t* words, uint64_t n, int32_t op, void* stream);
    int (*all_gather_i64)(void* user, const int64_t* send, int64_t* recv, uint64_t n, void* stream);
    int (*all_to_all_v)(void* user, uint32_t n_cols, const void* const* send_cols, void* const* recv_cols,
                        const uint32_t* elem_bytes, const uint64_t* send_counts, const uint64_t* send_displs,
                        const uint64_t* recv_counts, const uint64_t* recv_displs, void* stream);
} crdt_comm_ops;

#define CRDT_COMM_ID_BYTES 128
int crdt_comm_unique_id(uint8_t* id );
int crdt_comm_init_rccl(crdt_ctx* ctx, uint32_t n_ranks, uint32_t rank, const uint8_t* id);
int crdt_comm_init_ops(crdt_ctx* ctx, uint32_t n_ranks, uint32_t rank, const crdt_comm_ops* ops);
int crdt_comm_info(const crdt_ctx* ctx, uint32_t* n_ranks, uint32_t* rank);
int crdt_comm_free(crdt_ctx* ctx);
int crdt_set_comm_timeout(crdt_ctx* ctx, uint32_t ms);
int crdt_comm_state(const crdt_ctx* ctx, int32_t* state, const char** phase);
int crdt_set_presharded(crdt_ctx* ctx, int presharded);

enum crdt_path { CRDT_PATH_AUTO = 0, CRDT_PATH_GATHER = 1, CRDT_PATH_SORTED = 2 };
int crdt_set_merge_path(crdt_ctx* ctx, int path);

int crdt_set_counts(crdt_ctx* ctx, int exact);
int crdt_set_rank_bound(crdt_ctx* ctx, uint32_t bound);
int crdt_last_path(const crdt_ctx* ctx, int* path);
enum crdt_plan_flags {
    CRDT_PLAN_SORTED = 1,
    CRDT_PLAN_PACKED = 2,
    CRDT_PLAN_TWO_LEVEL = 4,
    CRDT_PLAN_HIST_IN_SCAN = 8,
    CRDT_PLAN_KEY8 = 16,
    CRDT_PLAN_KEY16 = 32,
    CRDT_PLAN_HIGH_WATER = 64,
    CRDT_PLAN_ANCHORED = 128,
    CRDT_PLAN_WIRE_PACKED = 256,
    CRDT_PLAN_OWN_IN_PLACE = 512,
    CRDT_PLAN_FLAGGED = 1024,
    CRDT_PLAN_ORDERED = 2048,
    CRDT_PLAN_COMBINED = 4096,
    CRDT_PLAN_ROUTE_L1 = 8192,
    CRDT_PLAN_ROUTE_TUNED = 16384,
    CRDT_PLAN_RL1_PIECES_SHIFT = 15,
    CRDT_PLAN_RL1_HEAD = 262144,
    CRDT_PLAN_COMPACT = 524288,
    CRDT_PLAN_HOT_DIRECT = 1048576,
    CRDT_PLAN_TABLE = 2097152,
    CRDT_PLAN_SYNC = 4194304,
    CRDT_PLAN_FANIN = 8388608,
    CRDT_PLAN_FANOUT = 16777216
};
int crdt_last_plan(const crdt_ctx* ctx, uint32_t* flags);

int crdt_route_tune_info(const crdt_ctx* ctx, int32_t* best, int64_t* us );

int crdt_place_info(const crdt_ctx* ctx, int32_t* n, int32_t* kept, int32_t* done, float* ms );

int crdt_set_timing(crdt_ctx* ctx, int enable);
int crdt_get_timing(const crdt_ctx* ctx, crdt_timing* out);

#ifdef __cplusplus
}
#endif
#endif
```

Before: 55.79 billion.

## Overlap item-list building on side stream and fuse hot/cold L1 scan chains

```diff
diff --git a/crdt_amd/_capi.py b/crdt_amd/_capi.py
--- a/crdt_amd/_capi.py
+++ b/crdt_amd/_capi.py
@@ -135,6 +135,7 @@
     "crdt_reserve_scratch": (_INT, [_P, _U64]),
     "crdt_set_row_bytes": (_INT, [_P, _U32]),
     "crdt_last_plan": (_INT, [_P, _P]),
+    "crdt_last_hot_records": (_INT, [_P, _P]),
     "crdt_route_tune_info": (_INT, [_P, _P, _P]),
     "crdt_place_info": (_INT, [_P, _P, _P, _P, _P]),
     "crdt_last_path": (_INT, [_P, _P]),
diff --git a/crdt_amd/csrc/crdt_merge.hip b/crdt_amd/csrc/crdt_merge.hip
--- a/crdt_amd/csrc/crdt_merge.hip
+++ b/crdt_amd/csrc/crdt_merge.hip
@@ -203,22 +203,35 @@
     uint32_t* hhist = nullptr;
 };
 
-__global__ __launch_bounds__(1024) void k_hot_count(const uint32_t* __restrict__ hhist, uint64_t tiles, uint32_t hot,
-                                                    Misc* __restrict__ misc)
+constexpr uint32_t kHotCountGrid = 1024;
+__global__ __launch_bounds__(256) void k_hot_count(const uint32_t* __restrict__ hhist, uint64_t tiles, uint32_t hot,
+                                                   unsigned long long* __restrict__ part)
 {
-    __shared__ unsigned long long s_sum[16];
+    __shared__ unsigned long long s_sum[4];
+    const uint32_t lane = threadIdx.x & 63, w = threadIdx.x >> 6;
     unsigned long long n = 0;
-    const uint64_t words = tiles * 256;
-    for (uint64_t x = (uint64_t)blockIdx.x * 1024 + threadIdx.x; x < words; x += (uint64_t)gridDim.x * 1024)
-        if ((x & 255u) < hot) n += hhist[x];
+#pragma unroll 4
+    for (uint64_t t = (uint64_t)blockIdx.x * 4 + w; t < tiles; t += (uint64_t)gridDim.x * 4) {
+        const uint32_t* h = hhist + t * 256;
+        for (uint32_t b = lane; b < hot; b += 64) n += h[b];
+    }
+#pragma unroll
+    for (int off = 32; off > 0; off >>= 1) n += __shfl_xor(n, off, 64);
+    if (lane == 0) s_sum[w] = n;
+    __syncthreads();
+    if (threadIdx.x == 0) part[blockIdx.x] = s_sum[0] + s_sum[1] + s_sum[2] + s_sum[3];
+}
+__global__ __launch_bounds__(256) void k_hot_sum(const unsigned long long* __restrict__ part, uint32_t n_part,
+                                                 Misc* __restrict__ misc)
+{
+    __shared__ unsigned long long s_sum[4];
+    unsigned long long n = 0;
+    for (uint32_t x = threadIdx.x; x < n_part; x += 256) n += part[x];
 #pragma unroll
     for (int off = 32; off > 0; off >>= 1) n += __shfl_xor(n, off, 64);
     if ((threadIdx.x & 63) == 0) s_sum[threadIdx.x >> 6] = n;
     __syncthreads();
-    if (threadIdx.x == 0) {
-        for (int k = 1; k < 16; ++k) n += s_sum[k];
-        if (n) atomicAdd(&misc->hot_n, n);
-    }
+    if (threadIdx.x == 0) misc->hot_n = s_sum[0] + s_sum[1] + s_sum[2] + s_sum[3];
 }
 
 template <bool kEager, bool kMillis, bool kFrame, bool kHist, bool kVec, bool kHot = false>
@@ -1758,6 +1771,7 @@
     DBuf<uint32_t> p_hist, p_toff, p_part, p_choff, p_dstart1, p_dstart2, p_l2map;
     DBuf<uint64_t> p_plan, p_l1beg;
     DBuf<uint32_t> p_ibase, p_ksu32, p_tseg, p_ibucket;
+    DBuf<uint32_t> p_tseg2;
     DBuf<uint32_t> p_ilist;
     HBuf<uint32_t> h_ilist;
     DBuf<int64_t> p_kslt;
@@ -1804,8 +1818,12 @@
     uint32_t hot_skip = 0;
     uint32_t hist1_hot = 0;
     bool last_hot_direct = false;
+    bool last_l1_one_chain = false;
+    bool last_lists_early = false;
+    uint64_t last_hot_n = 0;
     DBuf<uint32_t> p_hist1h, p_toffh, p_dstarth;
     DBuf<uint64_t> p_l1begh;
+    DBuf<unsigned long long> p_hotpart;
     int route_l1 = 1;
     bool rl1_call_head = false;
     bool rl1_call_all = false;
@@ -1840,6 +1858,7 @@
     HBuf<unsigned long long> h_hcnt;
     hipEvent_t rl_evh = nullptr;
     hipEvent_t ov_ev[2] = {};
+    hipEvent_t il_ev[2] = {};
     DBuf<uint32_t> e_key, e_val;
     DBuf<uint64_t> e_pk;
     DBuf<unsigned long long> e_cnt, e_cur;
@@ -1957,6 +1976,20 @@
     return CRDT_OK;
 }
 
+int lists_fork(crdt_ctx* c) {
+    if (!c->sstream) HIPCHK(hipStreamCreateWithFlags(&c->sstream, hipStreamNonBlocking));
+    for (hipEvent_t& e : c->il_ev)
+        if (!e) HIPCHK(hipEventCreateWithFlags(&e, hipEventDisableTiming));
+    HIPCHK(hipEventRecord(c->il_ev[0], c->stream));
+    HIPCHK(hipStreamWaitEvent(c->sstream, c->il_ev[0], 0));
+    return CRDT_OK;
+}
+int lists_join(crdt_ctx* c) {
+    HIPCHK(hipEventSynchronize(c->il_ev[1]));
+    HIPCHK(hipStreamWaitEvent(c->stream, c->il_ev[1], 0));
+    return CRDT_OK;
+}
+
 template <typename T>
 int stage(crdt_ctx* c, DBuf<T>& buf, const T* src, uint64_t n, int32_t mem, const T** out) {
     if (!src) { *out = nullptr; return CRDT_OK; }
@@ -2120,6 +2153,7 @@
     }
     if (hot) {
         HIPALLOC(c->p_hist1h.ensure(c->plan_ptiles * kDigits));
+        HIPALLOC(c->p_hotpart.ensure(kHotCountGrid));
         c->hist1_hot = hot;
     }
     const ScanHot shot{hot, c->p_hist1h.p};
@@ -2185,8 +2219,11 @@
                     cols.lt, cols.rank, cols.millis, c->d_offs, c->d_tstart, jb, c->canonical, wall,
                     c->local_rank, c->d_T.p, c->d_misc, c->d_candtile.p, ScanHist{}, jx);
         }
-        if (hot)
-            k_hot_count<<<64, 1024, 0, c->stream>>>(c->p_hist1h.p, c->plan_ptiles, hot, c->d_misc);
+        if (hot) {
+            const uint32_t gh = (uint32_t)std::max<uint64_t>(1, std::min<uint64_t>(kHotCountGrid, (c->plan_ptiles + 3) / 4));
+            k_hot_count<<<gh, 256, 0, c->stream>>>(c->p_hist1h.p, c->plan_ptiles, hot, c->p_hotpart.p);
+            k_hot_sum<<<1, 256, 0, c->stream>>>(c->p_hotpart.p, gh, c->d_misc);
+        }
         if (!c->fused)
             k_tmax<<<std::min<uint32_t>(R, 4096), 256, 0, c->stream>>>(c->d_T.p, c->d_tstart, R, d_maxima);
         HIPCHK(hipGetLastError());
@@ -2500,6 +2537,9 @@
     c->key_end_valid = true;
     c->last_hist1_fused = false;
     c->last_hot_direct = false;
+    c->last_l1_one_chain = false;
+    c->last_lists_early = false;
+    c->last_hot_n = 0;
     c->sorted_phases = false;
     const bool k8 = pk && two && pf.key4 && !(c->form_off & kFormNoKey8);
     const bool k16 = k8 && !(c->form_off & kFormNoKey16);
@@ -2567,7 +2607,7 @@
                               c->stream));
         const uint32_t nt2 = two ? (uint32_t)((nw + kPTile2 - 1) / kPTile2) + kDigits : 0;
         const uint32_t nc2 = two ? (nt2 + kChunkTiles - 1) / kChunkTiles + kDigits : 0;
-        const uint32_t ntm = std::max(nt1, nt2), ncm = std::max(nc1, nc2);
+        const uint32_t ntm = std::max(nt1, nt2), ncm = std::max(2 * nc1, nc2);
         HIPALLOC(c->p_hist.ensure((size_t)ntm * kDigits));
         HIPALLOC(c->p_toff.ensure((size_t)ntm * kDigits));
         HIPALLOC(c->p_part.ensure((size_t)ncm * kDigits));
@@ -2602,7 +2642,7 @@
         const uint64_t* d_end = c->p_plan.p + nseg;
         const uint32_t* d_sj = reinterpret_cast<const uint32_t*>(c->p_plan.p + 2 * (size_t)nseg);
         const uint32_t* d_tb1 = d_sj + nseg;
-        HIPALLOC(c->p_tseg.ensure(ntm));
+        HIPALLOC(c->p_tseg.ensure(nt1));
         k_seg_index<<<std::min<uint32_t>(grid_for(nt1, 256), 4096), 256, 0, c->stream>>>(d_tb1, nseg, nt1, c->p_tseg.p);
         const TileMap tm1{d_beg, d_end, d_tb1, c->p_tseg.p, d_sj, nseg, l1t};
         const ScanMap sm1z{reinterpret_cast<const uint32_t*>(c->p_plan.p + tail),
@@ -2614,6 +2654,7 @@
         const uint32_t* hist1 = h1 ? c->p_hist1.p : c->p_hist.p;
         const uint32_t hb = h1 ? c->hist1_hot : 0u;
         const uint64_t hot_n = hb && pk ? std::min<uint64_t>(c->h_misc->hot_n, nw) : 0;
+        if (hb && pk && s0 == 0) c->last_hot_n = c->h_misc->hot_n;
         const bool hotp = hb && cmp && !ord && !em && two && !c->has_comm && hot_n * 100 >= (uint64_t)c->hot_share * nw;
         if (hb && !hotp) {
             k_hot_fold<<<std::min<uint32_t>(nt1, 1024u), 64, 0, c->stream>>>(c->p_hist1.p, c->p_hist1h.p, nt1);
@@ -2621,27 +2662,92 @@
             c->hot_skip = c->hot_probe;
         }
         c->last_hot_direct = hotp;
+        c->last_l1_one_chain = hotp;
+        c->last_hist1_fused = h1;
         if (hotp) {
             HIPALLOC(c->p_toffh.ensure((size_t)nt1 * kDigits));
             HIPALLOC(c->p_dstarth.ensure(kDigits + 1));
             HIPALLOC(c->p_l1begh.ensure(kDigits + 1));
             HIPALLOC(c->p2_rec.ensure(rec_units));
-            k_hist_trim<<<256, 256, 0, c->stream>>>(c->p_hist1h.p, c->d_ptb, R, c->d_misc);
-            k_scan_part<<<nc1, 256, 0, c->stream>>>(c->p_hist1h.p, sm1z, c->p_part.p);
-            k_scan_seg<<<1, 256, 0, c->stream>>>(c->p_part.p, sm1z, c->p_choff.p, c->p_dstarth.p, c->p_l1begh.p);
-            k_scan_tiles<<<nc1, 256, 0, c->stream>>>(c->p_hist1h.p, c->p_choff.p, sm1z, c->p_dstarth.p, c->p_toffh.p);
-        }
-        const ScanMap sm1 = hotp ? ScanMap{sm1z.tbase, sm1z.cbase, c->p_l1begh.p + kDigits, 1} : sm1z;
-        if (h1)
-            k_hist_trim<<<256, 256, 0, c->stream>>>(c->p_hist1.p, c->d_ptb, R, c->d_misc);
-        else
-            k_part_hist<true><<<nt1, kHThreads, 0, c->stream>>>(cols.key, tm1, jb, c->d_misc,
-                                                                 c->cap, shift1, c->p_hist.p);
-        c->last_hist1_fused = h1;
-        k_scan_part<<<nc1, 256, 0, c->stream>>>(hist1, sm1, c->p_part.p);
-        k_scan_seg<<<1, 256, 0, c->stream>>>(c->p_part.p, sm1, c->p_choff.p, c->p_dstart1.p,
-                                             two ? c->p_l1beg.p : nullptr);
-        k_scan_tiles<<<nc1, 256, 0, c->stream>>>(hist1, c->p_choff.p, sm1, c->p_dstart1.p, c->p_toff.p);
+            uint32_t* part_h = c->p_part.p + (size_t)nc1 * kDigits;
+            uint32_t* choff_h = c->p_choff.p + (size_t)nc1 * kDigits;
+            k_hist_trim<<<dim3(256, 2), 256, 0, c->stream>>>(c->p_hist1.p, c->d_ptb, R, c->d_misc, c->p_hist1h.p);
+            k_scan_part<<<dim3(nc1, 2), 256, 0, c->stream>>>(hist1, sm1z, c->p_part.p, c->p_hist1h.p, part_h);
+            k_scan_seg_hot<<<2, 256, 0, c->stream>>>(c->p_part.p, part_h, sm1z, c->p_choff.p, choff_h, c->p_dstart1.p,
+                                                     c->p_l1beg.p, c->p_dstarth.p, c->p_l1begh.p);
+            k_scan_tiles<<<dim3(nc1, 2), 256, 0, c->stream>>>(hist1, c->p_choff.p, sm1z, c->p_dstart1.p, c->p_toff.p,
+                                                              c->p_hist1h.p, choff_h, c->p_dstarth.p, c->p_toffh.p);
+        } else {
+            if (h1)
+                k_hist_trim<<<256, 256, 0, c->stream>>>(c->p_hist1.p, c->d_ptb, R, c->d_misc);
+            else
+                k_part_hist<true><<<nt1, kHThreads, 0, c->stream>>>(cols.key, tm1, jb, c->d_misc,
+                                                                     c->cap, shift1, c->p_hist.p);
+            k_scan_part<<<nc1, 256, 0, c->stream>>>(hist1, sm1z, c->p_part.p);
+            k_scan_seg<<<1, 256, 0, c->stream>>>(c->p_part.p, sm1z, c->p_choff.p, c->p_dstart1.p,
+                                                 two ? c->p_l1beg.p : nullptr);
+            k_scan_tiles<<<nc1, 256, 0, c->stream>>>(hist1, c->p_choff.p, sm1z, c->p_dstart1.p, c->p_toff.p);
+        }
+        const uint32_t ts2 = k16 && !(c->form_off & kFormNoHistW) && !(c->form_off & kFormBigTile2)
+                             ? (uint32_t)kPTile2 : (uint32_t)kPTile;
+        uint32_t *tb2 = nullptr, *cb2 = nullptr;
+        if (two) {
+            HIPALLOC(c->p_l2map.ensure(2 * (kDigits + 1)));
+            HIPALLOC(c->p_tseg2.ensure(nt2));
+            HIPALLOC(c->p_dstart2.ensure(kDigits * kDigits + 1));
+            tb2 = c->p_l2map.p;
+            cb2 = c->p_l2map.p + kDigits + 1;
+            k_l2_plan<<<1, 256, 0, c->stream>>>(c->p_l1beg.p, tb2, cb2, ts2);
+            k_seg_index<<<std::min<uint32_t>(grid_for(nt2, 256), 4096), 256, 0, c->stream>>>(tb2, kDigits, nt2,
+                                                                                            c->p_tseg2.p);
+        }
+        const uint32_t nb = two ? kDigits * kDigits : kDigits;
+        const uint32_t* bst = two ? c->p_dstart2.p : c->p_dstart1.p;
+        const uint32_t max_items = nb + (uint32_t)(nw / kRPart) + 1;
+        const size_t ksn = (size_t)(2 * (nw / kRPart) + 2) * kSKeys;
+        const uint32_t max_hot = std::min<uint32_t>(nb, (uint32_t)(nw / kRPart) + 1);
+        HIPALLOC(c->p_ibase.ensure(2 * (nb + 1) + 1 + max_hot));
+        HIPALLOC(c->p_kslt.ensure(2 * ksn));
+        HIPALLOC(c->p_ksu32.ensure(6 * ksn));
+        uint32_t* d_ib = c->p_ibase.p;
+        uint32_t* d_hb = c->p_ibase.p + nb + 1;
+        uint32_t* d_hot = c->p_ibase.p + 2 * (nb + 1);
+        HIPALLOC(c->p_ibucket.ensure(max_items));
+        const bool free_pk = !em && !ord && !c->counts && pk;
+        const bool spk = c->sparse_t > 0 && !(c->form_off & (kFormNoSparseK | kFormNoWholeLines));
+        const bool lists = !c->has_comm && !(c->form_off & kFormNoItemLists) &&
+                           (ord || (free_pk && !(c->form_off & kFormNoWholeLines)));
+        uint32_t il_fold = max_items, il_dense = max_items, il_sparse = max_items, il_hot = max_hot, il_items = max_items;
+        auto lists_launch = [&]() -> int {
+            int st;
+            HIPALLOC(c->p_ilist.ensure(kListHead + 3 * (size_t)max_items));
+            HIPALLOC(c->h_ilist.ensure(kListHead));
+            if ((st = lists_fork(c))) return st;
+            k_bucket_items<<<(nb + 1023) / 1024, 1024, 0, c->sstream>>>(bst, nb, d_ib, d_hb, d_hot, c->d_misc, nullptr);
+            k_seg_index<<<std::min<uint32_t>(grid_for(max_items, 256), 4096), 256, 0, c->sstream>>>(
+                d_ib, nb, max_items, c->p_ibucket.p);
+            k_item_lists<<<(nb + 1023) / 1024, 1024, 0, c->sstream>>>(
+                bst, nb, d_ib, d_hb, d_hot, free_pk && spk ? c->hw_read : 0, free_pk && spk ? c->sparse_t : 0,
+                c->p_ilist.p, max_items);
+            HIPCHK(hipMemcpyAsync(c->h_ilist.p, c->p_ilist.p, kListHead * sizeof(uint32_t), hipMemcpyDeviceToHost,
+                                  c->sstream));
+            HIPCHK(hipEventRecord(c->il_ev[1], c->sstream));
+            c->last_lists_early = true;
+            return CRDT_OK;
+        };
+        auto lists_wait = [&]() -> int {
+            int st;
+            if ((st = lists_join(c))) return st;
+            const uint32_t* h = c->h_ilist.p;
+            if (h[0] > max_items || h[1] > max_items || h[2] > max_items || h[3] > max_hot || h[4] > max_items)
+                return CRDT_E_HIP;
+            il_fold = h[0]; il_dense = h[1]; il_sparse = h[2]; il_hot = h[3]; il_items = h[4];
+            return CRDT_OK;
+        };
+        if (lists && !two) {
+            int st;
+            if ((st = lists_launch())) return st;
+        }
         const bool ph = c->timing && s0 == 0 && !em;
         if (ph) ev_record(c, ev_window(1, false));
         if (c->place_timed && s0 == 0) HIPCHK(hipEventRecord(c->place_ev[0], c->stream));
@@ -2710,15 +2816,9 @@
         const uint32_t* h2f = nullptr;
         const uint32_t* t2f = nullptr;
         if (two) {
-            HIPALLOC(c->p_l2map.ensure(2 * (kDigits + 1)));
-            HIPALLOC(c->p_dstart2.ensure(kDigits * kDigits + 1));
             HIPALLOC(c->p2_rec.ensure(rec_units)); HIPALLOC(c->p2_kj.ensure(kj2_units));
             p2r = c->p2_rec.p;
             p2k = c->p2_kj.p;
-            uint32_t* tb2 = c->p_l2map.p;
-            uint32_t* cb2 = c->p_l2map.p + kDigits + 1;
-            const uint32_t ts2 = k16 && !(c->form_off & kFormNoHistW) && !(c->form_off & kFormBigTile2)
-                                 ? (uint32_t)kPTile2 : (uint32_t)kPTile;
             if (fl) {
                 HIPALLOC(c->f_hist2.ensure((size_t)nt2 * kDigits));
                 HIPALLOC(c->f_toff2.ensure((size_t)nt2 * kDigits));
@@ -2727,10 +2827,7 @@
             uint32_t* t2p = fl ? c->f_toff2.p : c->p_toff.p;
             h2f = h2p;
             t2f = t2p;
-            k_l2_plan<<<1, 256, 0, c->stream>>>(c->p_l1beg.p, tb2, cb2, ts2);
-            k_seg_index<<<std::min<uint32_t>(grid_for(nt2, 256), 4096), 256, 0, c->stream>>>(tb2, kDigits, nt2,
-                                                                                            c->p_tseg.p);
-            const TileMap tm2{c->p_l1beg.p, c->p_l1beg.p + 1, tb2, c->p_tseg.p, nullptr, kDigits, ts2};
+            const TileMap tm2{c->p_l1beg.p, c->p_l1beg.p + 1, tb2, c->p_tseg2.p, nullptr, kDigits, ts2};
             tm2f = tm2;
             nt2f = (uint32_t)((nw + ts2 - 1) / ts2) + kDigits;
             const ScanMap sm2{tb2, cb2, c->p_l1beg.p, kDigits};
@@ -2753,6 +2850,10 @@
             k_scan_seg<<<kDigits, 256, 0, c->stream>>>(c->p_part.p, sm2, c->p_choff.p, c->p_dstart2.p, nullptr);
             k_scan_tiles<<<nc2, 256, 0, c->stream>>>(h2p, c->p_choff.p, sm2, c->p_dstart2.p, t2p);
             if (hotp) k_hot_starts<<<1, 256, 0, c->stream>>>(c->p_dstart2.p, c->p_dstarth.p, hb);
+            if (lists) {
+                int st;
+                if ((st = lists_launch())) return st;
+            }
             const uint64_t nw2 = hotp ? nw - hot_n : nw;
             const uint32_t nt2s = (uint32_t)((nw2 + ts2 - 1) / ts2) + kDigits;
             const uint32_t xper2 = c->xcd_map ? (nt2s + kXcds - 1) / kXcds : 0;
@@ -2796,44 +2897,22 @@
                     p1r, p1k, tm2, kSBits, t2p, p2r, p2k, xper2, rev1 ? h2p : nullptr);
         }
         if (ph) ev_record(c, ev_window(2, true));
-        const uint32_t nb = two ? kDigits * kDigits : kDigits;
-        const uint32_t* bst = two ? c->p_dstart2.p : c->p_dstart1.p;
         const u32x4* rec = two ? p2r : p1r;
         const uint32_t* rv = two ? p2k : p1k;
-        const uint32_t max_items = nb + (uint32_t)(nw / kRPart) + 1;
-        const size_t ksn = (size_t)(2 * (nw / kRPart) + 2) * kSKeys;
-        const uint32_t max_hot = std::min<uint32_t>(nb, (uint32_t)(nw / kRPart) + 1);
-        HIPALLOC(c->p_ibase.ensure(2 * (nb + 1) + 1 + max_hot));
-        HIPALLOC(c->p_kslt.ensure(2 * ksn));
-        HIPALLOC(c->p_ksu32.ensure(6 * ksn));
-        uint32_t* d_ib = c->p_ibase.p;
-        uint32_t* d_hb = c->p_ibase.p + nb + 1;
-        uint32_t* d_hot = c->p_ibase.p + 2 * (nb + 1);
         KeyState ps{c->p_kslt.p, c->p_ksu32.p, c->p_ksu32.p + ksn, c->p_ksu32.p + 2 * ksn};
         KeyState cy{c->p_kslt.p + ksn, c->p_ksu32.p + 3 * ksn, c->p_ksu32.p + 4 * ksn, c->p_ksu32.p + 5 * ksn};
-        HIPALLOC(c->p_ibucket.ensure(max_items));
         const bool ov = !em && pk && (ord || !c->counts) && two && (c->form_off & kFormOverlap);
         if (ph) ev_record(c, ev_window(3, false));
-        if (em) HIPALLOC(c->e_bbase.ensure(nb));
-        k_bucket_items<<<(nb + 1023) / 1024, 1024, 0, c->stream>>>(bst, nb, d_ib, d_hb, d_hot, c->d_misc,
-                                                                    em ? c->e_bbase.p : nullptr);
-        k_seg_index<<<std::min<uint32_t>(grid_for(max_items, 256), 4096), 256, 0, c->stream>>>(d_ib, nb, max_items,
-                                                                                               c->p_ibucket.p);
-        auto item_lists = [&](uint64_t hw_s, uint32_t sparse_s, uint32_t* n_fold, uint32_t* n_dense, uint32_t* n_sparse,
-                              uint32_t* n_hot, uint32_t* n_items) -> int {
-            HIPALLOC(c->p_ilist.ensure(kListHead + 3 * (size_t)max_items));
-            HIPALLOC(c->h_ilist.ensure(kListHead));
-            k_item_lists<<<(nb + 1023) / 1024, 1024, 0, c->stream>>>(bst, nb, d_ib, d_hb, d_hot, hw_s, sparse_s,
-                                                                    c->p_ilist.p, max_items);
-            HIPCHK(hipMemcpyAsync(c->h_ilist.p, c->p_ilist.p, kListHead * sizeof(uint32_t), hipMemcpyDeviceToHost,
-                                  c->stream));
-            HIPCHK(hipStreamSynchronize(c->stream));
-            const uint32_t* h = c->h_ilist.p;
-            if (h[0] > max_items || h[1] > max_items || h[2] > max_items || h[3] > max_hot || h[4] > max_items)
-                return CRDT_E_HIP;
-            *n_fold = h[0]; *n_dense = h[1]; *n_sparse = h[2]; *n_hot = h[3]; *n_items = h[4];
-            return CRDT_OK;
-        };
+        if (lists) {
+            int st;
+            if ((st = lists_wait())) return st;
+        } else {
+            if (em) HIPALLOC(c->e_bbase.ensure(nb));
+            k_bucket_items<<<(nb + 1023) / 1024, 1024, 0, c->stream>>>(bst, nb, d_ib, d_hb, d_hot, c->d_misc,
+                                                                        em ? c->e_bbase.p : nullptr);
+            k_seg_index<<<std::min<uint32_t>(grid_for(max_items, 256), 4096), 256, 0, c->stream>>>(d_ib, nb, max_items,
+                                                                                                   c->p_ibucket.p);
+        }
         if (em) {
             const uint32_t n_items = max_items + max_hot * (kSKeys / 256);
             const size_t slots = (size_t)std::min<uint64_t>(nw, (uint64_t)nb * kSKeys) + 1;
@@ -2881,12 +2960,8 @@
             if (fl) HIPALLOC(c->f_flag2.ensure(nw + 8));
             uint8_t* fl2 = fl ? c->f_flag2.p : nullptr;
             int st = CRDT_OK;
-            uint32_t g_fold = max_items, g_hot = max_hot, g_items = max_items, g_d, g_s;
-            const uint32_t* l_fold = nullptr;
-            if (!c->has_comm && !(c->form_off & kFormNoItemLists)) {
-                if ((st = item_lists(0, 0, &g_fold, &g_d, &g_s, &g_hot, &g_items))) return st;
-                l_fold = c->p_ilist.p + kListHead;
-            }
+            const uint32_t g_fold = il_fold, g_hot = il_hot, g_items = il_items;
+            const uint32_t* l_fold = lists ? c->p_ilist.p + kListHead : nullptr;
             if ((st = ov ? overlap_fork(c) : CRDT_OK)) return st;
             const hipStream_t fs = ov ? c->sstream : c->stream;
             if (!g_fold) {
@@ -2949,8 +3024,6 @@
                 else { CRDT_FBACK2(0, false); }
 #undef CRDT_FBACK2
                 f1 = c->f_flag1.p;
-                k_seg_index<<<std::min<uint32_t>(grid_for(nt1, 256), 4096), 256, 0, c->stream>>>(d_tb1, nseg, nt1,
-                                                                                                 c->p_tseg.p);
             }
             const bool fx1 = c->xcd_map && (c->form_off & kFormFbackXcd);
             const uint32_t xf1 = fx1 ? (nt1 + kXcds - 1) / kXcds : 0;
@@ -2981,16 +3054,10 @@
             uint64_t* ps_key = reinterpret_cast<uint64_t*>(c->p_kslt.p);
             uint32_t* ps_val = c->p_ksu32.p;
             const Rec12* rec12 = reinterpret_cast<const Rec12*>(rec);
-            const bool spk = c->sparse_t > 0 && !(c->form_off & (kFormNoSparseK | kFormNoWholeLines));
             int st = CRDT_OK;
-            const bool lists = !c->has_comm && !(c->form_off & (kFormNoItemLists | kFormNoWholeLines));
-            uint32_t g_fold = max_items, g_dense = max_items, g_sparse = max_items, g_hot = max_hot;
+            const uint32_t g_fold = il_fold, g_dense = il_dense, g_sparse = il_sparse, g_hot = il_hot;
             const uint32_t *l_fold = nullptr, *l_dense = nullptr, *l_sparse = nullptr;
             if (lists) {
-                uint32_t g_items;
-                if ((st = item_lists(spk ? c->hw_read : 0, spk ? c->sparse_t : 0, &g_fold, &g_dense, &g_sparse, &g_hot,
-                                     &g_items)))
-                    return st;
                 l_fold = c->p_ilist.p + kListHead;
                 l_dense = l_fold + max_items;
                 l_sparse = l_dense + max_items;
@@ -3314,6 +3381,7 @@
     if (c->rl_evo) hipEventDestroy(c->rl_evo);
     if (c->rl_evh) hipEventDestroy(c->rl_evh);
     for (hipEvent_t e : c->ov_ev) if (e) hipEventDestroy(e);
+    for (hipEvent_t e : c->il_ev) if (e) hipEventDestroy(e);
     if (c->sstream) hipStreamDestroy(c->sstream);
     if (c->ostream) hipStreamDestroy(c->ostream);
     if (c->table.base) hipFree(c->table.base);
@@ -3335,11 +3403,11 @@
     c->p1_rec.release(); c->p1_kj.release(); c->p2_rec.release(); c->p2_kj.release();
     for (int i = 0; i < crdt_ctx::kPlaceMax; ++i) { c->pc_rec[i].release(); c->pc_kj[i].release(); }
     for (hipEvent_t e : c->place_ev) if (e) hipEventDestroy(e);
-    c->p_hist1h.release(); c->p_toffh.release(); c->p_dstarth.release(); c->p_l1begh.release();
+    c->p_hist1h.release(); c->p_toffh.release(); c->p_dstarth.release(); c->p_l1begh.release(); c->p_hotpart.release();
     c->p_hist.release(); c->p_hist1.release(); c->p_toff.release(); c->p_part.release(); c->p_choff.release();
     c->p_dstart1.release(); c->p_dstart2.release(); c->p_l2map.release();
     c->p_plan.release(); c->p_l1beg.release(); c->h_pplan.release();
-    c->p_ibase.release(); c->p_ksu32.release(); c->p_kslt.release(); c->p_tseg.release();
+    c->p_ibase.release(); c->p_ksu32.release(); c->p_kslt.release(); c->p_tseg.release(); c->p_tseg2.release();
     c->p_ibucket.release(); c->p_ilist.release(); c->h_ilist.release();
     c->f_pos1.release(); c->f_pos2.release(); c->f_flag1.release(); c->f_flag2.release();
     c->f_cin_key.release(); c->f_cin_val.release(); c->f_cin_pres.release();
@@ -4368,6 +4436,8 @@
         if (c->last_route_l1) f |= CRDT_PLAN_ROUTE_L1;
         if (c->last_compact) f |= CRDT_PLAN_COMPACT;
         if (c->last_hot_direct) f |= CRDT_PLAN_HOT_DIRECT;
+        if (c->last_lists_early) f |= CRDT_PLAN_LISTS_EARLY;
+        if (c->last_l1_one_chain) f |= CRDT_PLAN_L1_ONE_CHAIN;
     }
     if (c->last_wire_pk) f |= CRDT_PLAN_WIRE_PACKED;
     if (c->last_own_in_place) f |= CRDT_PLAN_OWN_IN_PLACE;
@@ -4378,6 +4448,12 @@
     return CRDT_OK;
 }
 
+int crdt_last_hot_records(const crdt_ctx* c, uint64_t* n) {
+    if (!c || !n) return CRDT_E_INVALID;
+    *n = c->last_sorted && !c->last_table ? c->last_hot_n : 0;
+    return CRDT_OK;
+}
+
 int crdt_place_info(const crdt_ctx* c, int32_t* n, int32_t* kept, int32_t* done, float* ms) {
     if (!c || !n || !kept || !done || !ms) return CRDT_E_INVALID;
     *n = c->place_k;
diff --git a/crdt_amd/csrc/sorted_path.inc b/crdt_amd/csrc/sorted_path.inc
--- a/crdt_amd/csrc/sorted_path.inc
+++ b/crdt_amd/csrc/sorted_path.inc
@@ -191,10 +191,12 @@
 }
 
 __global__ __launch_bounds__(256) void k_hist_trim(uint32_t* __restrict__ hist, const uint32_t* __restrict__ ptb,
-                                                   uint32_t R, const Misc* __restrict__ misc)
+                                                   uint32_t R, const Misc* __restrict__ misc,
+                                                   uint32_t* __restrict__ hist_y = nullptr)
 {
     const uint32_t stop = misc->stop;
     if (stop >= R) return;
+    if (blockIdx.y) hist = hist_y;
     const uint64_t a = (uint64_t)ptb[stop] * kDigits, b = (uint64_t)ptb[R] * kDigits;
     for (uint64_t x = a + (uint64_t)blockIdx.x * 256 + threadIdx.x; x < b; x += (uint64_t)gridDim.x * 256)
         hist[x] = 0;
@@ -222,10 +224,13 @@
 static_assert(kDigits == 256, "k_scan<.., kHist> counts 256 digits");
 
 __global__ __launch_bounds__(256) void k_scan_part(const uint32_t* __restrict__ hist, ScanMap sm,
-                                                   uint32_t* __restrict__ part)
+                                                   uint32_t* __restrict__ part,
+                                                   const uint32_t* __restrict__ hist_y = nullptr,
+                                                   uint32_t* __restrict__ part_y = nullptr)
 {
     const uint32_t c = blockIdx.x;
     if (c >= sm.cbase[sm.nseg]) return;
+    if (blockIdx.y) { hist = hist_y; part = part_y; }
     const uint32_t s = seg_of(sm.cbase, sm.nseg, c);
     const uint32_t t0 = sm.tbase[s] + (c - sm.cbase[s]) * kChunkTiles;
     const uint32_t t1 = std::min<uint32_t>(t0 + kChunkTiles, sm.tbase[s + 1]);
@@ -261,13 +266,55 @@
     if (s + 1 == sm.nseg && d == kDigits - 1) dstart[(uint64_t)sm.nseg * kDigits] = (uint32_t)(sm.seg_pos[s] + total);
 }
 
+__global__ __launch_bounds__(256) void k_scan_seg_hot(const uint32_t* __restrict__ part,
+                                                      const uint32_t* __restrict__ part_h, ScanMap sm,
+                                                      uint32_t* __restrict__ choff, uint32_t* __restrict__ choff_h,
+                                                      uint32_t* __restrict__ dstart, uint64_t* __restrict__ dstart64,
+                                                      uint32_t* __restrict__ dstart_h,
+                                                      uint64_t* __restrict__ dstart64_h)
+{
+    __shared__ uint32_t s_w[4];
+    const bool hotwg = blockIdx.x == 1;
+    const uint32_t d = threadIdx.x;
+    const uint32_t c0 = sm.cbase[0], c1 = sm.cbase[1];
+    uint32_t run = 0, run_h = 0;
+    if (hotwg) { part = part_h; choff = choff_h; dstart = dstart_h; dstart64 = dstart64_h; }
+#pragma unroll 8
+    for (uint32_t c = c0; c < c1; ++c) {
+        const uint32_t v = part[(uint64_t)c * kDigits + d];
+        if (!hotwg) run_h += part_h[(uint64_t)c * kDigits + d];
+        choff[(uint64_t)c * kDigits + d] = run;
+        run += v;
+    }
+    uint64_t base = sm.seg_pos[0];
+    uint32_t total;
+    if (!hotwg) {
+        scan256_excl(run_h, s_w, &total);
+        base += total;
+        __syncthreads();
+    }
+    const uint32_t ex = scan256_excl(run, s_w, &total);
+    const uint64_t pos = base + ex;
+    dstart[d] = (uint32_t)pos;
+    if (dstart64) dstart64[d] = pos;
+    if (d == kDigits - 1) {
+        dstart[kDigits] = (uint32_t)(base + total);
+        if (dstart64) dstart64[kDigits] = base + total;
+    }
+}
+
 __global__ __launch_bounds__(256) void k_scan_tiles(const uint32_t* __restrict__ hist,
                                                     const uint32_t* __restrict__ choff, ScanMap sm,
                                                     const uint32_t* __restrict__ dstart,
-                                                    uint32_t* __restrict__ toff)
+                                                    uint32_t* __restrict__ toff,
+                                                    const uint32_t* __restrict__ hist_y = nullptr,
+                                                    const uint32_t* __restrict__ choff_y = nullptr,
+                                                    const uint32_t* __restrict__ dstart_y = nullptr,
+                                                    uint32_t* __restrict__ toff_y = nullptr)
 {
     const uint32_t c = blockIdx.x;
     if (c >= sm.cbase[sm.nseg]) return;
+    if (blockIdx.y) { hist = hist_y; choff = choff_y; dstart = dstart_y; toff = toff_y; }
     const uint32_t s = seg_of(sm.cbase, sm.nseg, c);
     const uint32_t t0 = sm.tbase[s] + (c - sm.cbase[s]) * kChunkTiles;
     const uint32_t t1 = std::min<uint32_t>(t0 + kChunkTiles, sm.tbase[s + 1]);
diff --git a/crdt_amd/device.py b/crdt_amd/device.py
--- a/crdt_amd/device.py
+++ b/crdt_amd/device.py
@@ -458,13 +458,18 @@
                   "flagged": 1024, "ordered": 2048,
                   "combined": 4096, "route_l1": 8192, "route_tuned": 16384, "rl1_head": 262144,
                   "compact": 524288, "hot_direct": 1048576, "table": 2097152,
-                  "sync": 4194304, "fanin": 8388608, "fanout": 16777216}
+                  "sync": 4194304, "fanin": 8388608, "fanout": 16777216, "lists_early": 33554432,
+                  "l1_one_chain": 67108864}
 
     def last_plan(self) -> dict:
         v = ctypes.c_uint32(0)
         self._check(self._lib.crdt_last_plan(self._ctx, ctypes.byref(v)), "crdt_last_plan")
         plan = {k: bool(v.value & b) for k, b in self.PLAN_FLAGS.items()}
         plan["rl1_pieces"] = (v.value >> 15) & 7
+        plan["l1_chains"] = (2 if plan["hot_direct"] and not plan["l1_one_chain"] else 1) if plan["sorted"] else 0
+        n = ctypes.c_uint64(0)
+        self._check(self._lib.crdt_last_hot_records(self._ctx, ctypes.byref(n)), "crdt_last_hot_records")
+        plan["hot_records"] = n.value
         return plan
 
     def place_info(self) -> dict:
diff --git a/include/crdt_merge.h b/include/crdt_merge.h
--- a/include/crdt_merge.h
+++ b/include/crdt_merge.h
@@ -185,9 +185,12 @@
     CRDT_PLAN_TABLE = 2097152,
     CRDT_PLAN_SYNC = 4194304,
     CRDT_PLAN_FANIN = 8388608,
-    CRDT_PLAN_FANOUT = 16777216
+    CRDT_PLAN_FANOUT = 16777216,
+    CRDT_PLAN_LISTS_EARLY = 33554432,
+    CRDT_PLAN_L1_ONE_CHAIN = 67108864
 };
 int crdt_last_plan(const crdt_ctx* ctx, uint32_t* flags);
+int crdt_last_hot_records(const crdt_ctx* ctx, uint64_t* n);
 
 int crdt_route_tune_info(const crdt_ctx* ctx, int32_t* best, int64_t* us );
 
```

Measured after the change: 56.47 billion, median of 2. No clear change (+1.2%).
